# DeepBlender/DeepDenoiser

Hardware: AMD Instinct MI355X
Metric: train tiles/sec (128x128x32ch U-Net KPCN) (higher is better)
Workload: dtype bf16; 1 GPU; BASELINE config 2: U-Net [64,96,128]x4 + 5x5 KernelPrediction + 3-scale MultiScalePrediction, 32-channel render-pass stack, 128x128 tiles, full training step (fwd+SMAPE loss+bwd+Adam); global_batch=128, parallelism=dp1, hipgraph=True, inputs=resident in HBM

## Files before the change

### deepdenoiser_amd/_lib.py

```python

import ctypes as C
import os

_HERE = os.path.dirname(os.path.abspath(__file__))
LIB_PATH = os.environ.get("DD_LIB", os.path.join(_HERE, "libdd_hip.so"))

DD_F32, DD_BF16, DD_F16 = 0, 1, 2
IN_RELU, OUT_RELU, ACCUM, PIXSHUF, GATHER2X2 = 1, 2, 4, 8, 16
MAX_FEATURES, MAX_COMBINED = 32, 8
METRIC_SOURCES = MAX_FEATURES + MAX_COMBINED + 1
HISTOGRAM_DIFFERENCE, HISTOGRAM_VARIATION_DIFFERENCE, HISTOGRAM_MASKED_DIFFERENCE = 0, 1, 2
HISTOGRAM_VALUES_SCRATCH_BYTES = 20480
PREVIEW_SOURCE, PREVIEW_PREDICTION, PREVIEW_TARGET, PREVIEW_DIFFERENCE = 1, 2, 4, 8
PREVIEW_MAX_IMAGES, PREVIEW_THRESHOLDS = 16, 255
NONFINITE_MAX_PLANES = 32


def histogram_stats_offset(nb):
    return (nb + 1) // 2 * 8


def histogram_record_bytes(nb):
    return histogram_stats_offset(nb) + 48


SYMBOLS = (
    "dd_version", "dd_last_error", "dd_pack_weights", "dd_pack_weights_batched", "dd_conv_igemm", "dd_conv_wgrad", "dd_colsum", "dd_colsum_segments",
    "dd_maxpool_fwd", "dd_maxpool_bwd", "dd_avgpool", "dd_prepare_feature", "dd_gather_input",
    "dd_kpcn_fwd", "dd_kpcn_bwd", "dd_kpcn_hidden_fwd", "dd_kpcn_hidden_bwd", "dd_compose_pack", "dd_compose_blend_fwd", "dd_compose_blend_bwd",
    "dd_compose_unpack_bwd", "dd_invert_std_fwd", "dd_invert_std_bwd", "dd_loss_head", "dd_adam_step",
    "dd_stitch", "dd_recombine", "dd_probe_tr16", "dd_masked_add", "dd_zero_stuff", "dd_zero_unstuff", "dd_convert_channels",
    "dd_augment", "dd_loss_mask_sums", "dd_crc32c", "dd_extract_tiles", "dd_compose_net_fwd", "dd_compose_net_bwd",
    "dd_kpcn_head_fwd", "dd_kpcn_head_bwd", "dd_kpcn_head_bwd_multi", "dd_assemble_input", "dd_assemble_input_frames", "dd_conv3x3_bwd", "dd_conv3x3_bwd_multi", "dd_convt2x2_fwd", "dd_convt2x2_bwd", "dd_conv3x3_ks",
    "dd_conv_pw_count", "dd_wgrad_pw_count", "dd_space_to_depth2", "dd_convt3_wgrad", "dd_compose_stream_plan", "dd_compose_bwd_scratch_bytes",
    "dd_loss_msssim_scratch_bytes", "dd_loss_msssim_fwd", "dd_loss_msssim_bwd", "dd_loss_msssim_values",
    "dd_loss_metrics_scratch_bytes", "dd_loss_metrics", "dd_loss_head_path_count",
    "dd_loss_head_dscale", "dd_loss_msssim_bwd_dscale", "dd_grads_nonfinite", "dd_adam_step_scaled", "dd_scaler_update",
    "dd_histogram_values", "dd_loss_histograms_scratch_bytes", "dd_loss_histograms", "dd_loss_previews",
    "dd_nonfinite_scan", "dd_nonfinite_repair",
)


class ConvT3WgradArgs(C.Structure):
    _fields_ = [("s", C.c_void_p), ("lds", C.c_int), ("cout", C.c_int), ("cp", C.c_int),
                ("x", C.c_void_p), ("ldx", C.c_int), ("cin", C.c_int),
                ("dk", C.c_void_p),
                ("B", C.c_int), ("H", C.c_int), ("W", C.c_int), ("dtype", C.c_int)]


class ConvArgs(C.Structure):
    _fields_ = [("x", C.c_void_p), ("ldx", C.c_int), ("cin", C.c_int),
                ("wp", C.c_void_p), ("k_pad", C.c_int), ("n_pad", C.c_int),
                ("bias", C.c_void_p), ("nbias", C.c_int),
                ("res", C.c_void_p), ("ldres", C.c_int),
                ("mask", C.c_void_p), ("ldmask", C.c_int),
                ("y", C.c_void_p), ("ldy", C.c_int), ("n", C.c_int),
                ("B", C.c_int), ("H", C.c_int), ("W", C.c_int),
                ("taps", C.c_int), ("flags", C.c_int), ("dtype", C.c_int)]


class WgradArgs(C.Structure):
    _fields_ = [("p", C.c_void_p), ("ldp", C.c_int), ("m", C.c_int),
                ("q", C.c_void_p), ("ldq", C.c_int), ("n", C.c_int),
                ("out", C.c_void_p), ("bias_out", C.c_void_p), ("bias_mode", C.c_int),
                ("B", C.c_int), ("H", C.c_int), ("W", C.c_int),
                ("taps", C.c_int), ("flags", C.c_int), ("dtype", C.c_int), ("ksplit", C.c_int),
                ("stack_blocks", C.c_int), ("stack_width", C.c_int), ("stack_m0", C.c_int),
                ("stack_out", C.c_void_p * 8), ("stack_bias", C.c_void_p * 8)]


class ConvBwdArgs(C.Structure):
    _fields_ = [("dy", C.c_void_p), ("ld_dy", C.c_int), ("cout", C.c_int),
                ("x", C.c_void_p), ("ld_x", C.c_int), ("cin", C.c_int),
                ("wd", C.c_void_p), ("n_pad", C.c_int), ("k_pad", C.c_int),
                ("dx", C.c_void_p), ("ld_dx", C.c_int),
                ("dw", C.c_void_p), ("db", C.c_void_p),
                ("B", C.c_int), ("H", C.c_int), ("W", C.c_int),
                ("use_mask", C.c_int), ("accumulate", C.c_int), ("dtype", C.c_int)]


class ConvTArgs(C.Structure):
    _fields_ = [("x", C.c_void_p), ("ld_x", C.c_int), ("cin", C.c_int),
                ("y", C.c_void_p), ("ld_y", C.c_int), ("cout", C.c_int),
                ("w", C.c_void_p), ("n_pad", C.c_int), ("k_pad", C.c_int),
                ("bias", C.c_void_p), ("relu", C.c_int),
                ("dx", C.c_void_p), ("ld_dx", C.c_int), ("dw", C.c_void_p), ("db", C.c_void_p), ("use_mask", C.c_int), ("accumulate", C.c_int),
                ("B", C.c_int), ("H", C.c_int), ("W", C.c_int), ("dtype", C.c_int)]


class ConvKsArgs(C.Structure):
    _fields_ = [("x", C.c_void_p), ("ldx", C.c_int), ("cin", C.c_int),
                ("wp", C.c_void_p), ("n_pad", C.c_int), ("k_pad", C.c_int),
                ("bias", C.c_void_p), ("nbias", C.c_int),
                ("y", C.c_void_p), ("ldy", C.c_int),
                ("n0", C.c_int), ("n", C.c_int),
                ("B", C.c_int), ("H", C.c_int), ("W", C.c_int),
                ("mode", C.c_int), ("flags", C.c_int), ("dtype", C.c_int),
                ("mask", C.c_void_p), ("ldmask", C.c_int)]


class PackDesc(C.Structure):
    _fields_ = [("src", C.c_void_p), ("dst", C.c_void_p), ("taps", C.c_int), ("n", C.c_int), ("k", C.c_int), ("n_pad", C.c_int),
                ("k_pad", C.c_int), ("tap_flip", C.c_int), ("s_tap", C.c_long), ("s_n", C.c_long), ("s_k", C.c_long),
                ("dst_ld", C.c_long), ("dst_tap_stride", C.c_long)]


class FeatureParams(C.Structure):
    _fields_ = [("use_log1p", C.c_int), ("mean", C.c_float), ("inv_std", C.c_float),
                ("use_variance", C.c_int), ("variance_before", C.c_int), ("mode_neighbor", C.c_int),
                ("relative", C.c_int), ("compress", C.c_int), ("epsilon", C.c_float)]


class GatherEntry(C.Structure):
    _fields_ = [("src", C.c_void_p), ("pixel_stride", C.c_int), ("batch_stride_pixels", C.c_int),
                ("nch", C.c_int), ("dst_ch", C.c_int)]


class AssembleEntry(C.Structure):
    _fields_ = [("src", C.c_void_p), ("cs", C.c_int), ("kind", C.c_int), ("fp", FeatureParams), ("nch", C.c_int), ("dst_ch", C.c_int),
                ("std_out", C.c_void_p), ("ld_std", C.c_int)]


class LossDesc(C.Structure):
    _fields_ = [("n_features", C.c_int),
                ("pred", C.c_void_p * MAX_FEATURES), ("target", C.c_void_p * MAX_FEATURES),
                ("dpred", C.c_void_p * MAX_FEATURES),
                ("target_ld", C.c_int * MAX_FEATURES), ("pred_ld", C.c_int * MAX_FEATURES), ("nch", C.c_int * MAX_FEATURES),
                ("weight", C.c_float * MAX_FEATURES), ("var_weight", C.c_float * MAX_FEATURES),
                ("masked_weight", C.c_float * MAX_FEATURES), ("mask_feature", C.c_int * MAX_FEATURES),
                ("n_combined", C.c_int), ("comb", (C.c_int * 3) * MAX_COMBINED),
                ("comb_weight", C.c_float * MAX_COMBINED), ("comb_var_weight", C.c_float * MAX_COMBINED),
                ("comb_masked_weight", C.c_float * MAX_COMBINED), ("comb_mask_feature", C.c_int * MAX_COMBINED),
                ("n_image_combined", C.c_int), ("image_combined", C.c_int * MAX_COMBINED),
                ("n_image_features", C.c_int), ("image_features", C.c_int * MAX_FEATURES),
                ("image_weight", C.c_float), ("image_var_weight", C.c_float), ("kind", C.c_int), ("epsilon", C.c_float),
                ("mask_sums", C.c_void_p),
                ("pred_std", C.c_void_p * MAX_FEATURES), ("pred_inv", C.c_void_p * MAX_FEATURES),
                ("inv_log1p", C.c_int * MAX_FEATURES), ("inv_mean", C.c_float * MAX_FEATURES), ("inv_std", C.c_float * MAX_FEATURES)]


class MsSsimDesc(C.Structure):
    _fields_ = [("n_features", C.c_int),
                ("pred", C.c_void_p * MAX_FEATURES), ("target", C.c_void_p * MAX_FEATURES), ("dpred", C.c_void_p * MAX_FEATURES),
                ("target_ld", C.c_int * MAX_FEATURES), ("pred_ld", C.c_int * MAX_FEATURES), ("nch", C.c_int * MAX_FEATURES),
                ("ssim_weight", C.c_float * MAX_FEATURES),
                ("n_combined", C.c_int), ("comb", (C.c_int * 3) * MAX_COMBINED), ("comb_ssim_weight", C.c_float * MAX_COMBINED),
                ("n_image_combined", C.c_int), ("image_combined", C.c_int * MAX_COMBINED),
                ("n_image_features", C.c_int), ("image_features", C.c_int * MAX_FEATURES),
                ("image_ssim_weight", C.c_float)]


class ScalerState(C.Structure):
    _fields_ = [("scale", C.c_float), ("good_steps", C.c_int), ("found_nonfinite", C.c_int), ("adam_t", C.c_int), ("skipped_total", C.c_int)]


class AugmentDraw(C.Structure):
    _fields_ = [("flip", C.c_int), ("rotate", C.c_int), ("permute", C.c_int), ("normal_rotation", C.c_float * 9)]


AUG_PLAIN, AUG_RGB, AUG_NORMAL, AUG_SCREEN_NORMAL = 0, 1, 2, 3


class StitchEntry(C.Structure):
    _fields_ = [("tile", C.c_int), ("crop_y0", C.c_int), ("crop_y1", C.c_int), ("crop_x0", C.c_int),
                ("crop_x1", C.c_int), ("dst_img", C.c_int), ("dst_y", C.c_int), ("dst_x", C.c_int)]


class ComposeArgs(C.Structure):
    _fields_ = [("small", C.c_void_p), ("ld_small", C.c_int), ("fine", C.c_void_p), ("ld_fine", C.c_int), ("out", C.c_void_p), ("ld_out", C.c_int),
                ("w_in", C.c_void_p), ("b_in", C.c_void_p), ("w_res", C.c_void_p * 4), ("b_res", C.c_void_p * 4),
                ("w_out", C.c_void_p), ("b_out", C.c_void_p),
                ("save_netin", C.c_void_p), ("ld_netin", C.c_int), ("save_act", C.c_void_p * 5), ("ld_act", C.c_int * 5),
                ("save_wl", C.c_void_p), ("ld_wl", C.c_int),
                ("N", C.c_int), ("H", C.c_int), ("W", C.c_int), ("dtype", C.c_int)]


class ComposeBwdArgs(C.Structure):
    _fields_ = [("small", C.c_void_p), ("ld_small", C.c_int), ("fine", C.c_void_p), ("ld_fine", C.c_int), ("dout", C.c_void_p), ("ld_dout", C.c_int),
                ("act", C.c_void_p * 5), ("ld_act", C.c_int * 5), ("wl", C.c_void_p), ("ld_wl", C.c_int),
                ("w_in", C.c_void_p), ("w_res", C.c_void_p * 4), ("w_out", C.c_void_p),
                ("d_small", C.c_void_p), ("ld_dsmall", C.c_int), ("accumulate_small", C.c_int), ("d_fine", C.c_void_p), ("ld_dfine", C.c_int),
                ("dw_in", C.c_void_p), ("db_in", C.c_void_p), ("dw_res", C.c_void_p * 4), ("db_res", C.c_void_p * 4),
                ("dw_out", C.c_void_p), ("db_out", C.c_void_p),
                ("N", C.c_int), ("H", C.c_int), ("W", C.c_int), ("dtype", C.c_int),
                ("scratch", C.c_void_p), ("scratch_bytes", C.c_long)]


class HeadArgs(C.Structure):
    _fields_ = [("x", C.c_void_p), ("ldx", C.c_int), ("C", C.c_int), ("src", C.c_void_p), ("ldsrc", C.c_int),
                ("wa", C.c_void_p), ("ba", C.c_void_p), ("wb", C.c_void_p), ("bb", C.c_void_p),
                ("out", C.c_void_p), ("ld_out", C.c_int), ("dout", C.c_void_p), ("ld_dout", C.c_int),
                ("dx", C.c_void_p), ("ld_dx", C.c_int), ("accumulate_dx", C.c_int),
                ("dwa", C.c_void_p), ("dba", C.c_void_p), ("dwb", C.c_void_p), ("dbb", C.c_void_p),
                ("N", C.c_int), ("H", C.c_int), ("W", C.c_int), ("ksize", C.c_int), ("dtype", C.c_int)]


class RecombineDesc(C.Structure):
    _fields_ = [("n_triples", C.c_int), ("color", C.c_void_p * 4), ("direct", C.c_void_p * 4), ("indirect", C.c_void_p * 4),
                ("combined", C.c_void_p * 4), ("n_singles", C.c_int), ("single", C.c_void_p * 8), ("image", C.c_void_p)]


class NonfinitePlane(C.Structure):
    _fields_ = [("data", C.c_void_p), ("C", C.c_int), ("ld", C.c_int), ("mask", C.c_void_p)]


class NonfiniteDesc(C.Structure):
    _fields_ = [("n_planes", C.c_int), ("plane", NonfinitePlane * NONFINITE_MAX_PLANES)]


_lib = None


def _check_source_hash(lib):
    if "DD_LIB" in os.environ:
        return
    from . import build as _build
    try:
        want = _build.source_hash()
    except OSError:
        return
    got = lib.dd_version().decode()
    if ("src=" + want) not in got:
        raise RuntimeError("libdd_hip.so is stale: built from sources %s, the sources here hash to %s -- run `python -m deepdenoiser_amd.build`"
                           % (got.split("src=")[-1], want))


def source_hash():
    return load().dd_version().decode().split("src=")[-1]


def load():
    global _lib
    if _lib is not None:
        return _lib
    import torch
    if not os.path.exists(LIB_PATH):
        raise RuntimeError("libdd_hip.so is not built (%s missing): run `python -m deepdenoiser_amd.build`. "
                           "There is no CPU/PyTorch fallback for the hot path." % LIB_PATH)
    lib = C.CDLL(LIB_PATH)
    missing = [s for s in SYMBOLS if not hasattr(lib, s)]
    if missing:
        raise RuntimeError("libdd_hip.so lacks symbols %s: rebuild it" % missing)
    lib.dd_version.restype = C.c_char_p
    lib.dd_last_error.restype = C.c_char_p
    _check_source_hash(lib)
    for s in SYMBOLS[2:]:
        getattr(lib, s).restype = C.c_int
    vp, i, l, f = C.c_void_p, C.c_int, C.c_long, C.c_float
    lib.dd_pack_weights.argtypes = [vp, vp, i, i, i, i, i, i, l, l, l, i, vp]
    lib.dd_pack_weights_batched.argtypes = [vp, i, i, vp]
    lib.dd_conv_igemm.argtypes = [C.POINTER(ConvArgs), vp]
    lib.dd_conv_wgrad.argtypes = [C.POINTER(WgradArgs), vp]
    lib.dd_conv3x3_bwd.argtypes = [C.POINTER(ConvBwdArgs), vp]
    lib.dd_conv3x3_bwd_multi.argtypes = [C.POINTER(ConvBwdArgs), i, vp]
    lib.dd_convt2x2_fwd.argtypes = [C.POINTER(ConvTArgs), vp]
    lib.dd_convt2x2_bwd.argtypes = [C.POINTER(ConvTArgs), vp]
    lib.dd_conv3x3_ks.argtypes = [C.POINTER(ConvKsArgs), vp]
    lib.dd_space_to_depth2.argtypes = [vp, i, vp, i, i, i, i, i, i, i, vp]
    lib.dd_convt3_wgrad.argtypes = [C.POINTER(ConvT3WgradArgs), vp]
    lib.dd_conv_pw_count.argtypes = []
    lib.dd_conv_pw_count.restype = C.c_long
    lib.dd_wgrad_pw_count.argtypes = []
    lib.dd_wgrad_pw_count.restype = C.c_long
    lib.dd_colsum.argtypes = [vp, i, i, l, vp, i, vp]
    lib.dd_colsum_segments.argtypes = [vp, i, i, l, i, vp, i, vp, i, vp]
    lib.dd_maxpool_fwd.argtypes = [vp, i, vp, i, vp, i, i, i, i, i, i, i, i, vp]
    lib.dd_maxpool_bwd.argtypes = [vp, i, vp, vp, i, vp, i, i, i, i, i, i, i, i, i, vp]
    lib.dd_avgpool.argtypes = [vp, i, vp, i, i, i, i, i, i, vp]
    lib.dd_prepare_feature.argtypes = [vp, i, vp, i, C.POINTER(FeatureParams), i, i, i, vp]
    lib.dd_gather_input.argtypes = [vp, i, i, vp, i, i, i, i, i, i, vp]
    lib.dd_kpcn_fwd.argtypes = [vp, i, vp, i, vp, i, i, i, i, i, i, vp]
    lib.dd_kpcn_bwd.argtypes = [vp, i, vp, i, vp, i, vp, i, i, i, i, i, i, i, vp]
    lib.dd_kpcn_hidden_fwd.argtypes = [vp, i, vp, i, i, vp, i, vp, vp, i, i, i, i, i, i, vp]
    lib.dd_kpcn_hidden_bwd.argtypes = [vp, i, vp, i, i, vp, i, vp, vp, i, vp, i, i, i, i, i, i, i, vp]
    lib.dd_compose_pack.argtypes = [vp, i, vp, i, vp, i, i, i, i, i, i, vp]
    lib.dd_compose_blend_fwd.argtypes = [vp, i, vp, i, vp, i, vp, i, i, i, i, i, vp]
    lib.dd_compose_blend_bwd.argtypes = [vp, i, vp, i, vp, i, vp, i, vp, i, i, vp, i, vp, i, i, i, i, i, i, vp]
    lib.dd_compose_unpack_bwd.argtypes = [vp, i, vp, i, vp, i, i, i, i, i, vp]
    lib.dd_invert_std_fwd.argtypes = [vp, vp, l, i, f, f, vp]
    lib.dd_invert_std_bwd.argtypes = [vp, vp, vp, l, i, f, f, vp]
    lib.dd_loss_head.argtypes = [C.POINTER(LossDesc), i, i, i, vp, f, vp]
    lib.dd_loss_head_path_count.argtypes = [i]
    lib.dd_loss_head_path_count.restype = C.c_long
    lib.dd_loss_msssim_scratch_bytes.argtypes = [i, i, i, i]
    lib.dd_loss_msssim_scratch_bytes.restype = C.c_long
    lib.dd_loss_msssim_fwd.argtypes = [C.POINTER(MsSsimDesc), i, i, i, vp, vp, vp]
    lib.dd_loss_msssim_bwd.argtypes = [C.POINTER(MsSsimDesc), i, i, i, vp, f, vp]
    lib.dd_loss_msssim_values.argtypes = [C.POINTER(MsSsimDesc), i, i, i, vp, vp, vp]
    lib.dd_loss_metrics_scratch_bytes.argtypes = [i, i, i]
    lib.dd_loss_metrics_scratch_bytes.restype = C.c_long
    lib.dd_loss_metrics.argtypes = [C.POINTER(LossDesc), i, i, i, vp, vp, vp]
    lib.dd_histogram_values.argtypes = [vp, l, vp, i, vp, vp, vp]
    lib.dd_loss_histograms_scratch_bytes.argtypes = [i, i, i, i]
    lib.dd_loss_histograms_scratch_bytes.restype = C.c_long
    lib.dd_loss_histograms.argtypes = [C.POINTER(LossDesc), i, i, i, C.POINTER(C.c_int), i, vp, i, vp, vp, vp]
    lib.dd_loss_previews.argtypes = [C.POINTER(LossDesc), C.POINTER(vp), C.POINTER(C.c_int), i, i, i, C.POINTER(C.c_int), i, C.POINTER(C.c_int), i, i, vp, f, f,
                                     vp, vp]
    lib.dd_adam_step.argtypes = [vp, vp, vp, vp, l, f, f, f, f, f, vp]
    lib.dd_loss_head_dscale.argtypes = [C.POINTER(LossDesc), i, i, i, vp, vp, vp]
    lib.dd_loss_msssim_bwd_dscale.argtypes = [C.POINTER(MsSsimDesc), i, i, i, vp, vp, vp]
    lib.dd_grads_nonfinite.argtypes = [vp, l, vp, vp]
    lib.dd_adam_step_scaled.argtypes = [vp, vp, vp, vp, l, C.c_double, C.c_double, C.c_double, f, f, vp, vp]
    lib.dd_scaler_update.argtypes = [vp, f, f, i, f, f, vp]
    lib.dd_nonfinite_scan.argtypes = [C.POINTER(NonfiniteDesc), i, i, i, vp, vp]
    lib.dd_nonfinite_repair.argtypes = [C.POINTER(NonfiniteDesc), i, i, i, i, vp, vp]
    lib.dd_stitch.argtypes = [vp, i, i, vp, i, i, i, i, vp, i, vp]
    lib.dd_recombine.argtypes = [C.POINTER(RecombineDesc), l, vp]
    lib.dd_probe_tr16.argtypes = [vp, vp, vp, vp]
    lib.dd_masked_add.argtypes = [vp, i, vp, i, vp, i, i, l, i, i, vp]
    lib.dd_convert_channels.argtypes = [vp, i, i, vp, i, i, i, i, l, vp]
    lib.dd_zero_stuff.argtypes = [vp, i, vp, i, i, i, i, i, i, vp]
    lib.dd_zero_unstuff.argtypes = [vp, i, vp, i, vp, i, i, i, i, i, i, i, vp]
    lib.dd_augment.argtypes = [vp, vp, i, i, i, i, vp, i, i, i, i, i, vp]
    lib.dd_loss_mask_sums.argtypes = [vp, i, i, i, vp, vp]
    lib.dd_crc32c.argtypes = [vp, C.c_size_t, C.c_uint32, C.POINTER(C.c_uint32)]
    lib.dd_extract_tiles.argtypes = [vp, i, i, i, i, vp, i, i, vp, i, vp]
    lib.dd_compose_net_fwd.argtypes = [C.POINTER(ComposeArgs), vp]
    lib.dd_compose_net_bwd.argtypes = [C.POINTER(ComposeBwdArgs), vp]
    lib.dd_compose_stream_plan.argtypes = [i, i, i, i, C.POINTER(C.c_int)]
    lib.dd_compose_bwd_scratch_bytes.argtypes = [i, i, i]
    lib.dd_compose_bwd_scratch_bytes.restype = C.c_long
    lib.dd_assemble_input.argtypes = [vp, i, i, vp, i, i, i, i, i, i, vp]
    lib.dd_assemble_input_frames.argtypes = [vp, i, i, vp, i, i, i, i, i, i, vp, i, i, vp]
    lib.dd_kpcn_head_fwd.argtypes = [C.POINTER(HeadArgs), vp]
    lib.dd_kpcn_head_bwd.argtypes = [C.POINTER(HeadArgs), vp]
    lib.dd_kpcn_head_bwd_multi.argtypes = [C.POINTER(HeadArgs), i, vp]
    _lib = lib
    return lib


def check(rc):
    if rc != 0:
        raise RuntimeError("libdd_hip: %s (status %d)" % (load().dd_last_error().decode(), rc))
```

### deepdenoiser_amd/csrc/dd_compose_stream.h

```cpp
#pragma once
#include "dd_common.h"
#include <type_traits>

namespace {

typedef __attribute__((ext_vector_type(16))) float f32x16_t;
typedef __attribute__((ext_vector_type(2))) unsigned int cs_u32x2;

template <typename T> __device__ __forceinline__ f32x16_t mma32(uint4 a, uint4 b, f32x16_t c);
template <> __device__ __forceinline__ f32x16_t mma32<bf16_t>(uint4 a, uint4 b, f32x16_t c) {
  return __builtin_amdgcn_mfma_f32_32x32x16_bf16(__builtin_bit_cast(bf16x8_t, a), __builtin_bit_cast(bf16x8_t, b), c, 0, 0, 0);
}
template <> __device__ __forceinline__ f32x16_t mma32<f16_t>(uint4 a, uint4 b, f32x16_t c) {
  return __builtin_amdgcn_mfma_f32_32x32x16_f16(__builtin_bit_cast(f16x8_t, a), __builtin_bit_cast(f16x8_t, b), c, 0, 0, 0);
}

typedef __attribute__((ext_vector_type(4))) unsigned int cs_u32x4;
template <typename T> __device__ __forceinline__ f32x16_t mma32_zero(uint4 a, uint4 b);
template <> __device__ __forceinline__ f32x16_t mma32_zero<bf16_t>(uint4 a, uint4 b) {
  f32x16_t d;
  const cs_u32x4 av = {a.x, a.y, a.z, a.w}, bv = {b.x, b.y, b.z, b.w};
  asm volatile("v_mfma_f32_32x32x16_bf16 %0, %1, %2, 0" : "=&v"(d) : "v"(av), "v"(bv));
  return d;
}
template <> __device__ __forceinline__ f32x16_t mma32_zero<f16_t>(uint4 a, uint4 b) {
  f32x16_t d;
  const cs_u32x4 av = {a.x, a.y, a.z, a.w}, bv = {b.x, b.y, b.z, b.w};
  asm volatile("v_mfma_f32_32x32x16_f16 %0, %1, %2, 0" : "=&v"(d) : "v"(av), "v"(bv));
  return d;
}

template <typename T> __device__ __forceinline__ void unpack2(uint32_t w, float& lo, float& hi);
template <> __device__ __forceinline__ void unpack2<bf16_t>(uint32_t w, float& lo, float& hi) { lo = __uint_as_float(w << 16); hi = __uint_as_float(w & 0xffff0000u); }
template <> __device__ __forceinline__ void unpack2<f16_t>(uint32_t w, float& lo, float& hi) { unpack_f16x2(w, lo, hi); }
template <typename T> __device__ __forceinline__ uint32_t packo(float lo, float hi) {
  uint32_t w = pack2<T>(lo, hi);
  asm("" : "+v"(w));
  return w;
}
template <typename T> struct One;
template <> struct One<bf16_t> { static constexpr uint32_t v = 0x3f80u; };
template <> struct One<f16_t> { static constexpr uint32_t v = 0x3c00u; };

__device__ __forceinline__ float dpp_xor1(float v) { return __int_as_float(__builtin_amdgcn_update_dpp(0, __float_as_int(v), 0xB1, 0xF, 0xF, true)); }
__device__ __forceinline__ void both_halves(float v, float& lower, float& upper) {
  const cs_u32x2 r = __builtin_amdgcn_permlane32_swap(__float_as_uint(v), __float_as_uint(v), false, false);
  lower = __uint_as_float(r[0]); upper = __uint_as_float(r[1]);
}

constexpr int PIXB = 48;

struct Unit { int b, yb0, yb1, xs, xe, fx0; };

template <typename P>
__device__ __forceinline__ void decode_unit(const P& p, int u, Unit& U) {
  const int j = u % p.nb, t = u / p.nb;
  const int st = t % p.n_strips;
  U.b = t / p.n_strips;
  U.yb0 = j * p.BH; U.yb1 = min(p.H, U.yb0 + p.BH);
  U.xs = st * p.SO; U.xe = min(p.W, U.xs + p.SO);
  U.fx0 = p.n_strips > 1 ? U.xs - 4 : 0;
}

struct Cursor {
  int urel, i;
  Unit U;
  template <typename P>
  __device__ __forceinline__ void init(const P& p, int u0, int nunits, int V) {
    urel = V >= 0 ? V / p.VB : -1 - ((-V - 1) / p.VB);
    i = V - urel * p.VB;
    U = Unit{0, 0, 0, 0, 0, 0};
    if (urel >= 0 && urel < nunits) decode_unit(p, u0 + urel, U);
  }
  template <typename P>
  __device__ __forceinline__ void advance(const P& p, int u0, int nunits, int rows) {
    i += rows;
    while (i >= p.VB) {
      i -= p.VB;
      ++urel;
      if (urel >= 0 && urel < nunits) decode_unit(p, u0 + urel, U);
    }
  }
};

__device__ __forceinline__ int sfl(int v) { return __builtin_amdgcn_readfirstlane(v); }
__device__ __forceinline__ int opaque(int v) { asm volatile("" : "+v"(v)); return v; }
__device__ __forceinline__ int posmod(int v, int d) { const int m = v % d; return m < 0 ? m + d : m; }

template <typename T> __device__ __forceinline__ float split3(float v, int e) {
  const float hi = Elem<T>::to_f32(Elem<T>::from_f32(v));
  const float mid = Elem<T>::to_f32(Elem<T>::from_f32(v - hi));
  const float lo = Elem<T>::to_f32(Elem<T>::from_f32(v - hi - mid));
  return e == 0 ? hi : e == 1 ? mid : lo;
}

}
```

### deepdenoiser_amd/csrc/dd_compose_stream.hip

```cpp
#include "dd_compose_stream.h"

#ifdef CS_PROFILE
__device__ unsigned long long cs_phase[4][8];
#define CSP_DECL() unsigned long long csp_last = __builtin_readcyclecounter(); const bool csp_on = blockIdx.x == 0 && t == 0 && lane == 0
#define CSP(i) do { const unsigned long long now_ = __builtin_readcyclecounter(); if (csp_on) cs_phase[LAYER][i] += now_ - csp_last; csp_last = now_; } while (0)
extern "C" int dd_debug_cs_phases(unsigned long long* out32, int reset) {
  if (out32) (void)hipMemcpyFromSymbol(out32, HIP_SYMBOL(cs_phase), sizeof(unsigned long long) * 32);
  if (reset) { unsigned long long z[32] = {0}; (void)hipMemcpyToSymbol(HIP_SYMBOL(cs_phase), z, sizeof(z)); }
  return 0;
}
#else
#define CSP_DECL()
#define CSP(i)
#endif


namespace {

constexpr int KS_MAX = 16;
constexpr int AUX_BYTES = 16 + 3 * 1024;

struct CsP {
  const float* small; const float* fine; float* out;
  const float* w_in; const float* b_in; const float* w_res[4]; const float* b_res[4]; const float* w_out; const float* b_out;
  void* save_act[5]; void* save_wl; void* save_netin;
  int ld_small, ld_fine, ld_out, ld_act[5], ld_wl, ld_netin;
  int N, H, W;
  int FW, R, TPR;
  int n_strips, SO;
  int BH, nb, VB;
  int units;
};

template <typename T>
__device__ __forceinline__ void stage_weights(char* img, char* aux, const CsP& p, int tid) {
  for (int i = tid; i < 4 * KS_MAX * 64 * 8; i += 1024) {
    const int e = i & 7, ln = (i >> 3) & 63, c = (i >> 9) & (KS_MAX - 1), l = i >> 13;
    const int m = ln & 31, g = 2 * c + (ln >> 5);
    float v = 0.f;
    if (m < 24) {
      if (g < 27) v = p.w_res[l][((g / 3) * 24 + 8 * (g % 3) + e) * 24 + m];
      else if (g == 27) { if (e < 3) v = split3<T>(p.b_res[l][m], e); }
    }
    reinterpret_cast<T*>(img)[i] = Elem<T>::from_f32(v);
  }
  T* ax = reinterpret_cast<T*>(aux);
  for (int i = tid; i < 8 + 3 * 512; i += 1024) {
    float v = 0.f;
    if (i < 8) v = i < 3 ? 1.f : 0.f;
    else {
      const int j = i - 8, e = j & 7, ln = (j >> 3) & 63, which = j >> 9;
      const int m = ln & 31, h = ln >> 5;
      if (which == 0) { if (m == 0) v = p.w_out[e < 4 ? 4 * h + e : 8 + 4 * h + e - 4]; }
      else if (which == 1) { if (m == 0) v = e < 4 ? p.w_out[16 + 4 * h + e] : (e < 7 && h == 0) ? split3<T>(p.b_out[0], e - 4) : 0.f; }
      else if (m < 24) v = e < 3 ? p.w_in[((h ? 0 : 3) + e) * 24 + m] : (e < 6 && h == 0) ? split3<T>(p.b_in[m], e - 3) : 0.f;
    }
    ax[i] = Elem<T>::from_f32(v);
  }
}

template <typename T, int LAYER, bool SAVE, int NPRE>
__device__ __forceinline__ void cs_role(const CsP& p, char* smem, char* aux, int ring_bytes, int t, int lane, int u0, int nunits, int steps) {
  constexpr bool RESIDUAL = LAYER == 1 || LAYER == 3;
  constexpr bool FINAL = LAYER == 3;
  constexpr int KS = 14;
  constexpr uint32_t ONE = One<T>::v, ONE2 = ONE | (ONE << 16);
  const int R = p.R, TPR = p.TPR, FW = p.FW, VB = p.VB;
  const int n = lane & 31, h = lane >> 5;
  const int r = t / TPR, xc = t - r * TPR;
  const bool has_task = t < R * TPR;
  const int x = xc * 32 + n;
  const int pitch = (FW + 2) * PIXB, rp = R * pitch;
  const int D0 = 3 * R + 2, D1 = 2 * R + 2, D4 = 3 * R + 2;
  const int off1 = D0 * pitch, off2 = off1 + D1 * pitch, off3 = off2 + D1 * pitch, off4 = off3 + D1 * pitch;
  const int Din = LAYER == 0 ? D0 : D1;
  const int Dres = LAYER == 1 ? D0 : D4;
  const int in_bytes = Din * pitch, out_bytes = D1 * pitch, res_bytes = Dres * pitch, raw_bytes = D4 * pitch;
  char* rin = smem + (LAYER == 0 ? 0 : LAYER == 1 ? off1 : LAYER == 2 ? off2 : off3);
  char* rout = smem + (LAYER == 0 ? off1 : LAYER == 1 ? off2 : off3);
  char* rres = smem + (LAYER == 1 ? 0 : off4);

  uint4 wa[KS];
#pragma unroll
  for (int c = 0; c < KS; ++c) wa[c] = *reinterpret_cast<const uint4*>(smem + ((LAYER * KS_MAX + c) * 64 + lane) * 16);
  __syncthreads();
  for (int i = threadIdx.x; i < ring_bytes / 16; i += 1024) reinterpret_cast<uint4*>(smem)[i] = uint4{0u, 0u, 0u, 0u};

  const int H = p.H, W = p.W, h2 = H >> 1, w2 = W >> 1;
  const int lag = (LAYER + 1) * (R + 1);
  const int total_rows = nunits * VB;
  const int s_beg = has_task ? (lag - r + R - 1) / R : steps, s_end = has_task ? (total_rows + lag - r + R - 1) / R : steps;
  Cursor cur;
  cur.init(p, u0, nunits, r - lag);
  int o_in = posmod(r - lag, Din) * pitch, o_out = posmod(r - lag, D1) * pitch, o_res = posmod(r - lag, Dres) * pitch, o_raw = posmod(r - lag, D4) * pitch;
  auto wrap_add = [](int o, int add, int bytes) { o += add; return o >= bytes ? o - bytes : o; };
  const int xo = x * PIXB + h * 16;
  const int a4c = h ? x * PIXB : x * PIXB + 128;
  const int a13c = h ? (int)(aux - rin) : x * PIXB + 128;
  const int wr = (x + 1) * PIXB + h * 8;
  int ybase = 0, pixb = 0;
  bool col_in = false, col_own = false, cols_all_in = false;
  auto unit_values = [&](const Cursor& c, int& yb, int& pb, bool& ci, bool& co, bool& call) {
    const int gx = c.U.fx0 + x;
    yb = c.U.yb0 - 4;
    ci = (unsigned)gx < (unsigned)W;
    co = ci && gx >= c.U.xs && gx < c.U.xe;
    pb = c.U.b * H * W + (ci ? gx : 0);
    call = c.U.fx0 + xc * 32 >= 0 && c.U.fx0 + xc * 32 + 32 <= W;
  };
  unit_values(cur, ybase, pixb, col_in, col_own, cols_all_in);

  Cursor c0;
  int o0 = 0, ybase0 = 0, pixb0 = 0, pix0 = 0;
  bool col_in0 = false, col_own0 = false, cols_all_in0 = false, in0 = false, own0 = false, row_in0 = false;
  float xin[3] = {0.f, 0.f, 0.f};
  const int s0_end = has_task ? (total_rows - r + R - 1) / R : 0;
  auto load_x0 = [&](int s_next) {
    in0 = false; own0 = false; row_in0 = false;
    if (s_next < s0_end) {
      const int y = ybase0 + c0.i;
      row_in0 = (unsigned)y < (unsigned)H;
      in0 = row_in0 && col_in0;
      own0 = in0 && col_own0 && y >= c0.U.yb0 && y < c0.U.yb1;
      const int cy = row_in0 ? y : 0;
      pix0 = pixb0 + cy * W;
      const int cx = pix0 - (c0.U.b * H + cy) * W;
      const float* src = h ? p.small + (size_t)((c0.U.b * h2 + (cy >> 1)) * w2 + (cx >> 1)) * p.ld_small : p.fine + (size_t)pix0 * p.ld_fine;
#ifdef CS_EXP_NO_STAGE0_LOADS
      xin[0] = (float)pix0; xin[1] = 1.f; xin[2] = 0.5f;
      (void)src;
#else
      xin[0] = src[0]; xin[1] = src[1]; xin[2] = src[2];
#endif
    }
  };
  if (LAYER == 0) {
    c0.init(p, u0, nunits, r);
    o0 = posmod(r, D0) * pitch;
    unit_values(c0, ybase0, pixb0, col_in0, col_own0, cols_all_in0);
    load_x0(0);
  }

  f32x16_t acc;
  auto conv_part_n = [&](auto pre_t) {
    constexpr bool pre = decltype(pre_t)::value;
    constexpr int C0 = pre ? 0 : NPRE, C1 = pre ? NPRE : KS;
    const int o_m1 = o_in == 0 ? in_bytes - pitch : o_in - pitch;
    const int o_p1 = o_in + pitch == in_bytes ? 0 : o_in + pitch;
    const char* q0 = rin + xo + o_m1;
    const char* q1 = rin + xo + 16 + o_in;
    const char* q2 = rin + xo + o_p1;
    const char* q4 = rin + a4c + (h ? o_in : o_m1);
    const char* q13 = rin + a13c + (h ? 0 : o_p1);
    f32x16_t c_init = {0.f, 0.f, 0.f, 0.f, 0.f, 0.f, 0.f, 0.f, 0.f, 0.f, 0.f, 0.f, 0.f, 0.f, 0.f, 0.f};
    if (RESIDUAL && pre) {
      const char* qr = rres + o_res + wr;
      uint2 rv[3];
#pragma unroll
      for (int b = 0; b < 3; ++b) rv[b] = *reinterpret_cast<const uint2*>(qr + b * 16);
#pragma unroll
      for (int b = 0; b < 3; ++b) {
        float r0, r1, r2, r3;
        unpack2<T>(rv[b].x, r0, r1); unpack2<T>(rv[b].y, r2, r3);
        c_init[4 * b] = r0; c_init[4 * b + 1] = r1; c_init[4 * b + 2] = r2; c_init[4 * b + 3] = r3;
      }
    }
    constexpr int BATCH = 6;
#pragma unroll
    for (int c0_ = C0; c0_ < C1; c0_ += BATCH) {
      uint4 bf[BATCH];
#pragma unroll
      for (int c = c0_; c < c0_ + BATCH && c < C1; ++c) {
        const char* a = c < 4 ? q0 + 32 * c : c == 4 ? q4 : c < 9 ? q1 + 32 * (c - 5) : c < 13 ? q2 + 32 * (c - 9) : q13;
#ifdef CS_EXP_NO_LDSREAD
        bf[c - c0_] = uint4{(uint32_t)x, (uint32_t)c, 0u, 0u};
#else
        bf[c - c0_] = *reinterpret_cast<const uint4*>(a);
#endif
      }
      __builtin_amdgcn_sched_barrier(0);
#pragma unroll
      for (int c = c0_; c < c0_ + BATCH && c < C1; ++c) {
#ifdef CS_EXP_NO_MFMA
        acc[c] = ((pre && c == 0) ? c_init[c] : acc[c]) + __uint_as_float(bf[c - c0_].x ^ wa[c].x);
#else
        acc = mma32<T>(wa[c], bf[c - c0_], (pre && c == 0) ? c_init : acc);
#endif
      }
      __builtin_amdgcn_sched_barrier(0);
    }
    if (pre && NPRE == 0) acc = c_init;
  };

  bool act = 0 >= s_beg && 0 < s_end;
  if (act) conv_part_n(std::true_type());

  CSP_DECL();
  for (int s = 0; s < steps; ++s) {
    CSP(0);
#ifndef CS_EXP_NO_BARRIER
    __syncthreads();
#endif
    CSP(1);
    if (LAYER == 0) {
      if (s < s0_end) {
        const uint4 w0 = *reinterpret_cast<const uint4*>(aux + 16 + 2048 + lane * 16);
        const uint4 bx = {pack2<T>(xin[0], xin[1]), pack2<T>(xin[2], h ? 0.f : 1.f), h ? 0u : ONE2, 0u};
        const f32x16_t z = {0.f, 0.f, 0.f, 0.f, 0.f, 0.f, 0.f, 0.f, 0.f, 0.f, 0.f, 0.f, 0.f, 0.f, 0.f, 0.f};
        const f32x16_t a0 = mma32<T>(w0, bx, z);
        char* o = rin + o0 + wr;
        const bool in_now = in0, own_now = own0, all_in = row_in0 && cols_all_in0;
        const int pix_now = pix0;
        if (SAVE && own_now && p.save_netin) {
          T* d = reinterpret_cast<T*>(p.save_netin) + (size_t)pix_now * p.ld_netin + (h ? 0 : 3);
#pragma unroll
          for (int e = 0; e < 3; ++e) d[e] = Elem<T>::from_f32(xin[e]);
          if (!h) { d[3] = Elem<T>::from_f32(0.f); d[4] = Elem<T>::from_f32(0.f); }
        }
        uint2 pk[3];
#pragma unroll
        for (int b = 0; b < 3; ++b) {
          pk[b].x = relu_bf16x2(packo<T>(a0[4 * b], a0[4 * b + 1]));
          pk[b].y = relu_bf16x2(packo<T>(a0[4 * b + 2], a0[4 * b + 3]));
        }
        if (!all_in) {
#pragma unroll
          for (int b = 0; b < 3; ++b) { pk[b].x = in_now ? pk[b].x : 0u; pk[b].y = in_now ? pk[b].y : 0u; }
        }
#pragma unroll
        for (int b = 0; b < 3; ++b) {
          *reinterpret_cast<uint2*>(o + b * 16) = pk[b];
          if (SAVE && own_now && p.save_act[0])
            *reinterpret_cast<uint2*>(reinterpret_cast<char*>(p.save_act[0]) + ((size_t)pix_now * p.ld_act[0] + 8 * b + 4 * h) * 2) = pk[b];
        }
      }
      c0.i += R;
      if (c0.i >= VB) {
        c0.i -= R;
        c0.advance(p, u0, nunits, R);
        unit_values(c0, ybase0, pixb0, col_in0, col_own0, cols_all_in0);
      }
      o0 = wrap_add(o0, rp, D0 * pitch);
      load_x0(s + 1);
    }
    CSP(2);
    if (act) {
      const int y = ybase + cur.i;
      const bool row_in = (unsigned)y < (unsigned)H;
      const bool all_in = row_in && cols_all_in;
      const bool inside = row_in && col_in;
      const bool own = inside && col_own && y >= cur.U.yb0 && y < cur.U.yb1;
      const int cy = row_in ? y : 0;
      const int pix = pixb + cy * W;
      float f3[3] = {0.f, 0.f, 0.f}, s3[3] = {0.f, 0.f, 0.f};
      if (FINAL) {
#ifndef CS_EXP_NO_TAIL_LOADS
        const int cx = pix - (cur.U.b * H + cy) * W;
        const float* fr = p.fine + (size_t)(pix + (h - (cy & 1)) * W) * p.ld_fine;
        const float* sp = p.small + (size_t)((cur.U.b * h2 + (cy >> 1)) * w2 + (cx >> 1)) * p.ld_small;
#pragma unroll
        for (int c = 0; c < 3; ++c) { f3[c] = fr[c]; s3[c] = sp[c]; }
#endif
      }
      conv_part_n(std::false_type());
      CSP(4);
      uint4 wo1 = {0u, 0u, 0u, 0u}, wo2 = {0u, 0u, 0u, 0u};
      if (FINAL) {
        wo1 = *reinterpret_cast<const uint4*>(aux + 16 + lane * 16);
        wo2 = *reinterpret_cast<const uint4*>(aux + 16 + 1024 + lane * 16);
      }
      uint2 pk[3];
#pragma unroll
      for (int b = 0; b < 3; ++b) {
        pk[b].x = packo<T>(acc[4 * b], acc[4 * b + 1]);
        pk[b].y = packo<T>(acc[4 * b + 2], acc[4 * b + 3]);
      }
      if (!FINAL) {
        if (LAYER == 1) {
          char* o4 = smem + off4 + o_raw + wr;
          if (!all_in) {
#pragma unroll
            for (int b = 0; b < 3; ++b) { pk[b].x = inside ? pk[b].x : 0u; pk[b].y = inside ? pk[b].y : 0u; }
          }
#pragma unroll
          for (int b = 0; b < 3; ++b) {
            *reinterpret_cast<uint2*>(o4 + b * 16) = pk[b];
            if (SAVE && own && p.save_act[2])
              *reinterpret_cast<uint2*>(reinterpret_cast<char*>(p.save_act[2]) + ((size_t)pix * p.ld_act[2] + 8 * b + 4 * h) * 2) = pk[b];
          }
        }
#pragma unroll
        for (int b = 0; b < 3; ++b) { pk[b].x = relu_bf16x2(pk[b].x); pk[b].y = relu_bf16x2(pk[b].y); }
        if (LAYER != 1 && !all_in) {
#pragma unroll
          for (int b = 0; b < 3; ++b) { pk[b].x = inside ? pk[b].x : 0u; pk[b].y = inside ? pk[b].y : 0u; }
        }
        char* o = rout + o_out + wr;
#pragma unroll
        for (int b = 0; b < 3; ++b) {
          *reinterpret_cast<uint2*>(o + b * 16) = pk[b];
          if (SAVE && LAYER != 1 && own && p.save_act[LAYER + 1])
            *reinterpret_cast<uint2*>(reinterpret_cast<char*>(p.save_act[LAYER + 1]) + ((size_t)pix * p.ld_act[LAYER + 1] + 8 * b + 4 * h) * 2) = pk[b];
        }
      } else {
#ifdef CS_EXP_NO_TAIL
        if (own && h == 0 && pk[0].x == 0x12345u) p.out[(size_t)pix * p.ld_out] = 1.f;
#else
        if (SAVE && own && p.save_act[4]) {
#pragma unroll
          for (int b = 0; b < 3; ++b)
            *reinterpret_cast<uint2*>(reinterpret_cast<char*>(p.save_act[4]) + ((size_t)pix * p.ld_act[4] + 8 * b + 4 * h) * 2) = pk[b];
        }
        const f32x16_t z = {0.f, 0.f, 0.f, 0.f, 0.f, 0.f, 0.f, 0.f, 0.f, 0.f, 0.f, 0.f, 0.f, 0.f, 0.f, 0.f};
        f32x16_t a2 = mma32<T>(wo1, uint4{pk[0].x, pk[0].y, pk[1].x, pk[1].y}, z);
        a2 = mma32<T>(wo2, uint4{pk[2].x, pk[2].y, ONE2, ONE}, a2);
        const uint32_t wlp = pack2<T>(fmaxf(a2[0], 0.f), 0.f);
        float wlv, unused;
        unpack2<T>(wlp, wlv, unused);
        const float wgt = 1.f / (1.f + __expf(-wlv));
        float res[3];
#pragma unroll
        for (int c = 0; c < 3; ++c) {
          const float pair = f3[c] + dpp_xor1(f3[c]);
          float p_lo, p_hi, f_lo, f_hi;
          both_halves(pair, p_lo, p_hi);
          both_halves(f3[c], f_lo, f_hi);
          const float low = 0.25f * (p_lo + p_hi);
          const float fme = (cy & 1) ? f_hi : f_lo;
          res[c] = fme - wgt * low + wgt * s3[c];
        }
        if (own && h == 0) {
          float* o = p.out + (size_t)pix * p.ld_out;
#pragma unroll
          for (int c = 0; c < 3; ++c) o[c] = res[c];
          if (SAVE && p.save_wl) reinterpret_cast<uint16_t*>(p.save_wl)[(size_t)pix * p.ld_wl] = (uint16_t)(wlp & 0xffffu);
        }
#endif
      }
    }
    CSP(5);
    cur.i += R;
    if (cur.i >= VB) {
      cur.i -= R;
      cur.advance(p, u0, nunits, R);
      unit_values(cur, ybase, pixb, col_in, col_own, cols_all_in);
    }
    o_in = wrap_add(o_in, rp, in_bytes);
    if (!FINAL) o_out = wrap_add(o_out, rp, out_bytes);
    if (RESIDUAL) o_res = wrap_add(o_res, rp, res_bytes);
    if (LAYER == 1) o_raw = wrap_add(o_raw, rp, raw_bytes);
    act = s + 1 >= s_beg && s + 1 < s_end;
    if (act) conv_part_n(std::true_type());
    CSP(6);
  }
}

template <typename T, bool SAVE, bool R1>
__global__ __launch_bounds__(1024) void compose_stream_fwd_kernel(const CsP p) {
  extern __shared__ __attribute__((aligned(16))) char smem[];
  const int tid = threadIdx.x, lane = tid & 63, wave = sfl(tid >> 6);
  const int rows = 12 * p.R + 10;
  const int ring_bytes = rows * (p.FW + 2) * PIXB;
  char* aux = smem + ring_bytes;
  stage_weights<T>(smem, aux, p, tid);
  const int G = gridDim.x, g = blockIdx.x;
  const int u0 = (int)(((long)p.units * g) / G), u1 = (int)(((long)p.units * (g + 1)) / G);
  const int nunits = u1 - u0;
  const int steps = nunits > 0 ? (nunits * p.VB + 4 * (p.R + 1) + p.R - 1) / p.R : 0;
  const int layer = wave >> 2, t = wave & 3;
  __syncthreads();
  const int r = t / p.TPR;
#define CS_ROLE(L)                                                                                   \
  do {                                                                                               \
    if (R1 || r == 0) cs_role<T, L, SAVE, 9>(p, smem, aux, ring_bytes, t, lane, u0, nunits, steps);  \
    else if (r == 1) cs_role<T, L, SAVE, 4>(p, smem, aux, ring_bytes, t, lane, u0, nunits, steps);   \
    else cs_role<T, L, SAVE, 0>(p, smem, aux, ring_bytes, t, lane, u0, nunits, steps);               \
  } while (0)
  if (layer == 0) CS_ROLE(0);
  else if (layer == 1) CS_ROLE(1);
  else if (layer == 2) CS_ROLE(2);
  else CS_ROLE(3);
#undef CS_ROLE
}

}

extern "C" int dd_compose_stream_plan(int N, int H, int W, int cus, int* out8) {
  if (N <= 0 || H <= 0 || W <= 0 || cus <= 0 || !out8) return DD_ERR_INVALID;
  int n_strips = 1, SO = W, FW = ((W + 31) / 32) * 32;
  if (W > 128) {
    for (n_strips = 2;; ++n_strips) {
      SO = (W + n_strips - 1) / n_strips;
      SO += SO & 1;
      FW = ((SO + 8 + 31) / 32) * 32;
      if (FW <= 128) break;
    }
  }
  const int R = FW == 32 ? 4 : FW == 64 ? 2 : 1;
  long best = -1; int bestBH = 0;
  for (int d = 1; d <= 16; ++d) {
    int BH = (H + d - 1) / d;
    BH = ((BH + 3) / 4) * 4;
    if (BH < 4) BH = 4;
    const int nb = (H + BH - 1) / BH;
    const long units = (long)N * n_strips * nb;
    const long G = units < cus ? units : cus;
    const long per = (units + G - 1) / G;
    const long cost = per * (BH + 8) + 4 * (R + 1);
    if (best < 0 || cost < best) { best = cost; bestBH = BH; }
  }
  const int nb = (H + bestBH - 1) / bestBH;
  out8[0] = FW; out8[1] = R; out8[2] = FW / 32; out8[3] = n_strips; out8[4] = SO; out8[5] = bestBH; out8[6] = nb; out8[7] = bestBH + 8;
  return DD_OK;
}

int dd_compose_stream_fwd_launch(const dd_compose_args* a, hipStream_t s) {
  CsP p;
  p.small = a->small; p.fine = a->fine; p.out = a->out;
  p.w_in = a->w_in; p.b_in = a->b_in; p.w_out = a->w_out; p.b_out = a->b_out;
  for (int l = 0; l < 4; ++l) { p.w_res[l] = a->w_res[l]; p.b_res[l] = a->b_res[l]; }
  bool save = a->save_wl != nullptr;
  for (int i = 0; i < 5; ++i) { p.save_act[i] = a->save_act[i]; p.ld_act[i] = a->ld_act[i]; save = save || a->save_act[i]; }
  p.save_wl = a->save_wl; p.ld_wl = a->ld_wl;
  p.save_netin = a->save_netin; p.ld_netin = a->ld_netin; save = save || a->save_netin;
  p.ld_small = a->ld_small; p.ld_fine = a->ld_fine; p.ld_out = a->ld_out;
  p.N = a->N; p.H = a->H; p.W = a->W;
  DD_REQUIRE((long)a->N * a->H * a->W < (1l << 31) / 64, "dd_compose_net_fwd: N * H * W = %ld pixels exceed the 32-bit offsets of the kernel", (long)a->N * a->H * a->W);
  const int cus = dd_device_cus();
  int g8[8];
  if (dd_compose_stream_plan(a->N, a->H, a->W, cus, g8) != DD_OK) return DD_ERR_INVALID;
  p.FW = g8[0]; p.R = g8[1]; p.TPR = g8[2]; p.n_strips = g8[3]; p.SO = g8[4]; p.BH = g8[5]; p.nb = g8[6]; p.VB = g8[7];
  p.units = a->N * p.n_strips * p.nb;
  const int grid = p.units < cus ? p.units : cus;
  const int lds = (12 * p.R + 10) * (p.FW + 2) * PIXB + AUX_BYTES;
#define CS_LAUNCH(T, SV, R1)                                                                          \
  do {                                                                                                \
    dd_allow_max_lds(reinterpret_cast<const void*>(compose_stream_fwd_kernel<T, SV, R1>));            \
    hipLaunchKernelGGL((compose_stream_fwd_kernel<T, SV, R1>), dim3(grid), dim3(1024), lds, s, p);    \
  } while (0)
#define CS_LAUNCH_R(T, SV) do { if (p.R == 1) CS_LAUNCH(T, SV, true); else CS_LAUNCH(T, SV, false); } while (0)
  if (a->dtype == DD_BF16) { if (save) CS_LAUNCH_R(bf16_t, true); else CS_LAUNCH_R(bf16_t, false); }
  else { if (save) CS_LAUNCH_R(f16_t, true); else CS_LAUNCH_R(f16_t, false); }
#undef CS_LAUNCH_R
#undef CS_LAUNCH
  DD_LAUNCH_CHECK();
  return DD_OK;
}
```

### deepdenoiser_amd/csrc/dd_compose_stream_bwd.hip

```cpp
#include "dd_compose_stream.h"

namespace {

constexpr int KS = 14;
constexpr int KS_MAX = 16;
constexpr int TAILB = 40;
constexpr int AUX_BYTES = 2 * 1024 + 128;

struct CbP {
  const float* small; const float* fine; const float* gout;
  const void* act[4];
  const void* wl;
  const float* w_in; const float* w_res[4]; const float* w_out;
  float* d_small; float* d_fine;
  void* g[5];
  void* x0;
  void* dz6;
  int ld_small, ld_fine, ld_gout, ld_act[4], ld_wl, ld_dsmall, ld_dfine, acc_small;
  int N, H, W;
  int FW, R, TPR, n_strips, SO, BH, nb, VB, units;
};

template <typename T>
__device__ __forceinline__ void stage_weights_bwd(char* img, char* aux, const CbP& p, int tid) {
  for (int i = tid; i < 4 * KS_MAX * 64 * 8; i += 1024) {
    const int e = i & 7, ln = (i >> 3) & 63, c = (i >> 9) & (KS_MAX - 1), l = i >> 13;
    const int m = ln & 31, g = 2 * c + (ln >> 5);
    float v = 0.f;
    if (m < 24 && g < 27) v = p.w_res[3 - l][((8 - g / 3) * 24 + m) * 24 + 8 * (g % 3) + e];
    reinterpret_cast<T*>(img)[i] = Elem<T>::from_f32(v);
  }
  T* ax = reinterpret_cast<T*>(aux);
  for (int i = tid; i < 2 * 512; i += 1024) {
    const int e = i & 7, ln = (i >> 3) & 63, which = i >> 9;
    const int m = ln & 31, h = ln >> 5;
    float v = 0.f;
    if (m < 6) {
      const int ch = which == 0 ? (e < 4 ? 4 * h + e : 8 + 4 * h + e - 4) : (e < 4 ? 16 + 4 * h + e : -1);
      if (ch >= 0) v = p.w_in[m * 24 + ch];
    }
    ax[i] = Elem<T>::from_f32(v);
  }
  float* wo = reinterpret_cast<float*>(aux + 2048);
  for (int i = tid; i < 32; i += 1024) wo[i] = i < 24 ? Elem<T>::to_f32(Elem<T>::from_f32(p.w_out[i])) : 0.f;
}

__device__ __forceinline__ uint2 mask2(uint2 v, uint2 m) { return uint2{mask_bf16x2(v.x, m.x), mask_bf16x2(v.y, m.y)}; }

template <typename T, int LAYER, int NPRE>
__device__ __forceinline__ void cb_role(const CbP& p, char* smem, char* aux, char* tail, int ring_bytes, int t, int lane, int u0, int nunits, int steps) {
  constexpr bool RES_AFTER = LAYER == 1;
  constexpr bool RES_INIT = LAYER == 3;
  constexpr bool FINAL = LAYER == 3;
  const int R = p.R, TPR = p.TPR, FW = p.FW, VB = p.VB;
  const int n = lane & 31, h = lane >> 5;
  const int r = t / TPR, xc = t - r * TPR;
  const bool has_task = t < R * TPR;
  const int x = xc * 32 + n;
  const int pitch = (FW + 2) * PIXB, rp = R * pitch;
  const int D0 = 3 * R + 2, D1 = 2 * R + 2;
  const int off1 = D0 * pitch, off2 = off1 + D1 * pitch, off3 = off2 + D0 * pitch;
  const int Din = (LAYER == 0 || LAYER == 2) ? D0 : D1;
  const int Dout = (LAYER == 1) ? D0 : D1;
  const int in_bytes = Din * pitch, out_bytes = Dout * pitch, res_bytes = D0 * pitch;
  char* rin = smem + (LAYER == 0 ? 0 : LAYER == 1 ? off1 : LAYER == 2 ? off2 : off3);
  char* rout = smem + (LAYER == 0 ? off1 : LAYER == 1 ? off2 : off3);
  char* rres = smem + (LAYER == 1 ? 0 : off2);
  const int DT = 2 * R + 2, tail_pitch = FW * TAILB, tail_bytes = DT * tail_pitch;

  uint4 wa[KS];
#pragma unroll
  for (int c = 0; c < KS; ++c) wa[c] = *reinterpret_cast<const uint4*>(smem + ((LAYER * KS_MAX + c) * 64 + lane) * 16);
  __syncthreads();
  for (int i = threadIdx.x; i < ring_bytes / 16; i += 1024) reinterpret_cast<uint4*>(smem)[i] = uint4{0u, 0u, 0u, 0u};

  const int H = p.H, W = p.W, h2 = H >> 1, w2 = W >> 1;
  const int lag = (LAYER + 1) * (R + 1);
  const int total_rows = nunits * VB;
  const int s_beg = has_task ? (lag - r + R - 1) / R : steps, s_end = has_task ? (total_rows + lag - r + R - 1) / R : steps;
  Cursor cur;
  cur.init(p, u0, nunits, r - lag);
  int o_in = posmod(r - lag, Din) * pitch, o_out = posmod(r - lag, Dout) * pitch, o_res = posmod(r - lag, D0) * pitch;
  int o_tail = posmod(r - lag, DT) * tail_pitch;
  auto wrap_add = [](int o, int add, int bytes) { o += add; return o >= bytes ? o - bytes : o; };
  const int xo = x * PIXB + h * 16;
  const int a4c = h ? x * PIXB : x * PIXB + 128;
  const int a13c = x * PIXB + 128;
  const int wr = (x + 1) * PIXB + h * 8;
  int ybase = 0, pixb = 0;
  bool col_in = false, col_own = false, cols_all_in = false;
  auto unit_values = [&](const Cursor& c, int& yb, int& pb, bool& ci, bool& co, bool& call) {
    const int gx = c.U.fx0 + x;
    yb = c.U.yb0 - 4;
    ci = (unsigned)gx < (unsigned)W;
    co = ci && gx >= c.U.xs && gx < c.U.xe;
    pb = c.U.b * H * W + (ci ? gx : 0);
    call = c.U.fx0 + xc * 32 >= 0 && c.U.fx0 + xc * 32 + 32 <= W;
  };
  unit_values(cur, ybase, pixb, col_in, col_own, cols_all_in);

  Cursor c0;
  int o0 = 0, ybase0 = 0, pixb0 = 0, pix0 = 0;
  bool col_in0 = false, col_own0 = false, cols_all_in0 = false, in0 = false, own0 = false, odd0 = false;
  float g0[3] = {0.f, 0.f, 0.f}, sm0[3] = {0.f, 0.f, 0.f}, f0[3] = {0.f, 0.f, 0.f}, wl0 = 0.f;
  const int s0_end = has_task ? (total_rows - r + R - 1) / R : 0;
  auto load_s0 = [&](int s_next) {
    in0 = false; own0 = false;
    if (s_next < s0_end) {
      const int y = ybase0 + c0.i;
      const bool row_in = (unsigned)y < (unsigned)H;
      in0 = row_in && col_in0;
      own0 = in0 && col_own0 && y >= c0.U.yb0 && y < c0.U.yb1;
      const int cy = row_in ? y : 0;
      odd0 = (cy & 1) != 0;
      pix0 = pixb0 + cy * W;
      const int cx = pix0 - (c0.U.b * H + cy) * W;
      const float* gp = p.gout + (size_t)pix0 * p.ld_gout;
      const float* sp = p.small + (size_t)((c0.U.b * h2 + (cy >> 1)) * w2 + (cx >> 1)) * p.ld_small;
      const float* fr = p.fine + (size_t)(pix0 + (h - (cy & 1)) * W) * p.ld_fine;
#pragma unroll
      for (int c = 0; c < 3; ++c) { g0[c] = gp[c]; sm0[c] = sp[c]; f0[c] = fr[c]; }
      wl0 = Elem<T>::to_f32(reinterpret_cast<const T*>(p.wl)[(size_t)pix0 * p.ld_wl]);
    }
  };
  if (LAYER == 0) {
    c0.init(p, u0, nunits, r);
    o0 = posmod(r, D0) * pitch;
    unit_values(c0, ybase0, pixb0, col_in0, col_own0, cols_all_in0);
    load_s0(0);
  }

  f32x16_t acc;
  auto conv_part_n = [&](auto pre_t) {
    constexpr bool pre = decltype(pre_t)::value;
    constexpr int C0 = pre ? 0 : NPRE, C1 = pre ? NPRE : KS;
    const int o_m1 = o_in == 0 ? in_bytes - pitch : o_in - pitch;
    const int o_p1 = o_in + pitch == in_bytes ? 0 : o_in + pitch;
    const char* q0 = rin + xo + o_m1;
    const char* q1 = rin + xo + 16 + o_in;
    const char* q2 = rin + xo + o_p1;
    const char* q4 = rin + a4c + (h ? o_in : o_m1);
    const char* q13 = rin + a13c + o_p1;
    f32x16_t c_init = {0.f, 0.f, 0.f, 0.f, 0.f, 0.f, 0.f, 0.f, 0.f, 0.f, 0.f, 0.f, 0.f, 0.f, 0.f, 0.f};
    if (RES_INIT && pre) {
      const char* qr = rres + o_res + wr;
      uint2 rv[3];
#pragma unroll
      for (int b = 0; b < 3; ++b) rv[b] = *reinterpret_cast<const uint2*>(qr + b * 16);
#pragma unroll
      for (int b = 0; b < 3; ++b) {
        float r0, r1, r2, r3;
        unpack2<T>(rv[b].x, r0, r1); unpack2<T>(rv[b].y, r2, r3);
        c_init[4 * b] = r0; c_init[4 * b + 1] = r1; c_init[4 * b + 2] = r2; c_init[4 * b + 3] = r3;
      }
    }
    constexpr int BATCH = 6;
#pragma unroll
    for (int c0_ = C0; c0_ < C1; c0_ += BATCH) {
      uint4 bf[BATCH];
#pragma unroll
      for (int c = c0_; c < c0_ + BATCH && c < C1; ++c) {
        const char* a = c < 4 ? q0 + 32 * c : c == 4 ? q4 : c < 9 ? q1 + 32 * (c - 5) : c < 13 ? q2 + 32 * (c - 9) : q13;
        bf[c - c0_] = *reinterpret_cast<const uint4*>(a);
      }
      __builtin_amdgcn_sched_barrier(0);
#pragma unroll
      for (int c = c0_; c < c0_ + BATCH && c < C1; ++c) acc = mma32<T>(wa[c], bf[c - c0_], (pre && c == 0) ? c_init : acc);
      __builtin_amdgcn_sched_barrier(0);
    }
    if (pre && NPRE == 0) acc = c_init;
  };

  bool act = 0 >= s_beg && 0 < s_end;
  if (act) conv_part_n(std::true_type());
  int prev_y = -1, prev_pixb = 0, prev_b = 0;
  bool prev_own_row = false, prev_col_own = false;

  for (int s = 0; s < steps; ++s) {
    __syncthreads();
    if (LAYER == 0) {
      if (s < s0_end) {
        float low[3], f_own[3], dwv = 0.f;
        const bool odd_row = odd0;
#pragma unroll
        for (int c = 0; c < 3; ++c) {
          const float pair = f0[c] + dpp_xor1(f0[c]);
          float p_lo, p_hi, f_lo, f_hi;
          both_halves(pair, p_lo, p_hi);
          both_halves(f0[c], f_lo, f_hi);
          f_own[c] = odd_row ? f_hi : f_lo;
          low[c] = 0.25f * (p_lo + p_hi);
          dwv += g0[c] * (sm0[c] - low[c]);
        }
        const float w = 1.f / (1.f + __expf(-wl0));
        float dz6 = (in0 && wl0 > 0.f) ? dwv * w * (1.f - w) : 0.f;
        const uint32_t dzp = pack2<T>(dz6, 0.f);
        float unused;
        unpack2<T>(dzp, dz6, unused);
        if (own0 && h == 0) {
          reinterpret_cast<uint16_t*>(p.dz6)[pix0] = (uint16_t)(dzp & 0xffffu);
          float fo[3];
#pragma unroll
          for (int c = 0; c < 3; ++c) fo[c] = f_own[c];
          reinterpret_cast<uint4*>(p.x0)[pix0] = uint4{pack2<T>(sm0[0], sm0[1]), pack2<T>(sm0[2], fo[0]), pack2<T>(fo[1], fo[2]), One<T>::v};
        }
        const float* wo = reinterpret_cast<const float*>(aux + 2048);
        char* o = rin + o0 + wr;
        char* gd = reinterpret_cast<char*>(p.g[4]) + ((size_t)pix0 * 24 + 4 * h) * 2;
#pragma unroll
        for (int b = 0; b < 3; ++b) {
          const f32x4_t wv = *reinterpret_cast<const f32x4_t*>(wo + 8 * b + 4 * h);
          uint2 pk;
          pk.x = pack2<T>(wv[0] * dz6, wv[1] * dz6); pk.y = pack2<T>(wv[2] * dz6, wv[3] * dz6);
          *reinterpret_cast<uint2*>(o + b * 16) = pk;
          if (own0) *reinterpret_cast<uint2*>(gd + b * 16) = pk;
        }
      }
      c0.i += R;
      if (c0.i >= VB) {
        c0.i -= R;
        c0.advance(p, u0, nunits, R);
        unit_values(c0, ybase0, pixb0, col_in0, col_own0, cols_all_in0);
      }
      o0 = wrap_add(o0, rp, D0 * pitch);
      load_s0(s + 1);
    }
    if (FINAL && prev_y >= 0 && (prev_y & 1)) {
      int o_odd = o_tail - R * tail_pitch; if (o_odd < 0) o_odd += tail_bytes;
      int o_even = o_odd - tail_pitch; if (o_even < 0) o_even += tail_bytes;
      const float* rec = reinterpret_cast<const float*>(tail + (h ? o_odd : o_even) + x * TAILB);
      float u[3], ds[3], q[3];
#pragma unroll
      for (int c = 0; c < 3; ++c) { u[c] = rec[c]; ds[c] = rec[3 + c]; q[c] = rec[6 + c]; }
      const int yrow = prev_y - 1 + h;
      const int pix = prev_pixb + yrow * W;
      const bool own = prev_own_row && prev_col_own;
      float* dsm = p.d_small + (size_t)((prev_b * h2 + (prev_y >> 1)) * w2 + ((pix - (prev_b * H + yrow) * W) >> 1)) * p.ld_dsmall;
      float old[3] = {0.f, 0.f, 0.f};
      const bool writer = own && h == 0 && !(n & 1);
      if (p.acc_small && writer) { old[0] = dsm[0]; old[1] = dsm[1]; old[2] = dsm[2]; }
#pragma unroll
      for (int c = 0; c < 3; ++c) {
        float a_lo, a_hi, b_lo, b_hi;
        both_halves(u[c] + dpp_xor1(u[c]), a_lo, a_hi);
        both_halves(ds[c] + dpp_xor1(ds[c]), b_lo, b_hi);
        const float ts = a_lo + a_hi, dsum = b_lo + b_hi;
        if (own) p.d_fine[(size_t)pix * p.ld_dfine + c] = q[c] - 0.25f * ts;
        if (writer) dsm[c] = old[c] + ts + dsum;
      }
    }
    int parked_y = -1;
    if (act) {
      const int y = ybase + cur.i;
      const bool row_in = (unsigned)y < (unsigned)H;
      const bool all_in = row_in && cols_all_in;
      const bool inside = row_in && col_in;
      const bool own_row = y >= cur.U.yb0 && y < cur.U.yb1;
      const bool own = inside && col_own && own_row;
      const int cy = row_in ? y : 0;
      const int pix = pixb + cy * W;
      constexpr int MASK_ACT = 3 - LAYER;
      const char* mp = reinterpret_cast<const char*>(p.act[MASK_ACT]) + ((size_t)pix * p.ld_act[MASK_ACT] + 4 * h) * 2;
      uint2 mk[3];
#pragma unroll
#ifdef CB_EXP_NO_MASK_LOADS
      for (int b = 0; b < 3; ++b) mk[b] = uint2{0x3f803f80u, (unsigned)pix};
      (void)mp;
#else
      for (int b = 0; b < 3; ++b) mk[b] = *reinterpret_cast<const uint2*>(mp + b * 16);
#endif
      float gt[3] = {0.f, 0.f, 0.f}, wlt = 0.f;
      if (FINAL) {
        const float* gp = p.gout + (size_t)pix * p.ld_gout;
#pragma unroll
        for (int c = 0; c < 3; ++c) gt[c] = gp[c];
        wlt = Elem<T>::to_f32(reinterpret_cast<const T*>(p.wl)[(size_t)pix * p.ld_wl]);
      }
      uint2 rv[3] = {uint2{0u, 0u}, uint2{0u, 0u}, uint2{0u, 0u}};
      if (RES_AFTER) {
        const char* qr = rres + o_res + wr;
#pragma unroll
        for (int b = 0; b < 3; ++b) rv[b] = *reinterpret_cast<const uint2*>(qr + b * 16);
      }
      conv_part_n(std::false_type());
      uint2 pk[3];
      if (RES_AFTER) {
#pragma unroll
        for (int b = 0; b < 3; ++b) {
          float m0, m1, m2, m3, r0, r1, r2, r3;
          unpack2<T>(mk[b].x, m0, m1); unpack2<T>(mk[b].y, m2, m3);
          unpack2<T>(rv[b].x, r0, r1); unpack2<T>(rv[b].y, r2, r3);
          pk[b].x = packo<T>(r0 + (m0 > 0.f ? acc[4 * b] : 0.f), r1 + (m1 > 0.f ? acc[4 * b + 1] : 0.f));
          pk[b].y = packo<T>(r2 + (m2 > 0.f ? acc[4 * b + 2] : 0.f), r3 + (m3 > 0.f ? acc[4 * b + 3] : 0.f));
        }
      } else {
#pragma unroll
        for (int b = 0; b < 3; ++b) {
          pk[b].x = packo<T>(acc[4 * b], acc[4 * b + 1]);
          pk[b].y = packo<T>(acc[4 * b + 2], acc[4 * b + 3]);
          pk[b] = mask2(pk[b], mk[b]);
        }
      }
      if (!all_in) {
#pragma unroll
        for (int b = 0; b < 3; ++b) { pk[b].x = inside ? pk[b].x : 0u; pk[b].y = inside ? pk[b].y : 0u; }
      }
#ifdef CB_EXP_NO_G_STORES
      if (own && pk[0].x == 0x12345u) {
#else
      if (own) {
#endif
        char* gp = reinterpret_cast<char*>(p.g[3 - LAYER]) + ((size_t)pix * 24 + 4 * h) * 2;
#pragma unroll
        for (int b = 0; b < 3; ++b) *reinterpret_cast<uint2*>(gp + b * 16) = pk[b];
      }
      if (!FINAL) {
        char* o = rout + o_out + wr;
#pragma unroll
        for (int b = 0; b < 3; ++b) *reinterpret_cast<uint2*>(o + b * 16) = pk[b];
      } else {
        const uint4 wi1 = *reinterpret_cast<const uint4*>(aux + lane * 16);
        const uint4 wi2 = *reinterpret_cast<const uint4*>(aux + 1024 + lane * 16);
        const f32x16_t z = {0.f, 0.f, 0.f, 0.f, 0.f, 0.f, 0.f, 0.f, 0.f, 0.f, 0.f, 0.f, 0.f, 0.f, 0.f, 0.f};
        f32x16_t d = mma32<T>(wi1, uint4{pk[0].x, pk[0].y, pk[1].x, pk[1].y}, z);
        d = mma32<T>(wi2, uint4{pk[2].x, pk[2].y, 0u, 0u}, d);
        float dx[4];
#pragma unroll
        for (int e = 0; e < 4; ++e) dx[e] = Elem<T>::to_f32(Elem<T>::from_f32(d[e]));
        const float w = 1.f / (1.f + __expf(-wlt));
        float* rec = reinterpret_cast<float*>(tail + o_tail + x * TAILB);
        const bool live = inside;
        if (h == 0) {
#pragma unroll
          for (int c = 0; c < 3; ++c) { rec[c] = live ? w * gt[c] : 0.f; rec[3 + c] = live ? dx[c] : 0.f; }
          rec[6] = gt[0] + dx[3];
        } else {
          rec[7] = gt[1] + dx[0];
          rec[8] = gt[2] + dx[1];
        }
        parked_y = y;
        prev_own_row = own_row; prev_col_own = col_own && col_in; prev_pixb = pixb; prev_b = cur.U.b;
      }
    }
    prev_y = parked_y;
    cur.i += R;
    if (cur.i >= VB) {
      cur.i -= R;
      cur.advance(p, u0, nunits, R);
      unit_values(cur, ybase, pixb, col_in, col_own, cols_all_in);
    }
    o_in = wrap_add(o_in, rp, in_bytes);
    if (!FINAL) o_out = wrap_add(o_out, rp, out_bytes);
    if (RES_AFTER || RES_INIT) o_res = wrap_add(o_res, rp, res_bytes);
    if (FINAL) o_tail = wrap_add(o_tail, R * tail_pitch, tail_bytes);
    act = s + 1 >= s_beg && s + 1 < s_end;
    if (act) conv_part_n(std::true_type());
  }
  if (FINAL) {
    __syncthreads();
    if (prev_y >= 0 && (prev_y & 1)) {
      int o_odd = o_tail - R * tail_pitch; if (o_odd < 0) o_odd += tail_bytes;
      int o_even = o_odd - tail_pitch; if (o_even < 0) o_even += tail_bytes;
      const float* rec = reinterpret_cast<const float*>(tail + (h ? o_odd : o_even) + x * TAILB);
      const int yrow = prev_y - 1 + h;
      const int pix = prev_pixb + yrow * W;
      const bool own = prev_own_row && prev_col_own;
      float* dsm = p.d_small + (size_t)((prev_b * h2 + (prev_y >> 1)) * w2 + ((pix - (prev_b * H + yrow) * W) >> 1)) * p.ld_dsmall;
      const bool writer = own && h == 0 && !(n & 1);
#pragma unroll
      for (int c = 0; c < 3; ++c) {
        float a_lo, a_hi, b_lo, b_hi;
        both_halves(rec[c] + dpp_xor1(rec[c]), a_lo, a_hi);
        both_halves(rec[3 + c] + dpp_xor1(rec[3 + c]), b_lo, b_hi);
        const float ts = a_lo + a_hi, dsum = b_lo + b_hi;
        if (own) p.d_fine[(size_t)pix * p.ld_dfine + c] = rec[6 + c] - 0.25f * ts;
        if (writer) dsm[c] = (p.acc_small ? dsm[c] : 0.f) + ts + dsum;
      }
    }
  } else {
    __syncthreads();
  }
}

template <typename T, int RR>
__global__ __launch_bounds__(1024) void compose_stream_bwd_kernel(const CbP p) {
  extern __shared__ __attribute__((aligned(16))) char smem[];
  const int tid = threadIdx.x, lane = tid & 63, wave = sfl(tid >> 6);
  const int rows = 10 * p.R + 8;
  const int ring_bytes = rows * (p.FW + 2) * PIXB;
  char* aux = smem + ring_bytes;
  char* tail = aux + AUX_BYTES;
  stage_weights_bwd<T>(smem, aux, p, tid);
  const int G = gridDim.x, g = blockIdx.x;
  const int u0 = (int)(((long)p.units * g) / G), u1 = (int)(((long)p.units * (g + 1)) / G);
  const int nunits = u1 - u0;
  const int steps = nunits > 0 ? (nunits * p.VB + 4 * (p.R + 1) + p.R - 1) / p.R : 0;
  const int layer = wave >> 2, t = wave & 3;
  __syncthreads();
  const int r = t / p.TPR;
#define CB_ROLE(L)                                                                                        \
  do {                                                                                                    \
    if (RR == 1 || r == 0) cb_role<T, L, 9>(p, smem, aux, tail, ring_bytes, t, lane, u0, nunits, steps);  \
    else if (RR == 2 || r == 1) cb_role<T, L, 4>(p, smem, aux, tail, ring_bytes, t, lane, u0, nunits, steps); \
    else cb_role<T, L, 0>(p, smem, aux, tail, ring_bytes, t, lane, u0, nunits, steps);                    \
  } while (0)
  if (layer == 0) CB_ROLE(0);
  else if (layer == 1) CB_ROLE(1);
  else if (layer == 2) CB_ROLE(2);
  else CB_ROLE(3);
#undef CB_ROLE
}

}

int dd_compose_stream_plan(int N, int H, int W, int cus, int* out8);

extern "C" long dd_compose_bwd_scratch_bytes(int N, int H, int W) { return (long)N * H * W * (5 * 48 + 16 + 16); }

int dd_compose_stream_bwd_data_launch(const dd_compose_bwd_args* a, void* scratch, hipStream_t s) {
  CbP p;
  p.small = a->small; p.fine = a->fine; p.gout = a->dout; p.wl = a->wl;
  for (int i = 0; i < 4; ++i) { p.act[i] = a->act[i]; p.ld_act[i] = a->ld_act[i]; }
  p.w_in = a->w_in; p.w_out = a->w_out;
  for (int l = 0; l < 4; ++l) p.w_res[l] = a->w_res[l];
  p.d_small = a->d_small; p.d_fine = a->d_fine;
  const long npix = (long)a->N * a->H * a->W;
  for (int i = 0; i < 5; ++i) p.g[i] = reinterpret_cast<char*>(scratch) + (size_t)i * npix * 48;
  p.x0 = reinterpret_cast<char*>(scratch) + (size_t)5 * npix * 48;
  p.dz6 = reinterpret_cast<char*>(scratch) + (size_t)npix * (5 * 48 + 16);
  p.ld_small = a->ld_small; p.ld_fine = a->ld_fine; p.ld_gout = a->ld_dout; p.ld_wl = a->ld_wl; p.ld_dsmall = a->ld_dsmall; p.ld_dfine = a->ld_dfine;
  p.acc_small = a->accumulate_small;
  p.N = a->N; p.H = a->H; p.W = a->W;
  const int cus = dd_device_cus();
  int g8[8];
  if (dd_compose_stream_plan(a->N, a->H, a->W, cus, g8) != DD_OK) return DD_ERR_INVALID;
  p.FW = g8[0]; p.R = g8[1]; p.TPR = g8[2]; p.n_strips = g8[3]; p.SO = g8[4]; p.BH = g8[5]; p.nb = g8[6]; p.VB = g8[7];
  p.units = a->N * p.n_strips * p.nb;
  const int grid = p.units < cus ? p.units : cus;
  const int lds = (10 * p.R + 8) * (p.FW + 2) * PIXB + AUX_BYTES + (2 * p.R + 2) * p.FW * TAILB;
#define CB_LAUNCH(T, RR)                                                                              \
  do {                                                                                                \
    dd_allow_max_lds(reinterpret_cast<const void*>(compose_stream_bwd_kernel<T, RR>));                \
    hipLaunchKernelGGL((compose_stream_bwd_kernel<T, RR>), dim3(grid), dim3(1024), lds, s, p);        \
  } while (0)
#define CB_LAUNCH_R(T) do { if (p.R == 1) CB_LAUNCH(T, 1); else if (p.R == 2) CB_LAUNCH(T, 2); else CB_LAUNCH(T, 4); } while (0)
  DD_REQUIRE(p.R == 1 || p.R == 2 || p.R == 4, "dd_compose_net_bwd: %d rows per step", p.R);
  if (a->dtype == DD_BF16) CB_LAUNCH_R(bf16_t); else CB_LAUNCH_R(f16_t);
#undef CB_LAUNCH_R
#undef CB_LAUNCH
  DD_LAUNCH_CHECK();
  return DD_OK;
}

namespace {

constexpr int WG_SW = 64;
constexpr int WG_GROW = 4096, WG_AROW = 3072;
constexpr int WG_WAVES = 12;

struct CwP {
  const void* act[5];
  const void* g[5];
  const void* x0;
  const void* dz6;
  const void* zero16;
  float* dw_in; float* db_in; float* dw_res[4]; float* db_res[4]; float* dw_out; float* db_out;
  int N, H, W, strips, BH, nb, units;
};

typedef __attribute__((address_space(3))) s16x4_t* cw_tr_ptr;
__device__ __forceinline__ uint2 cw_tr(unsigned addr) {
  const s16x4_t v = __builtin_amdgcn_ds_read_tr16_b64_v4i16(reinterpret_cast<cw_tr_ptr>(addr));
  return __builtin_bit_cast(uint2, v);
}
__device__ __forceinline__ void cw_dma_1k(const void* gptr, unsigned lds_addr) {
  asm volatile("s_mov_b32 m0, %1\n\ts_nop 0\n\tglobal_load_lds_dwordx4 %0, off" : : "v"(gptr), "s"(lds_addr) : "memory");
}

template <int N> __device__ __forceinline__ void cw_wait_vm() { asm volatile("s_waitcnt vmcnt(%0)" : : "n"(N) : "memory"); }

constexpr int CW_G_OFF = 0, CW_A_OFF = CW_G_OFF + 20 * WG_GROW, CW_A3_OFF = CW_A_OFF + 12 * WG_AROW, CW_Z1_OFF = CW_A3_OFF + 3 * WG_AROW;
constexpr int CW_X0_OFF = CW_Z1_OFF + 3 * WG_AROW, CW_Z6_OFF = CW_X0_OFF + 3 * 1024, CW_LDS = CW_Z6_OFF + 3 * 1024;

template <typename T>
__global__ __launch_bounds__(WG_WAVES * 64) void compose_stream_wgrad_kernel(const CwP p) {
  extern __shared__ __attribute__((aligned(1024))) char smem[];
  constexpr uint32_t ONE = One<T>::v, ONE2 = ONE | (ONE << 16);
  const int tid = threadIdx.x, lane = tid & 63, wave = sfl(tid >> 6);
  const unsigned lds0 = (unsigned)(uintptr_t)(__attribute__((address_space(3))) char*)smem;
  const int H = p.H, W = p.W;
  const int G = gridDim.x, gb = blockIdx.x;
  const int u0 = (int)(((long)p.units * gb) / G), u1 = (int)(((long)p.units * (gb + 1)) / G);

  const int layer = wave / 3, dyi = wave % 3;
  f32x16_t acc[4];
#pragma unroll
  for (int i = 0; i < 4; ++i)
#pragma unroll
    for (int e = 0; e < 16; ++e) acc[i][e] = 0.f;
  const int m = lane & 31, kh = lane >> 5, t16 = lane & 15, cblk = (lane >> 4) & 1;
  const unsigned tr_lane = (unsigned)((t16 >> 2) * PIXB + cblk * 32 + (t16 & 3) * 8);
  const bool ones_row = m == 24;
  auto gslot = [](int row) { return (row + 10) % 5; };
  auto aslot = [](int row) { return (row + 9) % 3; };

  for (int u = u0; u < u1; ++u) {
    const int j = u % p.nb, tq = u / p.nb, st = tq % p.strips, b = tq / p.strips;
    const int yb0 = j * p.BH, yb1 = min(H, yb0 + p.BH), xs = st * WG_SW;
    struct Piece { const char* src; bool colok; unsigned dst; int isg, rowb; size_t rb; };
    auto make_piece = [&](int c) {
      Piece q;
      int chunk, gx, part = 0;
      const char* base;
      size_t pxbytes = 48;
      q.rb = (size_t)W * 48;
      if (c < 16) {
        const int tensor = c >> 2; chunk = c & 3;
        const int piece = chunk * 64 + lane, px = (piece * 171) >> 9;
        part = piece - px * 3; gx = xs - 1 + px;
        base = reinterpret_cast<const char*>(p.g[1 + tensor]);
        q.isg = 1; q.rowb = WG_GROW;
        q.dst = lds0 + CW_G_OFF + tensor * 5 * WG_GROW + chunk * 1024;
      } else if (c < 34) {
        const int tensor = (c - 16) / 3; chunk = (c - 16) % 3;
        const int piece = chunk * 64 + lane, px = (piece * 171) >> 9;
        part = piece - px * 3; gx = xs + px;
        base = tensor < 5 ? reinterpret_cast<const char*>(p.act[tensor]) : reinterpret_cast<const char*>(p.g[0]);
        q.isg = 0; q.rowb = WG_AROW;
        q.dst = lds0 + chunk * 1024 + (tensor < 4 ? CW_A_OFF + tensor * 3 * WG_AROW : tensor == 4 ? CW_A3_OFF : CW_Z1_OFF);
      } else if (c == 34) {
        gx = xs + lane; base = reinterpret_cast<const char*>(p.x0); pxbytes = 16; q.rb = (size_t)W * 16;
        q.isg = 0; q.rowb = 1024; q.dst = lds0 + CW_X0_OFF;
      } else {
        gx = lane < 8 ? xs + 8 * lane : W; base = reinterpret_cast<const char*>(p.dz6); pxbytes = 2; q.rb = (size_t)W * 2;
        q.isg = 0; q.rowb = 1024; q.dst = lds0 + CW_Z6_OFF;
      }
      q.colok = (unsigned)gx < (unsigned)W;
      q.src = base + ((size_t)(b * H) * W + (q.colok ? gx : 0)) * pxbytes + part * 16;
      return q;
    };
    const Piece q0 = make_piece(wave), q1 = make_piece(wave + 12), q2 = make_piece(wave + 24);
    auto issue = [&](const Piece& q, int y) {
      const int row = y + q.isg;
      const bool ok = (unsigned)row < (unsigned)H && q.colok;
      const char* src = ok ? q.src + (size_t)row * q.rb : reinterpret_cast<const char*>(p.zero16);
      const unsigned dst = q.dst + (q.isg ? gslot(row) : aslot(row)) * q.rowb;
      cw_dma_1k(src, (unsigned)sfl((int)dst));
    };
    auto dma = [&](int y) { issue(q0, y); issue(q1, y); issue(q2, y); };
    auto dma_first = [&](int y) {
#pragma unroll
      for (int e = 0; e < 3; ++e) {
        const int c = wave + 12 * e;
        if (c < 32) {
          const int tensor = (c >> 2) & 3, chunk = c & 3, row = y - 1 + (c >> 4);
          const int piece = chunk * 64 + lane, px = (piece * 171) >> 9, part = piece - px * 3;
          const int gx = xs - 1 + px;
          const bool ok = (unsigned)row < (unsigned)H && (unsigned)gx < (unsigned)W;
          const char* src = ok ? reinterpret_cast<const char*>(p.g[1 + tensor]) + ((size_t)((b * H + row) * W + gx) * 24) * 2 + part * 16
                               : reinterpret_cast<const char*>(p.zero16);
          cw_dma_1k(src, (unsigned)sfl((int)(lds0 + CW_G_OFF + (tensor * 5 + gslot(row)) * WG_GROW + chunk * 1024)));
        }
      }
    };
    dma_first(yb0);
    dma(yb0);
    dma(yb0 + 1);
    for (int y = yb0; y < yb1; ++y) {
      cw_wait_vm<3>();
      __syncthreads();
      dma(y + 2);
      const int grow = y - (dyi - 1);
      const unsigned abase = lds0 + CW_A_OFF + (layer * 3 + aslot(y)) * WG_AROW + tr_lane + kh * 8 * PIXB;
      const unsigned gbase = lds0 + CW_G_OFF + (layer * 5 + gslot(grow)) * WG_GROW + tr_lane + kh * 8 * PIXB;
      if ((unsigned)grow < (unsigned)H) {
#pragma unroll
        for (int k = 0; k < 4; ++k) {
          const uint2 a_lo = cw_tr(abase + k * 16 * PIXB), a_hi = cw_tr(abase + k * 16 * PIXB + 4 * PIXB);
          uint4 af = {a_lo.x, a_lo.y, a_hi.x, a_hi.y};
          if (layer == 2) af = relu16<T>(af);
          if (ones_row && dyi == 1) af = uint4{ONE2, ONE2, ONE2, ONE2};
          const uint2 w01 = cw_tr(gbase + k * 16 * PIXB), w23 = cw_tr(gbase + k * 16 * PIXB + 4 * PIXB), w45 = cw_tr(gbase + k * 16 * PIXB + 8 * PIXB);
          const uint4 f_m1 = {w01.x, w01.y, w23.x, w23.y};
          const uint4 f_p1 = {w01.y, w23.x, w23.y, w45.x};
          const uint4 f_0 = {__builtin_amdgcn_alignbit(w01.y, w01.x, 16), __builtin_amdgcn_alignbit(w23.x, w01.y, 16),
                             __builtin_amdgcn_alignbit(w23.y, w23.x, 16), __builtin_amdgcn_alignbit(w45.x, w23.y, 16)};
          acc[0] = mma32<T>(af, f_p1, acc[0]);
          acc[1] = mma32<T>(af, f_0, acc[1]);
          acc[2] = mma32<T>(af, f_m1, acc[2]);
        }
      }
      if (wave == 0) {
        const unsigned xbase = lds0 + CW_X0_OFF + aslot(y) * 1024 + (unsigned)((t16 >> 2) * 16 + (t16 & 3) * 8) + kh * 8 * 16;
        const unsigned zbase = lds0 + CW_Z1_OFF + aslot(y) * WG_AROW + tr_lane + kh * 8 * PIXB;
#pragma unroll
        for (int k = 0; k < 4; ++k) {
          uint4 af = {0u, 0u, 0u, 0u};
          if (cblk == 0) {
            const uint2 a_lo = cw_tr(xbase + k * 16 * 16), a_hi = cw_tr(xbase + k * 16 * 16 + 4 * 16);
            af = uint4{a_lo.x, a_lo.y, a_hi.x, a_hi.y};
          }
          const uint2 b_lo = cw_tr(zbase + k * 16 * PIXB), b_hi = cw_tr(zbase + k * 16 * PIXB + 4 * PIXB);
          acc[3] = mma32<T>(af, uint4{b_lo.x, b_lo.y, b_hi.x, b_hi.y}, acc[3]);
        }
      } else if (wave == 1) {
        const unsigned a3base = lds0 + CW_A3_OFF + aslot(y) * WG_AROW + tr_lane + kh * 8 * PIXB;
        const char* z6 = smem + CW_Z6_OFF + aslot(y) * 1024;
#pragma unroll
        for (int k = 0; k < 4; ++k) {
          const uint2 a_lo = cw_tr(a3base + k * 16 * PIXB), a_hi = cw_tr(a3base + k * 16 * PIXB + 4 * PIXB);
          uint4 af = {a_lo.x, a_lo.y, a_hi.x, a_hi.y};
          if (ones_row) {
            const int px = xs + k * 16 + kh * 8;
            af = uint4{px < W ? ONE2 : 0u, px + 2 < W ? ONE2 : 0u, px + 4 < W ? ONE2 : 0u, px + 6 < W ? ONE2 : 0u};
          }
          uint4 bfr = {0u, 0u, 0u, 0u};
          if (m == 0) bfr = *reinterpret_cast<const uint4*>(z6 + (k * 16 + kh * 8) * 2);
          acc[3] = mma32<T>(af, bfr, acc[3]);
        }
      }
    }
    cw_wait_vm<0>();
    __syncthreads();
  }

  dd_det_wait();
  if (u1 > u0) {
    float* dw = p.dw_res[layer];
#pragma unroll
    for (int dxi = 0; dxi < 3; ++dxi) {
      const int tap = dyi * 3 + dxi;
#pragma unroll
      for (int i = 0; i < 16; ++i) {
        const int row = (i >> 2) * 8 + kh * 4 + (i & 3), col = m;
        if (col < 24) {
          if (row < 24) atomicAdd(dw + (tap * 24 + row) * 24 + col, acc[dxi][i]);
          else if (row == 24 && tap == 4) atomicAdd(p.db_res[layer] + col, acc[dxi][i]);
        }
      }
    }
    if (wave == 0) {
#pragma unroll
      for (int i = 0; i < 16; ++i) {
        const int row = (i >> 2) * 8 + kh * 4 + (i & 3), col = m;
        if (col < 24) {
          if (row < 6) atomicAdd(p.dw_in + row * 24 + col, acc[3][i]);
          else if (row == 6) atomicAdd(p.db_in + col, acc[3][i]);
        }
      }
    } else if (wave == 1) {
#pragma unroll
      for (int i = 0; i < 16; ++i) {
        const int row = (i >> 2) * 8 + kh * 4 + (i & 3);
        if (m == 0) {
          if (row < 24) atomicAdd(p.dw_out + row, acc[3][i]);
          else if (row == 24) atomicAdd(p.db_out, acc[3][i]);
        }
      }
    }
  }
  dd_det_end();
}

}

static __device__ uint4 dd_cw_zero_page = {0u, 0u, 0u, 0u};

int dd_compose_stream_wgrad_launch(const dd_compose_bwd_args* a, void* scratch, hipStream_t s) {
  CwP p;
  for (int i = 0; i < 5; ++i) p.act[i] = a->act[i];
  const long npix = (long)a->N * a->H * a->W;
  for (int i = 0; i < 5; ++i) p.g[i] = reinterpret_cast<char*>(scratch) + (size_t)i * npix * 48;
  p.x0 = reinterpret_cast<char*>(scratch) + (size_t)5 * npix * 48;
  p.dz6 = reinterpret_cast<char*>(scratch) + (size_t)npix * (5 * 48 + 16);
  void* zp = nullptr;
  if (hipGetSymbolAddress(&zp, HIP_SYMBOL(dd_cw_zero_page)) != hipSuccess) { dd_set_error("dd_compose_net_bwd: no zero page"); return DD_ERR_LAUNCH; }
  p.zero16 = zp;
  p.dw_in = a->dw_in; p.db_in = a->db_in; p.dw_out = a->dw_out; p.db_out = a->db_out;
  for (int l = 0; l < 4; ++l) { p.dw_res[l] = a->dw_res[l]; p.db_res[l] = a->db_res[l]; }
  p.N = a->N; p.H = a->H; p.W = a->W;
  p.strips = (a->W + WG_SW - 1) / WG_SW;
  const int cus = dd_device_cus();
  long best = -1; int bestBH = a->H;
  for (int d = 1; d <= 32; ++d) {
    int BH = (a->H + d - 1) / d; BH += BH & 1;
    if (BH < 2) BH = 2;
    const int nb = (a->H + BH - 1) / BH;
    const long units = (long)a->N * p.strips * nb;
    const long Gn = units < cus ? units : cus;
    const long cost = ((units + Gn - 1) / Gn) * (BH + 2);
    if (best < 0 || cost < best) { best = cost; bestBH = BH; }
  }
  p.BH = bestBH; p.nb = (a->H + bestBH - 1) / bestBH;
  p.units = a->N * p.strips * p.nb;
  const int grid = p.units < cus ? p.units : cus;
  constexpr int LDS = CW_LDS;
  dd_det_sync();
  if (a->dtype == DD_BF16) {
    dd_allow_max_lds(reinterpret_cast<const void*>(compose_stream_wgrad_kernel<bf16_t>));
    hipLaunchKernelGGL(compose_stream_wgrad_kernel<bf16_t>, dim3(grid), dim3(WG_WAVES * 64), LDS, s, p);
  } else {
    dd_allow_max_lds(reinterpret_cast<const void*>(compose_stream_wgrad_kernel<f16_t>));
    hipLaunchKernelGGL(compose_stream_wgrad_kernel<f16_t>, dim3(grid), dim3(WG_WAVES * 64), LDS, s, p);
  }
  DD_LAUNCH_CHECK();
  return DD_OK;
}
```

### deepdenoiser_amd/program.py

```python

import ctypes as C
import math
import os

import numpy as np
import torch

from . import _lib as L
from . import loss_scale as LS
from .engine import DT, Graph, round_up
from .naming import Naming
from .render_passes import RenderPasses

_LOSS_KIND = {"DIFFERENCE": 1, "ABSOLUTE": 2, "SMOOTH_ABSOLUTE": 3, "SQUARED": 4, "SMAPE": 5}


class _Namer:

    def __init__(self, scope):
        self.scope, self.counts = scope, {}

    def __call__(self, kind):
        n = self.counts.get(kind, 0)
        self.counts[kind] = n + 1
        return "%s/%s" % (self.scope, kind if n == 0 else "%s_%d" % (kind, n))


def _block_ptr(t, image_offset):
    return t.ptr + image_offset * t.H * t.W * t.ld * 4


class HostInputStager:

    def __init__(self, program, depth=2):
        self.prog = program
        self.device = program.arch.device
        self.copy_stream = torch.cuda.Stream(device=self.device)
        self.depth = depth
        self.slots = [None] * depth
        self.ready = [None] * depth
        self.free = [None] * depth
        self.head = self.tail = self.count = 0

    def _like(self, slot, feats, labels):
        if self.slots[slot] is None:
            self.slots[slot] = ({k: torch.empty(v.shape, dtype=v.dtype, device=self.device) for k, v in feats.items()},
                                {k: torch.empty(v.shape, dtype=v.dtype, device=self.device) for k, v in (labels or {}).items()})
        return self.slots[slot]

    def stage(self, features, labels=None):
        assert self.count < self.depth, "every staging slot holds an unconsumed batch"
        slot = self.head
        df, dl = self._like(slot, features, labels)
        with torch.cuda.stream(self.copy_stream):
            if self.free[slot] is not None:
                self.copy_stream.wait_event(self.free[slot])
            for k, v in features.items():
                df[k].copy_(v, non_blocking=True)
            for k, v in (labels or {}).items():
                dl[k].copy_(v, non_blocking=True)
            ev = torch.cuda.Event()
            ev.record(self.copy_stream)
        self.ready[slot] = (ev, features, labels)
        self.head = (self.head + 1) % self.depth
        self.count += 1

    def consume(self):
        assert self.count > 0, "nothing staged"
        slot = self.tail
        ev = self.ready[slot][0]
        main = torch.cuda.current_stream(self.device)
        main.wait_event(ev)
        df, dl = self.slots[slot]
        self.prog.set_inputs(df, dl if dl else None)
        done = torch.cuda.Event()
        done.record(main)
        self.free[slot] = done
        self.tail = (self.tail + 1) % self.depth
        self.count -= 1


class Program:
    def __init__(self, arch, B, H, W, training_json=None):
        self.arch, self.B, self.H, self.W = arch, B, H, W
        self.training = training_json is not None
        self.training_json = training_json
        self.post_hidden = []
        self._invert_records = {}
        self._compose_scratch = []
        self._atable_ring = []
        S = arch.number_of_scales()
        if H % (1 << (len(arch.filters) - 1)) or W % (1 << (len(arch.filters) - 1)):
            raise ValueError("tile size %dx%d must be divisible by 2^(levels-1)" % (H, W))
        g = self.g = Graph(arch.device, arch.dtype, params=arch.params)
        g.training = self.training
        lib = self.lib = g.lib
        dev = arch.device
        tuples = arch.feature_prediction_tuples
        T, M = len(tuples), arch.tuple_size
        self.T, self.M, self.S = T, M, S
        self.head = [tuples[t].feature_predictions[j] for j in range(M) for t in range(T)]
        self.head_index = {f.name: i for i, f in enumerate(self.head)}
        NF, NA = len(self.head), len(arch.auxiliary_features)
        self.NF = NF
        all_feats = self.head + arch.auxiliary_features
        HW = H * W

        self.raw = {f.name: torch.zeros((B, H, W, f.number_of_channels), dtype=torch.float32, device=dev) for f in all_feats}
        nvs = [f.feature_variance.channels(f.number_of_channels) for f in all_feats]
        VL = 3 + max(nvs + [0])
        self.VL = VL
        fuse_input = os.environ.get("DD_FUSE_INPUT", "1") != "0"
        self.fused_input = fuse_input
        self.sources = torch.zeros(((NF if fuse_input else NF + NA) * B, H, W, VL), dtype=torch.float32, device=dev)
        if not fuse_input:
            for i, f in enumerate(all_feats):
                self._prepare_op(f, i, VL, self.sources)
        self.raw3 = None
        if arch.use_kernel_prediction and not arch.use_standardized_source_for_kernel_prediction:
            self.raw3 = torch.zeros((NF * B, H, W, 3), dtype=torch.float32, device=dev)
            for i, f in enumerate(self.head):
                self._prepare_op(f, i, 3, self.raw3, identity=True)

        emb = None
        if arch.feature_flag_mode == "EMBEDDING":
            V = len(arch.feature_flag_names)
            emb = g.params.get("embedding/feature_flags_embedding_matrix", (V, V // 2), V, V // 2)
        self.flags_raw = {}
        if arch.feature_flag_mode == "ONE_HOT_ENCODING":
            V = len(arch.feature_flag_names)
            self.flags_raw = {t.name: torch.zeros((B, H, W, V), dtype=torch.float32, device=dev) for t in tuples}
        cin = arch.input_channels()
        X = g.tensor(T * B, H, W, cin, requires_grad=(self.training and emb is not None))
        self.X = X
        n_entries = M + NA + (1 if arch.feature_flag_mode != "NONE" else 0)
        emb_ch0 = [0]

        def make_gather():
            tab = (L.GatherEntry * (T * n_entries))()
            for t, tup in enumerate(tuples):
                ch, e = 0, 0
                for j in range(M):
                    nch = 3 + nvs[j * T + t]
                    tab[t * n_entries + e] = L.GatherEntry(self.sources.data_ptr() + (j * T + t) * B * HW * VL * 4, VL, HW, nch, ch)
                    ch, e = ch + nch, e + 1
                for a in range(NA):
                    nch = 3 + nvs[NF + a]
                    tab[t * n_entries + e] = L.GatherEntry(self.sources.data_ptr() + (NF + a) * B * HW * VL * 4, VL, HW, nch, ch)
                    ch, e = ch + nch, e + 1
                if arch.feature_flag_mode == "ONE_HOT_ENCODING":
                    V = len(arch.feature_flag_names)
                    tab[t * n_entries + e] = L.GatherEntry(self.flags_raw[tup.name].data_ptr(), V, HW, V, ch)
                    ch += V
                elif emb is not None:
                    D = emb.shape[1]
                    row = arch.feature_flag_names.index(tup.name)
                    tab[t * n_entries + e] = L.GatherEntry(g.params.value_ptr(emb) + row * D * 4, 0, 0, D, ch)
                    emb_ch0[0] = ch
                    ch += D
                assert ch == cin, (ch, cin)
            table_dev = torch.frombuffer(bytearray(bytes(tab)), dtype=torch.uint8).to(dev)

            def gather(stream, table_dev=table_dev):
                L.check(lib.dd_gather_input(table_dev.data_ptr(), T, n_entries, X.ptr, X.ld, X.Cp, B, H, W, g.code, stream))
            return gather

        atable_dev = torch.zeros(T * n_entries * C.sizeof(L.AssembleEntry), dtype=torch.uint8, device=dev)

        self.frame_input = None
        self.frame_origins = None

        def build_assemble_table(frames=None):
            tab = (L.AssembleEntry * (T * n_entries))()
            for t, tup in enumerate(tuples):
                ch, e = 0, 0
                members = [(self.head[j * T + t], j * T + t) for j in range(M)] + [(f, None) for f in arch.auxiliary_features]
                for k, (f, head_i) in enumerate(members):
                    nv = nvs[head_i] if head_i is not None else nvs[NF + (k - M)]
                    en = tab[t * n_entries + e]
                    src = self.raw[f.name] if frames is None else frames[f.name]
                    en.src, en.cs, en.kind, en.fp = src.data_ptr(), f.number_of_channels, 0, self._feature_params(f)
                    en.nch, en.dst_ch = 3 + nv, ch
                    if head_i is not None:
                        en.std_out, en.ld_std = self.sources.data_ptr() + head_i * B * HW * VL * 4, VL
                    ch, e = ch + 3 + nv, e + 1
                if arch.feature_flag_mode == "ONE_HOT_ENCODING":
                    V = len(arch.feature_flag_names)
                    en = tab[t * n_entries + e]
                    en.src, en.kind, en.nch, en.dst_ch = self.flags_raw[tup.name].data_ptr(), 2, V, ch
                    ch += V
                elif emb is not None:
                    D = emb.shape[1]
                    row = arch.feature_flag_names.index(tup.name)
                    en = tab[t * n_entries + e]
                    en.src, en.kind, en.nch, en.dst_ch = g.params.value_ptr(emb) + row * D * 4, 1, D, ch
                    emb_ch0[0] = ch
                    ch += D
                assert ch == cin, (ch, cin)
            ring = self._atable_ring
            if not ring:
                for _ in range(4):
                    ring.append([torch.empty(atable_dev.numel(), dtype=torch.uint8, pin_memory=True), None])
            slot = ring.pop(0)
            ring.append(slot)
            if slot[1] is not None:
                slot[1].synchronize()
            slot[0].copy_(torch.frombuffer(bytearray(bytes(tab)), dtype=torch.uint8))
            atable_dev.copy_(slot[0], non_blocking=True)
            slot[1] = torch.cuda.Event()
            slot[1].record()

        self._build_assemble_table = build_assemble_table

        self._atable_sources = None

        def assemble(stream):
            if self.frame_input is not None:
                assert self._atable_sources == "frames", "enable_frame_input() without set_frame_sources()"
                L.check(lib.dd_assemble_input_frames(atable_dev.data_ptr(), T, n_entries, X.ptr, X.ld, X.Cp, B, H, W, g.code,
                                                     self.frame_origins.data_ptr(), self.frame_input[0], self.frame_input[1], stream))
                return
            if self._atable_sources != "tiles":
                build_assemble_table()
                self._atable_sources = "tiles"
            L.check(lib.dd_assemble_input(atable_dev.data_ptr(), T, n_entries, X.ptr, X.ld, X.Cp, B, H, W, g.code, stream))
        if fuse_input:
            g.fwd(assemble, "input_assembly")
        else:
            g.fwd(g._defer(make_gather, "input_assembly"))
        if X.requires_grad:
            def emb_backward():
                if not X.grad_written:
                    return
                gx = X.grad()
                D = emb.shape[1]
                esz = 4 if g.dtype == "f32" else 2

                rows_of = (C.c_int * T)(*[arch.feature_flag_names.index(tup.name) for tup in tuples])
                per16 = 16 // esz
                one_launch = (T <= 64 and D <= 8 * per16 and (emb_ch0[0] * esz) % 16 == 0 and gx.ld % per16 == 0
                              and emb_ch0[0] + -(-D // per16) * per16 <= gx.ld)

                def run(stream):
                    if one_launch:
                        L.check(lib.dd_colsum_segments(gx.ptr + emb_ch0[0] * esz, gx.ld, D, B * HW, T, g.params.grad_ptr(emb), D, rows_of,
                                                       g.code, stream))
                        return
                    for t, tup in enumerate(tuples):
                        row = arch.feature_flag_names.index(tup.name)
                        L.check(lib.dd_colsum(gx.ptr + (t * B * HW * gx.ld + emb_ch0[0]) * esz, gx.ld, D, B * HW,
                                              g.params.grad_ptr(emb) + row * D * 4, g.code, stream))
                g.bwd(run, "bias_grad", grad_params=[emb])
            g.on_backward(emb_backward)

        namer = _Namer("reused_core_architecture")
        if arch.core_name == "U-Net":
            outs = self._unet(X, namer)
        else:
            outs = self._tiramisu(X, namer)
        self.core_outputs = list(outs)
        post = []
        oc = arch.number_of_output_channels
        fuse_head = (arch.use_kernel_prediction and M == 1 and arch.kernel_size in (3, 5) and g.dtype != "f32"
                     and all(o.C % 8 == 0 and o.C <= 128 for o in outs) and os.environ.get("DD_FUSE_HEAD", "1") != "0")
        self.fused_head = fuse_head
        head_layers = []
        hidden = []
        for o in outs:
            la, lb = g.layer(namer("conv2d"), 1, o.C, oc), g.layer(namer("conv2d"), 1, oc, oc)
            head_layers.append((o, la, lb))
            if not fuse_head:
                hid = g.conv(o, la, relu=True)
                self.post_hidden.append(hid)
                hidden.append((hid, lb))
                post.append(g.conv(hid, lb, relu=False))
        if arch.use_multiscale_predictions:
            post, head_layers, hidden = list(reversed(post)), list(reversed(head_layers)), list(reversed(hidden))
        self.post = post
        self.fp32_logits = (not fuse_head and g.dtype != "f32" and arch.use_kernel_prediction and os.environ.get("DD_KPCN_FP32_LOGITS", "1") != "0")
        self._hidden = hidden

        N = NF * B
        dims = [(H >> s, W >> s) for s in range(len(head_layers))]
        K = [self._head_tensor(N, h, w) for (h, w) in dims]
        if arch.use_kernel_prediction:
            src0 = DT(self.sources if self.raw3 is None else self.raw3, N, H, W, 3, 3, 0, "f32")
            srcs = []
            for s, (h, w) in enumerate(dims):
                if s == 0:
                    src = src0
                else:
                    src = self._head_tensor(N, h, w, requires_grad=False)
                    g.fwd(self._avgpool_op(src0, src, 1 << s))
                srcs.append(src)
                if not fuse_head:
                    self._kpcn(src, post[s], K[s], hidden[s] if self.fp32_logits else None)
            if fuse_head:
                for s in reversed(range(len(dims))):
                    self._kpcn_head(head_layers[s], srcs[s], K[s])
        else:
            for s in range(len(post)):
                self._direct(post[s], K[s])
        P = list(K)
        if not arch.invert_standardization_after_multiscale_predictions:
            P = [self._invert(p) for p in P]
        if arch.use_multiscale_predictions:
            cnamer = None
            for s in range(len(P) - 1, 0, -1):
                cnamer = _Namer("reused_compose_scales")
                P[s - 1] = self._compose(P[s], P[s - 1], cnamer)
        if arch.invert_standardization_after_multiscale_predictions:
            P = [self._invert(p) for p in P]
        self.predictions = P
        self.dims = dims

        self.echo = {}
        for f in self.head:
            if not f.load_data:
                i = self.head_index[f.name]
                for s, (h, w) in enumerate(dims):
                    e = torch.zeros((B, h, w, 3), dtype=torch.float32, device=dev)
                    self.echo[(f.name, s)] = e
                    blk = self.sources[i * B:(i + 1) * B]
                    g.fwd(lambda stream, e=e, blk=blk, h=h, w=w: e.copy_(blk[:, :h, :w, :3]))

        self.loss_buf = torch.zeros(1, dtype=torch.float32, device=dev)
        self.label_ops, self.masked, self.mask_reduce = [], False, None
        ls = getattr(arch, "loss_scale", None)
        self.scaler = None
        if LS.is_dynamic(ls):
            if self.training:
                if getattr(arch, "loss_scaler", None) is None:
                    arch.loss_scaler = LS.LossScaler(LS.parse(ls, arch.dtype), dev, adam_t=getattr(arch, "adam_step", 0))
                self.scaler = arch.loss_scaler
            ls = None
        self.loss_scale = float(ls if ls is not None else (4096.0 if arch.dtype == "f16" else 1.0))
        if self.loss_scale <= 0.0:
            raise ValueError("loss_scale must be positive")
        self.step_count = 0
        self.grad_hook = None
        self._metric_state = None
        self._histogram_state = None
        self._preview_state = None
        self.write_histograms = False
        if self.training:
            self._build_loss(dims)
            g.build_backward()
            self._merge_head_backward()
        g.finalize(arch.seed)

    @property
    def loss_scale(self):
        return self.scaler.scale() if self.scaler is not None else self._loss_scale

    @loss_scale.setter
    def loss_scale(self, value):
        self._loss_scale = value

    @staticmethod
    def _feature_params(f, identity=False):
        fp = L.FeatureParams()
        st, fv = f.feature_standardization, f.feature_variance
        if identity:
            fp.use_log1p, fp.mean, fp.inv_std, fp.use_variance = 0, 0.0, 1.0, 0
        else:
            fp.use_log1p, fp.mean = int(st.use_log1p), st.mean
            fp.inv_std = 1.0 / math.sqrt(st.variance) if st.variance != 1.0 else 1.0
            fp.use_variance = int(fv.use_variance)
        fp.variance_before = int(fv.compute_before_standardization)
        fp.mode_neighbor = int(fv.variance_mode == "neighbor")
        fp.relative, fp.compress, fp.epsilon = int(fv.relative_variance), int(fv.compress_to_one_channel), 1e-4
        return fp

    def _prepare_op(self, f, index, ldd, dst, identity=False):
        g, lib, B, H, W = self.g, self.lib, self.B, self.H, self.W
        fp = self._feature_params(f, identity)
        raw = self.raw[f.name]
        ptr = dst.data_ptr() + index * B * H * W * ldd * 4
        cs = f.number_of_channels

        def run(stream, fp=fp):
            L.check(lib.dd_prepare_feature(raw.data_ptr(), cs, ptr, ldd, C.byref(fp), B, H, W, stream))
        g.fwd(run, "input_assembly")

    def _head_tensor(self, N, h, w, requires_grad=True):
        buf = torch.zeros((N, h, w, 3), dtype=torch.float32, device=self.arch.device)
        return DT(buf, N, h, w, 3, 3, 0, "f32", False, requires_grad)

    def _avgpool_op(self, x, y, f):
        lib = self.lib

        def run(stream):
            L.check(lib.dd_avgpool(x.ptr, x.ld, y.ptr, y.ld, 3, x.B, x.H, x.W, f, stream))
        return run

    def _unet(self, x, namer):
        g, arch = self.g, self.arch
        filters, n = arch.filters, arch.convs_per_block
        steps = len(filters) - 1
        for f in filters:
            if f % 8:
                raise ValueError("U-Net filter counts must be multiples of 8 (got %s)" % (filters,))
        cats, results = [], []

        def conv_run(x, f, count, last_out=None, first_split=None):
            layers = []
            for c in range(count):
                layers.append(g.layer(namer("conv2d"), 3, x.C if c == 0 else f, f))
            c = 0
            while c < count:
                out = last_out if c == count - 1 else None
                split = first_split if c == 0 else None
                x = g.conv(x, layers[c], relu=True, out=out, split_at=split)
                c += 1
            return x

        for i in range(steps):
            f = filters[i]
            cat = g.tensor(x.B, x.H, x.W, 2 * f, relu=True)
            x = conv_run(x, f, n, last_out=cat.view(0, f))
            cats.append(cat)
            x = g.maxpool(x, 3, 2)
        for i in range(steps):
            index = steps - i
            f = filters[index]
            x = conv_run(x, f, n, first_split=f if i > 0 else None)
            if arch.use_multiscale_predictions:
                results.append(x)
            cat, fp = cats[index - 1], filters[index - 1]
            g.conv_transpose2(x, g.layer(namer("conv2d_transpose"), 2, x.C, fp, "convT2"), out=cat.view(fp, fp), relu=True)
            x = cat
        x = conv_run(x, filters[0], n, first_split=filters[0])
        results.append(x)
        return results

    def _tiramisu(self, x, namer):
        g, arch = self.g, self.arch
        filters, n = arch.filters, arch.convs_per_block
        steps = len(filters) - 1
        for f in filters:
            if f % 8:
                raise ValueError("Tiramisu filter counts must be multiples of 8 (got %s)" % (filters,))
        c_in = [0] * (steps + 1)
        c_down = [0] * (steps + 1)
        c = filters[0]
        for i in range(steps + 1):
            c_in[i] = c
            c = c + n * filters[i]
            c_down[i] = c
        total = [0] * (steps + 1)
        total[steps] = c_down[steps]
        for i in range(steps):
            total[i] = c_down[i] + filters[i] + n * filters[i]
        bufs = [g.tensor(x.B, x.H >> i, x.W >> i, total[i], relu=False) for i in range(steps + 1)]
        for b in bufs:
            b.gstate["zero_init"] = True

        def dense(buf, c0, f):
            return g.dense_block(buf, c0, f, [g.layer(namer("conv2d"), 3, c0 + j * f, f) for j in range(n)])

        pre = bufs[0].view(0, filters[0], relu=False)
        pre.self_mask = True
        g.conv(x, g.layer(namer("conv2d"), 3, x.C, filters[0]), relu=True, out=pre)
        pre.relu = False
        results = []
        for i in range(steps):
            cc = dense(bufs[i], c_in[i], filters[i])
            assert cc == c_down[i]
            t = g.conv(bufs[i].view(0, cc), g.layer(namer("conv2d"), 1, cc, cc), relu=False, in_relu=True)
            g.maxpool(t, 2, 2, out=bufs[i + 1].view(0, cc, relu=False))
        cc = dense(bufs[steps], c_in[steps], filters[steps])
        cur = bufs[steps].view(0, cc)
        for i in range(steps):
            index = steps - i
            if arch.use_multiscale_predictions:
                results.append(cur)
            lvl = index - 1
            fp = filters[lvl]
            up = bufs[lvl].view(c_down[lvl], fp, relu=False)
            up.self_mask = True
            g.conv_transpose3(cur, g.layer(namer("conv2d_transpose"), 3, cur.C, fp, "convT3"), out=up, relu=True)
            up.relu = False
            cc = dense(bufs[lvl], c_down[lvl] + fp, fp)
            cur = bufs[lvl].view(0, cc)
        results.append(cur)
        return results

    def _kpcn(self, src, logits, out, hidden=None):
        g, lib, arch = self.g, self.lib, self.arch
        k2, ks = arch.kernel_size ** 2, arch.kernel_size
        TB, M = self.T * self.B, self.M
        esz = 4 if g.dtype == "f32" else 2
        h, w = out.H, out.W
        hid, lb = hidden if hidden is not None else (None, None)

        def hidden_args(j):
            return (hid.ptr, hid.ld, hid.C, g.params.value_ptr(lb.kernel) + 4 * j * k2, lb.cout, g.params.value_ptr(lb.bias) + 4 * j * k2)

        def run(stream):
            for j in range(M):
                if hid is not None:
                    L.check(lib.dd_kpcn_hidden_fwd(_block_ptr(src, j * TB), src.ld, *hidden_args(j), _block_ptr(out, j * TB), out.ld, TB, h, w, ks, g.code, stream))
                    continue
                L.check(lib.dd_kpcn_fwd(_block_ptr(src, j * TB), src.ld, logits.ptr + j * k2 * esz, logits.ld,
                                        _block_ptr(out, j * TB), out.ld, TB, h, w, ks, g.code, stream))
        g.fwd(run, "kpcn_apply")

        def backward():
            if not out.grad_written:
                return
            go, gl = out.grad(), logits.grad()

            def runb(stream):
                for j in range(M):
                    pad = (logits.Cp - j * k2) if j == M - 1 else k2
                    if hid is not None:
                        L.check(lib.dd_kpcn_hidden_bwd(_block_ptr(src, j * TB), src.ld, *hidden_args(j), _block_ptr(go, j * TB), go.ld,
                                                       gl.ptr + j * k2 * esz, gl.ld, pad, TB, h, w, ks, g.code, stream))
                        continue
                    L.check(lib.dd_kpcn_bwd(_block_ptr(src, j * TB), src.ld, logits.ptr + j * k2 * esz, logits.ld,
                                            _block_ptr(go, j * TB), go.ld, gl.ptr + j * k2 * esz, gl.ld, pad, TB, h, w, ks, g.code, stream))
            g.bwd(runb, "kpcn_apply")
            logits.mark_grad_written()
        g.on_backward(backward)

    def _kpcn_head(self, head, src, out):
        g, lib = self.g, self.lib
        x, la, lb = head
        assert x.B == out.B and (x.H, x.W) == (out.H, out.W)

        def make():
            ha = L.HeadArgs()
            self._head_args(ha, head, src, out)

            def run(stream, ha=ha):
                L.check(lib.dd_kpcn_head_fwd(C.byref(ha), stream))
            return run
        g.fwd(g._defer(make, "kpcn_head", keep=(x.buf, src.buf, out.buf)))

        def backward():
            if not (out.grad_written and x.requires_grad):
                return
            go, gx = out.grad(), x.grad()
            desc = (head, src, out, go, gx, 1 if x.grad_written else 0)

            def makeb():
                hb = L.HeadArgs()
                self._head_args(hb, *desc)

                def runb(stream, hb=hb):
                    L.check(lib.dd_kpcn_head_bwd(C.byref(hb), stream))
                return runb
            g.bwd(g._defer(makeb, "kpcn_head", keep=(go.buf, gx.buf), head_bwd=desc), grad_params=[la.kernel, la.bias, lb.kernel, lb.bias])
            x.mark_grad_written()
        g.on_backward(backward)

    def _head_args(self, h, head, src, out, go=None, gx=None, accumulate=0):
        ps = self.g.params
        x, la, lb = head
        h.x, h.ldx, h.C, h.src, h.ldsrc = x.ptr, x.ld, x.C, src.ptr, src.ld
        h.wa, h.ba, h.wb, h.bb = ps.value_ptr(la.kernel), ps.value_ptr(la.bias), ps.value_ptr(lb.kernel), ps.value_ptr(lb.bias)
        h.out, h.ld_out = out.ptr, out.ld
        h.N, h.H, h.W, h.ksize, h.dtype = x.B, x.H, x.W, self.arch.kernel_size, self.g.code
        if go is not None:
            h.dout, h.ld_dout, h.dx, h.ld_dx, h.accumulate_dx = go.ptr, go.ld, gx.ptr, gx.ld, accumulate
            h.dwa, h.dba, h.dwb, h.dbb = ps.grad_ptr(la.kernel), ps.grad_ptr(la.bias), ps.grad_ptr(lb.kernel), ps.grad_ptr(lb.bias)

    def _merge_head_backward(self):
        g, lib = self.g, self.lib
        if os.environ.get("DD_HEAD_BWD_MULTI", "1") == "0":
            return
        ops, out, i = g.bwd_ops, [], 0
        while i < len(ops):
            j = i
            while j < len(ops) and getattr(ops[j], "head_bwd", None) is not None and j - i < 3:
                j += 1
            if j - i < 2:
                out.append(ops[i])
                i += 1
                continue
            members = ops[i:j]

            def make(descs=[op.head_bwd for op in members]):
                arr = (L.HeadArgs * len(descs))()
                for h, desc in zip(arr, descs):
                    self._head_args(h, *desc)

                def run(stream, arr=arr, n=len(descs)):
                    L.check(lib.dd_kpcn_head_bwd_multi(arr, n, stream))
                return run
            out.append(g._defer(make, "kpcn_head", grad_params=tuple(p_ for op in members for p_ in op.grad_params),
                                keep=[getattr(op, "keep", None) for op in members]))
            i = j
        g.bwd_ops = out

    def _direct(self, logits, out):
        g, lib = self.g, self.lib
        TB, M = self.T * self.B, self.M
        esz = 4 if g.dtype == "f32" else 2
        npix = TB * out.H * out.W

        def run(stream):
            for j in range(M):
                L.check(lib.dd_convert_channels(logits.ptr + j * 3 * esz, g.code, logits.ld, _block_ptr(out, j * TB), L.DD_F32, 3, 3, 3, npix, stream))
        g.fwd(run)

        def backward():
            if not out.grad_written:
                return
            go, gl = out.grad(), logits.grad()

            def runb(stream):
                for j in range(M):
                    pad = (logits.Cp - j * 3) if j == M - 1 else 3
                    L.check(lib.dd_convert_channels(_block_ptr(go, j * TB), L.DD_F32, 3, gl.ptr + j * 3 * esz, g.code, gl.ld, 3, pad, npix, stream))
            g.bwd(runb)
            logits.mark_grad_written()
        g.on_backward(backward)

    def _invert(self, x):
        g, lib, B = self.g, self.lib, self.B
        groups = []
        for i, f in enumerate(self.head):
            st = f.feature_standardization
            key = (st.use_log1p, st.mean, st.variance) if f.invert_standardization else (False, 0.0, 1.0)
            if groups and groups[-1][0] == key:
                groups[-1][2] += 1
            else:
                groups.append([key, i, 1])
        if all(k[0] == (False, 0.0, 1.0) for k in groups):
            return x
        y = self._head_tensor(x.B, x.H, x.W)
        per = B * x.H * x.W * 3

        def run(stream):
            for (log1p, mean, var), i0, cnt in groups:
                L.check(lib.dd_invert_std_fwd(_block_ptr(x, i0 * B), _block_ptr(y, i0 * B), per * cnt, int(log1p), mean, math.sqrt(var), stream))
        g.fwd(run)

        def backward():
            if not y.grad_written:
                return
            gy, gx = y.grad(), x.grad()
            assert not x.grad_written, "invert-standardization is expected to be the first gradient writer"

            def runb(stream):
                for (log1p, mean, var), i0, cnt in groups:
                    L.check(lib.dd_invert_std_bwd(_block_ptr(x, i0 * B), _block_ptr(gy, i0 * B), _block_ptr(gx, i0 * B), per * cnt,
                                                  int(log1p), mean, math.sqrt(var), stream))
            g.bwd(runb)
            x.mark_grad_written()
        g.on_backward(backward)
        self._invert_records[id(y)] = {"x": x, "groups": groups, "fwd": run, "tape": backward}
        return y

    def _compose(self, small, fine, namer):
        g, lib = self.g, self.lib
        N, h, w = fine.B, fine.H, fine.W
        netin = g.tensor(N, h, w, 6, requires_grad=self.training)
        n_fwd0, n_tape0 = len(g.fwd_ops), len(g._tape)

        def pack(stream):
            L.check(lib.dd_compose_pack(small.ptr, small.ld, fine.ptr, fine.ld, netin.ptr, netin.ld, netin.Cp, N, h, w, g.code, stream))
        g.fwd(pack)

        def pack_backward():
            if not netin.grad_written:
                return
            gn, gs, gf = netin.grad(), small.grad(), fine.grad()

            def runb(stream):
                L.check(lib.dd_compose_unpack_bwd(gn.ptr, gn.ld, gs.ptr, gs.ld, gf.ptr, gf.ld, N, h, w, g.code, stream))
            g.bwd(runb)
        g.on_backward(pack_backward)

        lay_in = g.layer(namer("conv2d"), 1, 6, 24)
        x = g.conv(netin, lay_in, relu=True)
        acts, lay_res = [x], []
        for _ in range(2):
            lay_res.append(g.layer(namer("conv2d"), 3, 24, 24))
            r = g.conv(x, lay_res[-1], relu=False, in_relu=True)
            lay_res.append(g.layer(namer("conv2d"), 3, 24, 24))
            x = g.conv(r, lay_res[-1], relu=False, in_relu=True, res=x)
            acts += [r, x]
        lay_out = g.layer(namer("conv2d"), 1, 24, 1)
        wl = g.conv(x, lay_out, relu=True)
        out = self._head_tensor(N, h, w)

        def blend(stream):
            L.check(lib.dd_compose_blend_fwd(small.ptr, small.ld, fine.ptr, fine.ld, wl.ptr, wl.ld, out.ptr, out.ld, N, h, w, g.code, stream))
        g.fwd(blend)

        def blend_backward():
            if not out.grad_written:
                return
            go, gs, gf, gw = out.grad(), small.grad(), fine.grad(), wl.grad()
            acc_small = 1 if small.grad_written else 0
            assert not fine.grad_written

            def runb(stream):
                L.check(lib.dd_compose_blend_bwd(go.ptr, go.ld, small.ptr, small.ld, fine.ptr, fine.ld, wl.ptr, wl.ld,
                                                 gs.ptr, gs.ld, acc_small, gf.ptr, gf.ld, gw.ptr, gw.ld, gw.Cp, N, h, w, g.code, stream))
            g.bwd(runb)
            small.mark_grad_written()
            fine.mark_grad_written()
            wl.mark_grad_written()
        g.on_backward(blend_backward)

        if g.dtype != "f32" and os.environ.get("DD_FUSE_COMPOSE", "1") != "0":
            del g.fwd_ops[n_fwd0:]
            ps, save = g.params, self.training
            fused_bwd = self.training and os.environ.get("DD_FUSE_COMPOSE_BWD", "1") != "0"

            def make_fused():
                ca = L.ComposeArgs()
                ca.small, ca.ld_small, ca.fine, ca.ld_fine, ca.out, ca.ld_out = small.ptr, small.ld, fine.ptr, fine.ld, out.ptr, out.ld
                ca.w_in, ca.b_in = ps.value_ptr(lay_in.kernel), ps.value_ptr(lay_in.bias)
                for i, lay in enumerate(lay_res):
                    ca.w_res[i], ca.b_res[i] = ps.value_ptr(lay.kernel), ps.value_ptr(lay.bias)
                ca.w_out, ca.b_out = ps.value_ptr(lay_out.kernel), ps.value_ptr(lay_out.bias)
                if save:
                    if not fused_bwd:
                        ca.save_netin, ca.ld_netin = netin.ptr, netin.ld
                    for i, t in enumerate(acts):
                        ca.save_act[i], ca.ld_act[i] = t.ptr, t.ld
                    ca.save_wl, ca.ld_wl = wl.ptr, wl.ld
                ca.N, ca.H, ca.W, ca.dtype = N, h, w, g.code

                def fused(stream, ca=ca):
                    L.check(lib.dd_compose_net_fwd(C.byref(ca), stream))
                return fused
            g.fwd(g._defer(make_fused, "compose_net", keep=(small.buf, fine.buf, out.buf, netin.buf, wl.buf, [t.buf for t in acts])))

            if fused_bwd:
                del g._tape[n_tape0:]
                layers = [lay_in] + lay_res + [lay_out]

                def fused_backward():
                    if not out.grad_written:
                        return
                    go, gs, gf = out.grad(), small.grad(), fine.grad()
                    acc_small = 1 if small.grad_written else 0
                    assert not fine.grad_written
                    cb = L.ComposeBwdArgs()
                    cb.small, cb.ld_small, cb.fine, cb.ld_fine, cb.dout, cb.ld_dout = small.ptr, small.ld, fine.ptr, fine.ld, go.ptr, go.ld
                    for i, t in enumerate(acts):
                        cb.act[i], cb.ld_act[i] = t.ptr, t.ld
                    cb.wl, cb.ld_wl = wl.ptr, wl.ld
                    cb.d_small, cb.ld_dsmall, cb.accumulate_small, cb.d_fine, cb.ld_dfine = gs.ptr, gs.ld, acc_small, gf.ptr, gf.ld
                    cb.N, cb.H, cb.W, cb.dtype = N, h, w, g.code
                    if os.environ.get("DD_COMPOSE_STREAM_BWD", "1") != "0":
                        need = int(lib.dd_compose_bwd_scratch_bytes(N, h, w))
                        pool = self._compose_scratch
                        if not pool or pool[-1].numel() < need:
                            pool.append(torch.empty(need, dtype=torch.uint8, device=self.arch.device))
                        cb.scratch, cb.scratch_bytes = pool[-1].data_ptr(), pool[-1].numel()

                    def make_fused_bwd():
                        cb.w_in, cb.w_out = ps.value_ptr(lay_in.kernel), ps.value_ptr(lay_out.kernel)
                        cb.dw_in, cb.db_in = ps.grad_ptr(lay_in.kernel), ps.grad_ptr(lay_in.bias)
                        cb.dw_out, cb.db_out = ps.grad_ptr(lay_out.kernel), ps.grad_ptr(lay_out.bias)
                        for i, lay in enumerate(lay_res):
                            cb.w_res[i], cb.dw_res[i], cb.db_res[i] = ps.value_ptr(lay.kernel), ps.grad_ptr(lay.kernel), ps.grad_ptr(lay.bias)

                        def runb(stream, cb=cb):
                            L.check(lib.dd_compose_net_bwd(C.byref(cb), stream))
                        return runb
                    g.bwd(g._defer(make_fused_bwd, "compose_net", keep=(go.buf, gs.buf, gf.buf)),
                          grad_params=[p_ for lay in layers for p_ in (lay.kernel, lay.bias)])
                    small.mark_grad_written()
                    fine.mark_grad_written()
                g.on_backward(fused_backward)
        return out

    def _build_loss(self, dims):
        arch, tj, g, lib, B = self.arch, self.training_json, self.g, self.lib, self.B
        dev = arch.device
        N = self.NF * B
        ms_loss = bool(tj["use_multiscale_loss"])
        n_scales = len(dims) if (ms_loss or tj["use_multiscale_metrics"]) else 1
        self.targets = [torch.zeros((N, h, w, 3), dtype=torch.float32, device=dev) for (h, w) in dims[:n_scales]]
        t0 = DT(self.targets[0], N, dims[0][0], dims[0][1], 3, 3, 0, "f32")
        for s in range(1, n_scales):
            op = self._avgpool_op(t0, DT(self.targets[s], N, dims[s][0], dims[s][1], 3, 3, 0, "f32"), 1 << s)
            op.tag = "pointwise"
            self.label_ops.append(op)

        def w3(j):
            return float(j["mean"]), float(j["variation"]), float(j["ms_ssim"])
        fs, cf, ci = tj["features_training_settings"], tj["combined_features_training_settings"], tj["combined_image_training_settings"]
        def wm(j):
            if j and j["ms_ssim"] > 0:
                raise NotImplementedError("the masked ms_ssim loss term cannot run: the reference raises 'Not implemented' there too "
                                          "(BaseFeatureTraining.masked_ms_ssim, Training.py:206-207)")
            if j and j["variation"] > 0:
                raise NotImplementedError("the masked variation loss term is out of scope (weight 0 in TrainingExample.json)")
            return float(j["mean"]) if j else 0.0
        m_feat, m_comb = wm(fs.get("loss_weights_masked")), wm(cf.get("loss_weights_masked"))

        def mask_pass(name):
            if RenderPasses.is_color_render_pass(name) or name in ("Environment", "Emission", "Volume Direct", "Volume Indirect"):
                return name
            if RenderPasses.is_direct_or_indirect_render_pass(name):
                return RenderPasses.direct_or_indirect_to_color_render_pass(name)
            return None
        (w_feat, v_feat, q_feat), (w_comb, v_comb, q_comb), (w_img, v_img, q_img) = w3(fs["loss_weights"]), w3(cf["loss_weights"]), w3(ci["loss_weights"])
        use_image = w_img > 0 or v_img > 0 or q_img > 0 or ci["statistics"]["track_mean"]
        use_comb = (use_image or w_comb > 0 or v_comb > 0 or q_comb > 0 or cf["statistics"]["track_mean"]
                    or cf.get("statistics_masked", {}).get("track_mean", False))
        loss_scales = len(dims) if ms_loss else 1
        norm = 1.0 / sum(1.0 / 4.0 ** s for s in range(loss_scales))
        dummy = self._dummy_dpred = [torch.zeros((B, h, w, 3), dtype=torch.float32, device=dev) for (h, w) in dims]
        self.loss_descs = []
        self.mask_sums = torch.zeros(loss_scales * (L.MAX_FEATURES + L.MAX_COMBINED), dtype=torch.float32, device=dev)
        n_triples = sum(all(n in self.head_index for n in names) for _, names in self._combined_triples()) if use_comb else 0
        ms_ssim = (q_feat > 0 and any(f.load_data for f in self.head)) or (q_comb > 0 and n_triples > 0) or q_img > 0
        if ms_ssim:
            self._check_ms_ssim(dims[0], q_feat)
        fuse_invert = (arch.invert_standardization_after_multiscale_predictions and v_feat == 0 and v_comb == 0 and v_img == 0 and not ms_ssim
                       and os.environ.get("DD_FUSE_LOSS_INVERT", "1") != "0")
        for s in range(loss_scales):
            h, w = dims[s]
            P = self.predictions[s]
            rec = self._invert_records.get(id(P)) if fuse_invert else None
            if rec is not None:
                assert not rec["x"].grad_written, "invert-standardization is expected to be the first gradient writer"
                g.fwd_ops.remove(rec["fwd"])
                g._tape.remove(rec["tape"])
                gP = rec["x"].grad()
            else:
                gP = P.grad()
            d = L.LossDesc()
            d.n_features = self.NF
            d.kind, d.epsilon = _LOSS_KIND[tj["loss_difference"]], 1e-2
            sf = norm / 4.0 ** s
            for i, f in enumerate(self.head):
                d.target[i] = self.targets[s].data_ptr() + i * B * h * w * 3 * 4
                d.target_ld[i] = 3
                d.nch[i] = f.number_of_channels
                if f.load_data:
                    d.pred[i], d.pred_ld[i] = _block_ptr(P, i * B), 3
                    d.dpred[i] = _block_ptr(gP, i * B)
                    if rec is not None:
                        (log1p, mean, var) = [k for k, i0, cnt in rec["groups"] if i0 <= i < i0 + cnt][0]
                        d.pred_std[i], d.pred_inv[i] = _block_ptr(rec["x"], i * B), _block_ptr(P, i * B)
                        d.inv_log1p[i], d.inv_mean[i], d.inv_std[i] = int(log1p), mean, math.sqrt(var)
                    d.weight[i], d.var_weight[i] = w_feat * sf, v_feat * sf
                    d.masked_weight[i], d.mask_feature[i] = 0.0, -1
                    if m_feat > 0:
                        if f.name == "Alpha":
                            raise Exception("Masking is not supported for the alpha pass, because it does not seem to make sense.")
                        cp = mask_pass(f.name)
                        if cp is not None:
                            d.masked_weight[i], d.mask_feature[i] = m_feat * sf, self.head_index[cp]
                else:
                    d.pred[i], d.pred_ld[i] = self.echo[(f.name, s)].data_ptr(), 3
                    d.dpred[i] = dummy[s].data_ptr()
                    d.weight[i], d.var_weight[i] = 0.0, 0.0
                    d.masked_weight[i], d.mask_feature[i] = 0.0, -1
            ncomb = 0
            comb_names = {}
            if use_comb:
                for tup_name, names in self._combined_triples():
                    if not all(n in self.head_index for n in names):
                        continue
                    for c in range(3):
                        d.comb[ncomb][c] = self.head_index[names[c]]
                    d.comb_weight[ncomb], d.comb_var_weight[ncomb] = w_comb * sf, v_comb * sf
                    d.comb_masked_weight[ncomb], d.comb_mask_feature[ncomb] = 0.0, -1
                    if m_comb > 0:
                        d.comb_masked_weight[ncomb] = m_comb * sf
                        d.comb_mask_feature[ncomb] = self.head_index[RenderPasses.combined_to_color_render_pass(tup_name)]
                    comb_names[tup_name] = ncomb
                    ncomb += 1
            d.n_combined = ncomb
            d.n_image_combined = d.n_image_features = 0
            d.image_weight = d.image_var_weight = 0.0
            if use_image:
                for n in ("Diffuse", "Glossy", "Subsurface", "Transmission"):
                    d.image_combined[d.n_image_combined] = comb_names[n]
                    d.n_image_combined += 1
                for n in ("Volume Direct", "Volume Indirect", "Emission", "Environment"):
                    d.image_features[d.n_image_features] = self.head_index[n]
                    d.n_image_features += 1
                d.image_weight, d.image_var_weight = w_img * sf, v_img * sf
            masked = any(d.masked_weight[i] != 0.0 for i in range(self.NF)) or any(d.comb_masked_weight[k] != 0.0 for k in range(ncomb))
            nm = L.MAX_FEATURES + L.MAX_COMBINED
            msums = self.mask_sums[s * nm:(s + 1) * nm] if masked else None
            d.mask_sums = msums.data_ptr() if masked else None
            self.loss_descs.append((d, msums))
            if masked:
                self.masked = True

                def count(stream, d=d, h=h, w=w, msums=msums):
                    L.check(lib.dd_loss_mask_sums(C.byref(d), B, h, w, msums.data_ptr(), stream))
                count.tag = "loss_head"
                self.label_ops.append(count)

            if self.scaler is not None:
                def run(stream, d=d, h=h, w=w):
                    L.check(lib.dd_loss_head_dscale(C.byref(d), B, h, w, self.loss_buf.data_ptr(), self.scaler.ptr, stream))
            else:
                def run(stream, d=d, h=h, w=w):
                    L.check(lib.dd_loss_head(C.byref(d), B, h, w, self.loss_buf.data_ptr(), self.loss_scale, stream))
            g.fwd(run, "loss_head")
            (rec["x"] if rec is not None else P).mark_grad_written()
            if s == 0 and ms_ssim:
                if w_feat == 0 and not any(gP.buf is t for t in g.zero_init_buffers):
                    g.zero_init_buffers.append(gP.buf)
                self._build_ms_ssim(d, gP, dims[0], q_feat, q_comb, q_img)

    def _check_ms_ssim(self, dim, q_feat):
        h, w = dim
        if h % 4 or w % 4 or min(h, w) < 44:
            raise ValueError("the ms_ssim loss term needs tiles whose height and width are multiples of 4 and at least 44 (got %d x %d): "
                             "tf.image.ssim_multiscale refuses a level smaller than its 11 x 11 filter (3 levels: side / 4 >= 11), and "
                             "levels of odd size would need its symmetric pad before the 2x2 pool, which is not built" % (h, w))
        if q_feat > 0:
            for f in self.head:
                if f.load_data and f.number_of_channels != 3:
                    raise ValueError("a features-level ms_ssim weight cannot be used with the loaded 1-channel target pass '%s': the reference "
                                     "transposes such a tensor into an image 1 pixel high (Training.py:187-190) and cannot build either" % f.name)

    def _build_ms_ssim(self, d, gP, dim, q_feat, q_comb, q_img):
        g, lib, B = self.g, self.lib, self.B
        h, w = dim
        m = L.MsSsimDesc()
        m.n_features = d.n_features
        n_sources = 0
        for i, f in enumerate(self.head):
            m.pred[i], m.target[i], m.pred_ld[i], m.target_ld[i], m.nch[i] = d.pred[i], d.target[i], d.pred_ld[i], d.target_ld[i], d.nch[i]
            m.dpred[i] = _block_ptr(gP, i * B) if f.load_data else None
            m.ssim_weight[i] = q_feat if f.load_data else 0.0
            n_sources += m.ssim_weight[i] > 0
        m.n_combined = d.n_combined
        for k in range(d.n_combined):
            for c in range(3):
                m.comb[k][c] = d.comb[k][c]
            m.comb_ssim_weight[k] = q_comb
            n_sources += q_comb > 0
        m.n_image_combined, m.n_image_features = d.n_image_combined, d.n_image_features
        for k in range(d.n_image_combined):
            m.image_combined[k] = d.image_combined[k]
        for k in range(d.n_image_features):
            m.image_features[k] = d.image_features[k]
        m.image_ssim_weight = q_img
        n_sources += q_img > 0
        if n_sources == 0:
            return
        nbytes = lib.dd_loss_msssim_scratch_bytes(B, h, w, n_sources)
        if nbytes < 0:
            L.check(int(nbytes))
        scratch = torch.zeros(nbytes // 4, dtype=torch.float32, device=self.arch.device)
        self.ms_ssim_desc = (m, scratch)

        def run(stream, m=m, h=h, w=w, scratch=scratch):
            L.check(lib.dd_loss_msssim_fwd(C.byref(m), B, h, w, scratch.data_ptr(), self.loss_buf.data_ptr(), stream))
        g.fwd(run, "loss_head")

        def backward():
            if self.scaler is not None:
                def runb(stream, m=m, h=h, w=w, scratch=scratch):
                    L.check(lib.dd_loss_msssim_bwd_dscale(C.byref(m), B, h, w, scratch.data_ptr(), self.scaler.ptr, stream))
            else:
                def runb(stream, m=m, h=h, w=w, scratch=scratch):
                    L.check(lib.dd_loss_msssim_bwd(C.byref(m), B, h, w, scratch.data_ptr(), self.loss_scale, stream))
            g.bwd(runb, "loss_head")
        g.on_backward(backward)

    def _combined_triples(self):
        arch = self.arch
        out = []
        if arch.feature_prediction_tuple_type == "COMBINED":
            for tup in arch.feature_prediction_tuples:
                out.append((tup.name, [f.name for f in tup.feature_predictions]))
        else:
            for cname, names in arch.combined_feature_names:
                out.append((cname, names))
        return out

    def set_inputs(self, features, labels=None, non_blocking=False):
        if self.frame_input is not None:
            self.disable_frame_input()
        for f in self.head + self.arch.auxiliary_features:
            self.raw[f.name].copy_(features[Naming.source_feature_name(f.name, index=0)], non_blocking=non_blocking)
        for name, buf in self.flags_raw.items():
            key = Naming.feature_flags_name(name)
            if key in features:
                buf.copy_(features[key], non_blocking=non_blocking)
            else:
                buf.zero_()
                buf[..., self.arch.feature_flag_names.index(name)] = 1.0
        if labels is not None:
            B = self.B
            for i, f in enumerate(self.head):
                self.targets[0][i * B:(i + 1) * B, :, :, :f.number_of_channels].copy_(labels[Naming.target_feature_name(f.name)],
                                                                                      non_blocking=non_blocking)

    def enable_frame_input(self, frame_h, frame_w):
        if not self.fused_input:
            raise RuntimeError("frame input needs the fused input assembly (DD_FUSE_INPUT=0 is set)")
        if self.frame_origins is None:
            self.frame_origins = torch.zeros((self.B, 2), dtype=torch.int32, device=self.arch.device)
        self.frame_input = (int(frame_h), int(frame_w))

    def set_frame_sources(self, frames):
        fh, fw = self.frame_input
        for f in self.head + self.arch.auxiliary_features:
            t = frames[f.name]
            if tuple(t.shape) != (fh, fw, f.number_of_channels) or t.dtype != torch.float32 or not t.is_contiguous():
                raise ValueError("%s: expected a contiguous float32 [%d,%d,%d] frame, got %s" % (f.name, fh, fw, f.number_of_channels, tuple(t.shape)))
        ptrs = tuple(frames[f.name].data_ptr() for f in self.head + self.arch.auxiliary_features)
        if self._atable_sources == "frames" and ptrs == self.__dict__.get("_frame_ptrs"):
            return
        self._build_assemble_table(frames)
        self._atable_sources, self._frame_ptrs = "frames", ptrs

    def disable_frame_input(self):
        self.frame_input = None
        if self._atable_sources != "tiles":
            self._build_assemble_table()
            self._atable_sources = "tiles"

    def host_stager(self, depth=2):
        return HostInputStager(self, depth)

    def pack_weights(self):
        self.g.run(self.g.pack_ops)

    def run_label_ops(self):
        self.g.run(self.label_ops)
        if self.masked and self.mask_reduce is not None:
            self.mask_reduce(self.mask_sums)

    def forward(self, pack=True, labels=True):
        if pack:
            self.pack_weights()
        if labels and self.label_ops:
            self.run_label_ops()
        self.g.run(self.g.fwd_ops)

    def backward(self):
        self.g.run(self.g.bwd_ops)

    def zero_grads(self):
        self.arch.params.grads.zero_()
        self.loss_buf.zero_()
        for t in self.g.zero_init_buffers:
            t.zero_()

    def adam(self, learning_rate=None, grad_scale=1.0, beta1=0.9, beta2=0.999, eps=1e-8):
        ps = self.arch.params
        lr = self.training_json["learning_rate"] if learning_rate is None else learning_rate
        if self.scaler is not None:
            ps.raw_writes = getattr(ps, "raw_writes", 0) + 1
            self.scaler.step(ps, lr, grad_scale, beta1, beta2, eps, self.g.stream_ptr())
            return
        if self.arch.dtype == "f16" and not bool(torch.isfinite(ps.grads).all()):
            self.skipped_steps = getattr(self, "skipped_steps", 0) + 1
            import warnings
            warnings.warn("fp16 gradients overflowed at loss_scale=%g: optimizer step skipped (%d so far)" % (self.loss_scale, self.skipped_steps))
            return
        self.arch.adam_step = getattr(self.arch, "adam_step", 0) + 1
        t = self.arch.adam_step
        lr_t = lr * math.sqrt(1.0 - beta2 ** t) / (1.0 - beta1 ** t)
        ps.raw_writes = getattr(ps, "raw_writes", 0) + 1
        L.check(self.lib.dd_adam_step(ps.values.data_ptr(), ps.grads.data_ptr(), ps.m.data_ptr(), ps.v.data_ptr(), ps.values.numel(),
                                      lr_t, beta1, beta2, eps, grad_scale / self.loss_scale, self.g.stream_ptr()))

    def sync_adam_step(self):
        if self.scaler is None:
            return None
        st = self.scaler.state()
        self.arch.adam_step = st["adam_t"]
        return st

    def train_step(self, features=None, labels=None):
        if features is not None:
            self.set_inputs(features, labels)
        self.zero_grads()
        self.forward(pack=True)
        self.backward()
        grad_scale = 1.0
        if self.grad_hook is not None:
            grad_scale = self.grad_hook(self.arch.params.grads)
        self.adam(grad_scale=grad_scale)
        return self.loss_buf

    def profile_ops(self, repeats=3, detail=False):
        g = self.g
        ops = list(g.pack_ops) + list(self.label_ops) + list(g.fwd_ops) + list(g.bwd_ops)
        samples = [[] for _ in ops]
        for rep_i in range(repeats + 1):
            self.zero_grads()
            evs = []
            s = g.stream_ptr()
            for op in ops:
                e0, e1 = torch.cuda.Event(enable_timing=True), torch.cuda.Event(enable_timing=True)
                e0.record()
                op(s)
                e1.record()
                evs.append((e0, e1))
            torch.cuda.synchronize()
            if rep_i == 0:
                continue
            for i, (e0, e1) in enumerate(evs):
                samples[i].append(e0.elapsed_time(e1))
        per_op, acc = [], {}
        for op, v in zip(ops, samples):
            v = sorted(v)
            ms = v[len(v) // 2] if len(v) % 2 else 0.5 * (v[len(v) // 2 - 1] + v[len(v) // 2])
            per_op.append(1e3 * ms)
            tag = getattr(op, "tag", "pointwise")
            n, tot = acc.get(tag, (0, 0.0))
            acc[tag] = (n + 1, tot + ms)
        flops = {}
        for op in ops:
            info = getattr(op, "info", None)
            if info and "flops" in info:
                tag = getattr(op, "tag", "pointwise")
                flops[tag] = flops.get(tag, 0.0) + info["flops"]
        out = {tag: (n, ms, flops.get(tag, 0.0)) for tag, (n, ms) in acc.items()}
        if detail:
            return out, [(getattr(op, "tag", "pointwise"), getattr(op, "info", None), us) for op, us in zip(ops, per_op)]
        return out

    def metric_plan(self):
        return self._metrics_built()["plan"]

    def _metric_sources(self, d, s, triples, use_image):
        B = self.B
        h, w = self.dims[s]
        d.n_features = self.NF
        for i, f in enumerate(self.head):
            d.target[i], d.target_ld[i], d.nch[i] = self.targets[s].data_ptr() + i * B * h * w * 3 * 4, 3, f.number_of_channels
            d.pred[i] = _block_ptr(self.predictions[s], i * B) if f.load_data else self.echo[(f.name, s)].data_ptr()
            d.pred_ld[i] = self.predictions[s].ld if f.load_data else 3
        d.n_combined = len(triples)
        for k, (_, names) in enumerate(triples):
            for c in range(3):
                d.comb[k][c] = self.head_index[names[c]]
        d.n_image_combined = d.n_image_features = 0
        if use_image:
            cidx = {c: k for k, (c, _) in enumerate(triples)}
            for n in ("Diffuse", "Glossy", "Subsurface", "Transmission"):
                d.image_combined[d.n_image_combined] = cidx[n]
                d.n_image_combined += 1
            for n in ("Volume Direct", "Volume Indirect", "Emission", "Environment"):
                d.image_features[d.n_image_features] = self.head_index[n]
                d.n_image_features += 1

    def _metrics_built(self):
        if self._metric_state is not None:
            return self._metric_state
        if not self.training:
            raise RuntimeError("metrics() needs a training program (built with a Training.json): there are no targets otherwise")
        from . import metrics as M
        arch, tj, lib, B, dev = self.arch, self.training_json, self.lib, self.B, self.arch.device
        plan = M.metric_plan(arch, tj, histograms=self.write_histograms)
        scales = sorted({e.scale_index for e in plan if e.quantity != "ms_ssim"})
        assert all(k < len(self.targets) for k in scales), "scaled targets exist whenever use_multiscale_metrics is set"
        use_image, use_comb = M.combined_levels(tj)
        triples = M.combined_triples(arch) if use_comb else []
        slot_of = {("feature", f.name): i for i, f in enumerate(self.head)}
        slot_of.update({("combined", c): L.MAX_FEATURES + k for k, (c, _) in enumerate(triples)})
        slot_of[("image", M.IMAGE_NAME)] = L.MAX_FEATURES + L.MAX_COMBINED
        masked_feat = any(e.quantity == "masked_mean" and e.source[0] == "feature" for e in plan)
        masked_comb = any(e.quantity == "masked_mean" and e.source[0] == "combined" for e in plan)

        def sources(d, s, h, w):
            self._metric_sources(d, s, triples, use_image)

        rows = L.METRIC_SOURCES * B * 4
        ms_sources = [e.source for e in plan if e.quantity == "ms_ssim"]
        table = torch.zeros(len(scales) * rows + len(ms_sources) * B, dtype=torch.float32, device=dev)
        launches, keep = [], []
        for j, s in enumerate(scales):
            h, w = self.dims[s]
            d = L.LossDesc()
            sources(d, s, h, w)
            d.kind, d.epsilon = _LOSS_KIND[tj["loss_difference"]], 1e-2
            for i, f in enumerate(self.head):
                cp = M.mask_pass(f.name) if (masked_feat and f.load_data) else None
                d.mask_feature[i] = self.head_index[cp] if cp is not None else -1
            for k, (cname, _) in enumerate(triples):
                d.comb_mask_feature[k] = self.head_index[RenderPasses.combined_to_color_render_pass(cname)] if masked_comb else -1
            nbytes = lib.dd_loss_metrics_scratch_bytes(B, h, w)
            if nbytes < 0:
                L.check(int(nbytes))
            scratch = torch.zeros(nbytes // 4, dtype=torch.float32, device=dev)
            out = table[j * rows:(j + 1) * rows]
            keep.append((d, scratch))

            def run(stream, d=d, h=h, w=w, scratch=scratch, out=out):
                L.check(lib.dd_loss_metrics(C.byref(d), B, h, w, scratch.data_ptr(), out.data_ptr(), stream))
            launches.append(run)
        if ms_sources:
            h, w = self.dims[0]
            self._check_ms_ssim((h, w), 1.0 if any(src[0] == "feature" for src in ms_sources) else 0.0)
            ld = L.LossDesc()
            sources(ld, 0, h, w)
            m = L.MsSsimDesc()
            m.n_features, m.n_combined = ld.n_features, ld.n_combined
            m.n_image_combined, m.n_image_features = ld.n_image_combined, ld.n_image_features
            for i, f in enumerate(self.head):
                m.pred[i], m.target[i], m.pred_ld[i], m.target_ld[i], m.nch[i] = ld.pred[i], ld.target[i], ld.pred_ld[i], 3, ld.nch[i]
                m.dpred[i] = None
                m.ssim_weight[i] = 1.0 if ("feature", f.name) in ms_sources else 0.0
            for k, (cname, _) in enumerate(triples):
                for c in range(3):
                    m.comb[k][c] = ld.comb[k][c]
                m.comb_ssim_weight[k] = 1.0 if ("combined", cname) in ms_sources else 0.0
            for k in range(ld.n_image_combined):
                m.image_combined[k] = ld.image_combined[k]
            for k in range(ld.n_image_features):
                m.image_features[k] = ld.image_features[k]
            m.image_ssim_weight = 1.0 if ("image", M.IMAGE_NAME) in ms_sources else 0.0
            order = ([("feature", f.name) for f in self.head if ("feature", f.name) in ms_sources]
                     + [("combined", c) for c, _ in triples if ("combined", c) in ms_sources]
                     + [src for src in ms_sources if src[0] == "image"])
            nbytes = lib.dd_loss_msssim_scratch_bytes(B, h, w, len(order))
            if nbytes < 0:
                L.check(int(nbytes))
            scratch = torch.zeros(nbytes // 4, dtype=torch.float32, device=dev)
            out = table[len(scales) * rows:]
            keep.append((m, scratch))

            def run_ms(stream, m=m, h=h, w=w, scratch=scratch, out=out):
                L.check(lib.dd_loss_msssim_values(C.byref(m), B, h, w, scratch.data_ptr(), out.data_ptr(), stream))
            launches.append(run_ms)
            ms_sources = order
        self._metric_state = {"plan": plan, "scales": scales, "slot_of": slot_of, "table": table, "launches": launches, "keep": keep,
                              "rows": rows, "ms_sources": ms_sources}
        return self._metric_state

    def metric_table(self):
        st = self._metrics_built()
        self.g.run(st["launches"])
        return st["table"]

    def metric_values(self, table, real=None, count=None):
        from . import metrics as M
        st = self._metrics_built()
        if not st["plan"]:
            return []
        host = table.detach().cpu().numpy() if torch.is_tensor(table) else table
        n = len(st["scales"])
        images = host.size // (n * L.METRIC_SOURCES * 4 + len(st["ms_sources"]))
        rows = L.METRIC_SOURCES * images * 4
        assert host.size == n * rows + len(st["ms_sources"]) * images, "not a metric table of this program"
        tables = {s: host[j * rows:(j + 1) * rows].reshape(L.METRIC_SOURCES, images, 4) for j, s in enumerate(st["scales"])}
        ms = host[n * rows:].reshape(len(st["ms_sources"]), -1) if st["ms_sources"] else None
        ms_values = {src: ms[j] for j, src in enumerate(st["ms_sources"])}
        return M.metric_values(st["plan"], st["slot_of"], tables, self.dims, real, ms_values, count)

    def metrics(self, real=None):
        return self.metric_values(self.metric_table(), real)

    def histogram_plan(self):
        return self._histograms_built()["plan"]

    def _histograms_built(self):
        if self._histogram_state is not None:
            return self._histogram_state
        if not self.training:
            raise RuntimeError("histograms() needs a training program (built with a Training.json): there are no targets otherwise")
        from . import metrics as M
        arch, tj, lib, B, dev = self.arch, self.training_json, self.lib, self.B, self.arch.device
        plan = M.histogram_plan(arch, tj)
        scales = sorted({e.scale_index for e in plan})
        assert all(k < len(self.targets) for k in scales), "scaled targets exist whenever use_multiscale_metrics is set"
        use_image, use_comb = M.combined_levels(tj)
        triples = M.combined_triples(arch) if use_comb else []
        slot_of = {("feature", f.name): i for i, f in enumerate(self.head)}
        slot_of.update({("combined", c): L.MAX_FEATURES + k for k, (c, _) in enumerate(triples)})
        slot_of[("image", M.IMAGE_NAME)] = L.MAX_FEATURES + L.MAX_COMBINED
        limits_host = M.histogram_limits()
        nb = len(limits_host)
        rec_bytes = L.histogram_record_bytes(nb)
        limits = torch.from_numpy(limits_host).to(dev)
        records = torch.zeros(max(len(plan), 1) * rec_bytes, dtype=torch.uint8, device=dev)
        order, launches, keep = [], [], [limits]
        for s in scales:
            h, w = self.dims[s]
            entries = [i for i, e in enumerate(plan) if e.scale_index == s]
            d = L.LossDesc()
            self._metric_sources(d, s, triples, use_image)
            d.kind, d.epsilon = _LOSS_KIND[tj["loss_difference"]], 1e-2
            for i, f in enumerate(self.head):
                cp = M.mask_pass(f.name) if f.load_data else None
                d.mask_feature[i] = self.head_index.get(cp, -1) if cp is not None else -1
            for k, (cname, _) in enumerate(triples):
                d.comb_mask_feature[k] = self.head_index.get(RenderPasses.combined_to_color_render_pass(cname), -1)
            sel = (C.c_int * (2 * len(entries)))()
            for r, i in enumerate(entries):
                sel[2 * r], sel[2 * r + 1] = slot_of[plan[i].source], M.HISTOGRAM_KINDS.index(plan[i].kind)
            nbytes = lib.dd_loss_histograms_scratch_bytes(B, h, w, len(entries))
            if nbytes < 0:
                L.check(int(nbytes))
            scratch = torch.zeros(nbytes // 8, dtype=torch.float64, device=dev)
            out = records[len(order) * rec_bytes:(len(order) + len(entries)) * rec_bytes]
            order += entries
            keep.append((d, sel, scratch))

            def run(stream, d=d, h=h, w=w, sel=sel, n=len(entries), scratch=scratch, out=out):
                L.check(lib.dd_loss_histograms(C.byref(d), B, h, w, sel, n, limits.data_ptr(), nb, out.data_ptr(), scratch.data_ptr(), stream))
            launches.append(run)
        self._histogram_state = {"plan": plan, "order": order, "records": records, "launches": launches, "keep": keep, "nb": nb,
                                 "limits": limits_host}
        return self._histogram_state

    def histogram_table(self):
        st = self._histograms_built()
        self.g.run(st["launches"])
        return st["records"]

    def histogram_host_table(self, records=None):
        from . import metrics as M
        st = self._histograms_built()
        records = self.histogram_table() if records is None else records
        host = records.detach().cpu().numpy() if torch.is_tensor(records) else records
        n = len(st["plan"])
        table = M.decode_histogram_records(host[:n * L.histogram_record_bytes(st["nb"])], n, st["nb"])
        back = [0] * n
        for r, i in enumerate(st["order"]):
            back[i] = r
        return {k: v[back] for k, v in table.items()}

    def histograms(self, out=print):
        from . import metrics as M
        st = self._histograms_built()
        if not st["plan"]:
            return []
        return M.histogram_values(st["plan"], self.histogram_host_table(), st["limits"], out=out)

    def _previews_built(self):
        if self._preview_state is not None:
            return self._preview_state
        if not self.training:
            raise RuntimeError("previews() needs a training program (built with a Training.json): there are no targets otherwise")
        from . import metrics as M
        arch, tj, dev = self.arch, self.training_json, self.arch.device
        triples = M.combined_triples(arch)
        d = L.LossDesc()
        self._metric_sources(d, 0, triples, M.image_members(arch) is not None)
        d.kind, d.epsilon = _LOSS_KIND[tj["loss_difference"]], 1e-2
        source, source_ld = (C.c_void_p * L.MAX_FEATURES)(), (C.c_int * L.MAX_FEATURES)()
        for i, f in enumerate(self.head):
            source[i], source_ld[i] = self.raw[f.name].data_ptr(), f.number_of_channels
        slot_of = {("feature", f.name): i for i, f in enumerate(self.head)}
        slot_of.update({("combined", c): L.MAX_FEATURES + k for k, (c, _) in enumerate(triples)})
        slot_of[("image", M.IMAGE_NAME)] = L.MAX_FEATURES + L.MAX_COMBINED
        thresholds = torch.from_numpy(M.preview_thresholds()).to(dev)
        self._preview_state = {"desc": d, "source": source, "source_ld": source_ld, "slot_of": slot_of, "thresholds": thresholds, "out": {},
                               "plans": {w: M.preview_plan(arch, tj, w) for w in ("combined", "all")}}
        return self._preview_state

    def preview_plan(self, which="combined"):
        st = self._previews_built()
        if which not in st["plans"]:
            raise ValueError("previews: which = %r ('combined' or 'all')" % (which,))
        return st["plans"][which]

    def preview_table(self, images=(0, 1, 2), which="combined", panels=("source", "prediction", "target"), exposure=1.0, error_gain=1.0):
        from . import metrics as M
        st = self._previews_built()
        plan, mask = self.preview_plan(which), M.preview_panel_mask(panels)
        images = [int(b) for b in images]
        if not plan:
            raise ValueError("previews: the architecture has no source to show")
        P = bin(mask).count("1")
        shape = (len(plan), len(images) * self.H, P * self.W, 3)
        if shape not in st["out"]:
            st["out"][shape] = torch.zeros(shape, dtype=torch.uint8, device=self.arch.device)
        out = st["out"][shape]
        img = (C.c_int * max(len(images), 1))(*images)
        slots = (C.c_int * len(plan))(*[st["slot_of"][e.source] for e in plan])

        def run(stream):
            L.check(self.lib.dd_loss_previews(C.byref(st["desc"]), st["source"], st["source_ld"], self.B, self.H, self.W, img, len(images), slots, len(plan),
                                              mask, st["thresholds"].data_ptr(), float(exposure), float(error_gain), out.data_ptr(), stream))
        self.g.run([run])
        return out

    def preview_images(self, table, images, which="combined"):
        from . import metrics as M
        host = table.detach().cpu().numpy() if torch.is_tensor(table) else np.asarray(table)
        plan, n = self.preview_plan(which), len(images)
        assert host.shape[0] == len(plan) and host.shape[1] == n * self.H, "not a preview table of this plan"
        return [(tag, host[j, k * self.H:(k + 1) * self.H]) for j, e in enumerate(plan) for k, tag in enumerate(M.preview_tags(e.name, n))]

    def previews(self, images=(0, 1, 2), which="combined", panels=("source", "prediction", "target"), exposure=1.0, error_gain=1.0):
        images = list(images)
        return self.preview_images(self.preview_table(images, which, panels, exposure, error_gain), images, which)

    def prediction_dictionaries(self):
        B = self.B
        out = []
        for s, P in enumerate(self.predictions):
            d = {}
            for f in self.arch.feature_predictions:
                if not f.is_target:
                    continue
                i = self.head_index[f.name]
                if f.load_data:
                    p = P.buf[i * B:(i + 1) * B]
                else:
                    p = self.echo[(f.name, s)]
                d[Naming.feature_prediction_name(f.name)] = p[..., :f.number_of_channels]
            out.append(d)
        return out
```

### include/dd_hip.h

```cpp
#ifndef DD_HIP_H
#define DD_HIP_H

#include <stddef.h>
#include <stdint.h>

#ifdef __cplusplus
extern "C" {
#endif

typedef void* dd_stream;

enum dd_dtype { DD_F32 = 0, DD_BF16 = 1, DD_F16 = 2 };

enum dd_status {
  DD_OK = 0,
  DD_ERR_INVALID = -1,
  DD_ERR_LAUNCH = -2
};

enum dd_conv_flags {
  DD_IN_RELU = 1,
  DD_OUT_RELU = 2,
  DD_ACCUM = 4,
  DD_PIXSHUF = 8,
  DD_GATHER2X2 = 16
};

const char* dd_version(void);
const char* dd_last_error(void);

int dd_pack_weights(const float* src, void* dst, int dtype, int taps, int n, int k, int n_pad, int k_pad,
                    long s_tap, long s_n, long s_k, int tap_flip, dd_stream stream);

typedef struct { const float* src; void* dst; int taps, n, k, n_pad, k_pad, tap_flip; long s_tap, s_n, s_k; long dst_ld, dst_tap_stride; } dd_pack_desc;
int dd_pack_weights_batched(const dd_pack_desc* table, int n_layers, int dtype, dd_stream stream);

typedef struct {
  const void* x; int ldx; int cin;
  const void* wp; int k_pad; int n_pad;
  const float* bias; int nbias;
  const void* res; int ldres;
  const void* mask; int ldmask;
  void* y; int ldy; int n;
  int B, H, W;
  int taps; int flags; int dtype;
} dd_conv_args;
int dd_conv_igemm(const dd_conv_args* a, dd_stream stream);
long dd_conv_pw_count(void);
long dd_wgrad_pw_count(void);

typedef struct {
  const void* p; int ldp; int m;
  const void* q; int ldq; int n;
  float* out;
  float* bias_out; int bias_mode;
  int B, H, W;
  int taps; int flags; int dtype;
  int ksplit;
  int stack_blocks; int stack_width; int stack_m0;
  float* stack_out[8]; float* stack_bias[8];
} dd_wgrad_args;
int dd_conv_wgrad(const dd_wgrad_args* a, dd_stream stream);

typedef struct {
  const void* dy; int ld_dy; int cout;
  const void* x; int ld_x; int cin;
  const void* wd; int n_pad; int k_pad;
  void* dx; int ld_dx;
  float* dw; float* db;
  int B, H, W;
  int use_mask; int accumulate; int dtype;
} dd_conv_bwd_args;
int dd_conv3x3_bwd(const dd_conv_bwd_args* a, dd_stream stream);
int dd_conv3x3_bwd_multi(const dd_conv_bwd_args* a, int n, dd_stream stream);

typedef struct {
  const void* x; int ld_x; int cin;
  void* y; int ld_y; int cout;
  const void* w; int n_pad; int k_pad;
  const float* bias; int relu;
  void* dx; int ld_dx; float* dw; float* db; int use_mask; int accumulate;
  int B, H, W;
  int dtype;
} dd_convt_args;
int dd_convt2x2_fwd(const dd_convt_args* a, dd_stream stream);
int dd_convt2x2_bwd(const dd_convt_args* a, dd_stream stream);

typedef struct {
  const void* x; int ldx; int cin;
  const void* wp; int n_pad; int k_pad;
  const float* bias; int nbias;
  void* y; int ldy;
  int n0; int n;
  int B, H, W;
  int mode; int flags; int dtype;
  const void* mask; int ldmask;
} dd_conv_ks_args;
int dd_conv3x3_ks(const dd_conv_ks_args* a, dd_stream stream);

int dd_colsum(const void* x, int ld, int c, long rows, float* out, int dtype, dd_stream stream);
int dd_colsum_segments(const void* x, int ld, int c, long rows_per_segment, int n_segments, float* out, int out_ld, const int* out_row,
                       int dtype, dd_stream stream);

int dd_maxpool_fwd(const void* x, int ldx, void* y, int ldy, uint8_t* idx, int C, int B, int H, int W,
                   int pool, int stride, int relu_mask, int dtype, dd_stream stream);
int dd_maxpool_bwd(const void* dy, int lddy, const uint8_t* idx, void* dx, int lddx, const void* mask, int ldmask,
                   int C, int B, int H, int W, int pool, int stride, int accumulate, int dtype, dd_stream stream);

int dd_avgpool(const float* x, int ldx, float* y, int ldy, int C, int B, int H, int W, int f, dd_stream stream);

typedef struct {
  int use_log1p; float mean; float inv_std;
  int use_variance; int variance_before; int mode_neighbor; int relative; int compress; float epsilon;
} dd_feature_params;
int dd_prepare_feature(const float* src, int cs, float* dst, int ldd, const dd_feature_params* fp, int B, int H, int W, dd_stream stream);

typedef struct { const float* src; int pixel_stride; int batch_stride_pixels; int nch; int dst_ch; } dd_gather_entry;
int dd_gather_input(const dd_gather_entry* table, int n_tuples, int n_entries, void* dst, int ld, int c_pad,
                    int B, int H, int W, int dtype, dd_stream stream);

typedef struct { const float* src; int cs; int kind; dd_feature_params fp; int nch; int dst_ch; float* std_out; int ld_std; } dd_assemble_entry;
int dd_assemble_input(const dd_assemble_entry* table, int n_tuples, int n_entries, void* dst, int ld, int c_pad,
                      int B, int H, int W, int dtype, dd_stream stream);
int dd_assemble_input_frames(const dd_assemble_entry* table, int n_tuples, int n_entries, void* dst, int ld, int c_pad,
                             int B, int H, int W, int dtype, const int* origins_yx, int frame_h, int frame_w, dd_stream stream);

int dd_kpcn_fwd(const float* src, int ldsrc, const void* logits, int ldl, float* out, int ldo,
                int B, int H, int W, int ksize, int dtype, dd_stream stream);
int dd_kpcn_bwd(const float* src, int ldsrc, const void* logits, int ldl, const float* dout, int lddo,
                void* dlogits, int lddl, int dl_pad, int B, int H, int W, int ksize, int dtype, dd_stream stream);
int dd_kpcn_hidden_fwd(const float* src, int ldsrc, const void* hid, int ldh, int kh, const float* wb, int ldw, const float* bb,
                       float* out, int ldo, int B, int H, int W, int ksize, int dtype, dd_stream stream);
int dd_kpcn_hidden_bwd(const float* src, int ldsrc, const void* hid, int ldh, int kh, const float* wb, int ldw, const float* bb,
                       const float* dout, int lddo, void* dlogits, int lddl, int dl_pad, int B, int H, int W, int ksize, int dtype, dd_stream stream);

typedef struct {
  const void* x; int ldx; int C;
  const float* src; int ldsrc;
  const float* wa; const float* ba; const float* wb; const float* bb;
  float* out; int ld_out;
  const float* dout; int ld_dout;
  void* dx; int ld_dx; int accumulate_dx;
  float* dwa; float* dba; float* dwb; float* dbb;
  int N, H, W, ksize, dtype;
} dd_head_args;
int dd_kpcn_head_fwd(const dd_head_args* a, dd_stream stream);
int dd_kpcn_head_bwd(const dd_head_args* a, dd_stream stream);
int dd_kpcn_head_bwd_multi(const dd_head_args* a, int n, dd_stream stream);

int dd_compose_pack(const float* small, int lds, const float* fine, int ldf, void* dst, int ld, int c_pad,
                    int B, int H, int W, int dtype, dd_stream stream);
int dd_compose_blend_fwd(const float* small, int lds, const float* fine, int ldf, const void* wl, int ldw,
                         float* out, int ldo, int B, int H, int W, int dtype, dd_stream stream);
int dd_compose_blend_bwd(const float* dout, int lddo, const float* small, int lds, const float* fine, int ldf,
                         const void* wl, int ldw, float* dsmall, int ldds, int accumulate_small, float* dfine, int lddf,
                         void* dwl, int lddw, int dw_pad, int B, int H, int W, int dtype, dd_stream stream);
int dd_compose_unpack_bwd(const void* dnet, int ld, float* dsmall, int ldds, float* dfine, int lddf,
                          int B, int H, int W, int dtype, dd_stream stream);

typedef struct {
  const float* small; int ld_small;
  const float* fine; int ld_fine;
  float* out; int ld_out;
  const float* w_in; const float* b_in;
  const float* w_res[4]; const float* b_res[4];
  const float* w_out; const float* b_out;
  void* save_netin; int ld_netin;
  void* save_act[5]; int ld_act[5];
  void* save_wl; int ld_wl;
  int N, H, W, dtype;
} dd_compose_args;
int dd_compose_net_fwd(const dd_compose_args* a, dd_stream stream);
int dd_compose_stream_plan(int N, int H, int W, int cus, int* out8);

typedef struct {
  const float* small; int ld_small;
  const float* fine; int ld_fine;
  const float* dout; int ld_dout;
  const void* act[5]; int ld_act[5];
  const void* wl; int ld_wl;
  const float* w_in; const float* w_res[4]; const float* w_out;
  float* d_small; int ld_dsmall; int accumulate_small;
  float* d_fine; int ld_dfine;
  float* dw_in; float* db_in; float* dw_res[4]; float* db_res[4]; float* dw_out; float* db_out;
  int N, H, W, dtype;
  void* scratch; long scratch_bytes;
} dd_compose_bwd_args;
int dd_compose_net_bwd(const dd_compose_bwd_args* a, dd_stream stream);
long dd_compose_bwd_scratch_bytes(int N, int H, int W);

int dd_invert_std_fwd(const float* x, float* y, long n, int use_log1p, float mean, float std, dd_stream stream);
int dd_invert_std_bwd(const float* x, const float* dy, float* dx, long n, int use_log1p, float mean, float std, dd_stream stream);

#define DD_MAX_FEATURES 32
#define DD_MAX_COMBINED 8
typedef struct {
  int n_features;
  const float* pred[DD_MAX_FEATURES];
  const float* target[DD_MAX_FEATURES];
  float* dpred[DD_MAX_FEATURES];
  int target_ld[DD_MAX_FEATURES];
  int pred_ld[DD_MAX_FEATURES];
  int nch[DD_MAX_FEATURES];
  float weight[DD_MAX_FEATURES];
  float var_weight[DD_MAX_FEATURES];
  float masked_weight[DD_MAX_FEATURES];
  int mask_feature[DD_MAX_FEATURES];
  int n_combined;
  int comb[DD_MAX_COMBINED][3];
  float comb_weight[DD_MAX_COMBINED];
  float comb_var_weight[DD_MAX_COMBINED];
  float comb_masked_weight[DD_MAX_COMBINED];
  int comb_mask_feature[DD_MAX_COMBINED];
  int n_image_combined; int image_combined[DD_MAX_COMBINED];
  int n_image_features; int image_features[DD_MAX_FEATURES];
  float image_weight;
  float image_var_weight;
  int kind;
  float epsilon;
  const float* mask_sums;
  const float* pred_std[DD_MAX_FEATURES];
  float* pred_inv[DD_MAX_FEATURES];
  int inv_log1p[DD_MAX_FEATURES];
  float inv_mean[DD_MAX_FEATURES];
  float inv_std[DD_MAX_FEATURES];
} dd_loss_desc;
int dd_loss_mask_sums(const dd_loss_desc* desc, int B, int H, int W, float* mask_sums, dd_stream stream);
int dd_loss_head(const dd_loss_desc* desc, int B, int H, int W, float* loss_out, float grad_scale, dd_stream stream);
int dd_loss_head_dscale(const dd_loss_desc* desc, int B, int H, int W, float* loss_out, const float* grad_scale_dev, dd_stream stream);
long dd_loss_head_path_count(int path);

typedef struct {
  int n_features;
  const float* pred[DD_MAX_FEATURES];
  const float* target[DD_MAX_FEATURES];
  float* dpred[DD_MAX_FEATURES];
  int target_ld[DD_MAX_FEATURES];
  int pred_ld[DD_MAX_FEATURES];
  int nch[DD_MAX_FEATURES];
  float ssim_weight[DD_MAX_FEATURES];
  int n_combined;
  int comb[DD_MAX_COMBINED][3];
  float comb_ssim_weight[DD_MAX_COMBINED];
  int n_image_combined; int image_combined[DD_MAX_COMBINED];
  int n_image_features; int image_features[DD_MAX_FEATURES];
  float image_ssim_weight;
} dd_loss_msssim_desc;
long dd_loss_msssim_scratch_bytes(int B, int H, int W, int n_sources);
int dd_loss_msssim_fwd(const dd_loss_msssim_desc* desc, int B, int H, int W, float* scratch, float* loss_out, dd_stream stream);
int dd_loss_msssim_bwd(const dd_loss_msssim_desc* desc, int B, int H, int W, float* scratch, float grad_scale, dd_stream stream);
int dd_loss_msssim_bwd_dscale(const dd_loss_msssim_desc* desc, int B, int H, int W, float* scratch, const float* grad_scale_dev, dd_stream stream);
int dd_loss_msssim_values(const dd_loss_msssim_desc* desc, int B, int H, int W, float* scratch, float* ms_out, dd_stream stream);

#define DD_METRIC_SOURCES (DD_MAX_FEATURES + DD_MAX_COMBINED + 1)
long dd_loss_metrics_scratch_bytes(int B, int H, int W);
int dd_loss_metrics(const dd_loss_desc* desc, int B, int H, int W, float* scratch, float* table, dd_stream stream);

#define DD_HISTOGRAM_MAX_BUCKETS 4096
#define DD_HISTOGRAM_STATS_OFFSET(nb) ((((long)(nb) + 1) / 2) * 8)
#define DD_HISTOGRAM_RECORD_BYTES(nb) (DD_HISTOGRAM_STATS_OFFSET(nb) + 48)
#define DD_HISTOGRAM_VALUES_SCRATCH_BYTES 20480
#define DD_HISTOGRAM_MAX_CHUNKS 32
int dd_histogram_values(const float* values, long n, const double* limits, int nb, void* record, void* scratch, dd_stream stream);
#define DD_HISTOGRAM_DIFFERENCE 0
#define DD_HISTOGRAM_VARIATION_DIFFERENCE 1
#define DD_HISTOGRAM_MASKED_DIFFERENCE 2
long dd_loss_histograms_scratch_bytes(int B, int H, int W, int n_records);
int dd_loss_histograms(const dd_loss_desc* desc, int B, int H, int W, const int* selection, int n_records, const double* limits, int nb,
                       void* records, void* scratch, dd_stream stream);

#define DD_PREVIEW_MAX_IMAGES 16
#define DD_PREVIEW_THRESHOLDS 255
#define DD_PREVIEW_SOURCE 1
#define DD_PREVIEW_PREDICTION 2
#define DD_PREVIEW_TARGET 4
#define DD_PREVIEW_DIFFERENCE 8
int dd_loss_previews(const dd_loss_desc* desc, const float* const* source, const int* source_ld, int B, int H, int W, const int* images, int n_images,
                     const int* slots, int n_slots, int panels, const float* thresholds, float exposure, float error_gain, unsigned char* out,
                     dd_stream stream);

int dd_adam_step(float* params, const float* grads, float* m, float* v, long n, float lr_t, float beta1, float beta2,
                 float eps, float grad_scale, dd_stream stream);

typedef struct {
  float scale;
  int good_steps;
  int found_nonfinite;
  int adam_t;
  int skipped_total;
} dd_scaler_state;
int dd_grads_nonfinite(const float* grads, long n, dd_scaler_state* st, dd_stream stream);
int dd_adam_step_scaled(float* params, const float* grads, float* m, float* v, long n, double lr, double beta1, double beta2,
                        float eps, float grad_scale, const dd_scaler_state* st, dd_stream stream);
int dd_scaler_update(dd_scaler_state* st, float growth, float backoff, int growth_interval, float min_scale, float max_scale, dd_stream stream);

typedef struct { int tile; int crop_y0, crop_y1, crop_x0, crop_x1; int dst_img, dst_y, dst_x; } dd_stitch_entry;
int dd_stitch(const float* tiles, int tile_size, int ldt, float* frames, int frame_h, int frame_w, int ldf, int C,
              const dd_stitch_entry* table, int n_entries, dd_stream stream);

int dd_extract_tiles(const float* frame, int frame_h, int frame_w, int ldf, int C, float* tiles, int tile_size, int ldt,
                     const int* origins_yx, int n_tiles, dd_stream stream);

typedef struct {
  int n_triples; const float* color[4]; const float* direct[4]; const float* indirect[4]; float* combined[4];
  int n_singles; const float* single[8];
  float* image;
} dd_recombine_desc;
int dd_recombine(const dd_recombine_desc* desc, long npix, dd_stream stream);

#define DD_NONFINITE_MAX_PLANES 32
typedef struct { float* data; int C; int ld; unsigned char* mask; } dd_nonfinite_plane;
typedef struct { int n_planes; dd_nonfinite_plane plane[DD_NONFINITE_MAX_PLANES]; } dd_nonfinite_desc;
int dd_nonfinite_scan(const dd_nonfinite_desc* desc, int N, int H, int W, uint64_t* counts, dd_stream stream);
int dd_nonfinite_repair(const dd_nonfinite_desc* desc, int N, int H, int W, int radius, const uint64_t* counts, dd_stream stream);

int dd_masked_add(void* dst, int lddst, const void* src, int ldsrc, const void* mask, int ldmask, int C, long npix,
                  int accumulate, int dtype, dd_stream stream);
int dd_convert_channels(const void* src, int src_dtype, int ldsrc, void* dst, int dst_dtype, int lddst, int nch, int dst_pad,
                        long npix, dd_stream stream);
typedef struct { int flip; int rotate; int permute; float normal_rotation[9]; } dd_augment_draw;
enum { DD_AUG_PLAIN = 0, DD_AUG_RGB = 1, DD_AUG_NORMAL = 2, DD_AUG_SCREEN_NORMAL = 3 };
int dd_augment(const float* src, float* dst, int C, int B, int H, int W, const dd_augment_draw* draws, int kind,
               int use_flip, int use_rotate, int use_permute, int use_normal_rotation, dd_stream stream);

int dd_zero_stuff(const void* x, int ldx, void* y, int ldy, int C, int B, int H, int W, int dtype, dd_stream stream);
int dd_zero_unstuff(const void* dy, int lddy, void* dx, int lddx, const void* mask, int ldmask, int C, int B, int H, int W,
                    int accumulate, int dtype, dd_stream stream);

int dd_space_to_depth2(const void* y, int ldy, void* s, int lds, int C, int cp, int B, int H, int W, int dtype, dd_stream stream);
typedef struct {
  const void* s; int lds; int cout; int cp;
  const void* x; int ldx; int cin;
  float* dk;
  int B, H, W;
  int dtype;
} dd_convt3_wgrad_args;
int dd_convt3_wgrad(const dd_convt3_wgrad_args* a, dd_stream stream);

int dd_crc32c(const void* data, size_t n, uint32_t crc, uint32_t* out);

int dd_probe_tr16(const uint16_t* lds_image_4096, const int32_t* lane_byte_addr_64, uint16_t* out_64x4, dd_stream stream);

#ifdef __cplusplus
}
#endif
#endif
```

Baseline: 16010 tiles/s.

## Save compact ReLU bitmasks in compose forward and use them in backward

The fused compose-net forward now writes a 12-bit-per-half-pixel ReLU sign mask for each hidden activation. The streaming backward kernel reads this 2-byte word instead of reloading 48-byte bf16 activation rows to mask gradients, which cuts backward HBM traffic. It also stops materialising the g[4] gradient plane and instead has the weight-gradient kernel rebuild it from dz6 and w_out on the fly. In exchange it adds extra mask writes in forward, a new mask buffer, and more complex index logic.

```diff
diff --git a/deepdenoiser_amd/_lib.py b/deepdenoiser_amd/_lib.py
--- a/deepdenoiser_amd/_lib.py
+++ b/deepdenoiser_amd/_lib.py
@@ -32,7 +32,7 @@
     "dd_stitch", "dd_recombine", "dd_probe_tr16", "dd_masked_add", "dd_zero_stuff", "dd_zero_unstuff", "dd_convert_channels",
     "dd_augment", "dd_loss_mask_sums", "dd_crc32c", "dd_extract_tiles", "dd_compose_net_fwd", "dd_compose_net_bwd",
     "dd_kpcn_head_fwd", "dd_kpcn_head_bwd", "dd_kpcn_head_bwd_multi", "dd_assemble_input", "dd_assemble_input_frames", "dd_conv3x3_bwd", "dd_conv3x3_bwd_multi", "dd_convt2x2_fwd", "dd_convt2x2_bwd", "dd_conv3x3_ks",
-    "dd_conv_pw_count", "dd_wgrad_pw_count", "dd_space_to_depth2", "dd_convt3_wgrad", "dd_compose_stream_plan", "dd_compose_bwd_scratch_bytes",
+    "dd_conv_pw_count", "dd_wgrad_pw_count", "dd_space_to_depth2", "dd_convt3_wgrad", "dd_compose_stream_plan", "dd_compose_bwd_scratch_bytes", "dd_compose_mask_bytes",
     "dd_loss_msssim_scratch_bytes", "dd_loss_msssim_fwd", "dd_loss_msssim_bwd", "dd_loss_msssim_values",
     "dd_loss_metrics_scratch_bytes", "dd_loss_metrics", "dd_loss_head_path_count",
     "dd_loss_head_dscale", "dd_loss_msssim_bwd_dscale", "dd_grads_nonfinite", "dd_adam_step_scaled", "dd_scaler_update",
@@ -172,7 +172,7 @@
                 ("w_out", C.c_void_p), ("b_out", C.c_void_p),
                 ("save_netin", C.c_void_p), ("ld_netin", C.c_int), ("save_act", C.c_void_p * 5), ("ld_act", C.c_int * 5),
                 ("save_wl", C.c_void_p), ("ld_wl", C.c_int),
-                ("N", C.c_int), ("H", C.c_int), ("W", C.c_int), ("dtype", C.c_int)]
+                ("N", C.c_int), ("H", C.c_int), ("W", C.c_int), ("dtype", C.c_int), ("save_mask", C.c_void_p)]
 
 
 class ComposeBwdArgs(C.Structure):
@@ -183,7 +183,7 @@
                 ("dw_in", C.c_void_p), ("db_in", C.c_void_p), ("dw_res", C.c_void_p * 4), ("db_res", C.c_void_p * 4),
                 ("dw_out", C.c_void_p), ("db_out", C.c_void_p),
                 ("N", C.c_int), ("H", C.c_int), ("W", C.c_int), ("dtype", C.c_int),
-                ("scratch", C.c_void_p), ("scratch_bytes", C.c_long)]
+                ("scratch", C.c_void_p), ("scratch_bytes", C.c_long), ("mask", C.c_void_p)]
 
 
 class HeadArgs(C.Structure):
@@ -320,6 +320,8 @@
     lib.dd_compose_stream_plan.argtypes = [i, i, i, i, C.POINTER(C.c_int)]
     lib.dd_compose_bwd_scratch_bytes.argtypes = [i, i, i]
     lib.dd_compose_bwd_scratch_bytes.restype = C.c_long
+    lib.dd_compose_mask_bytes.argtypes = [i, i, i]
+    lib.dd_compose_mask_bytes.restype = C.c_long
     lib.dd_assemble_input.argtypes = [vp, i, i, vp, i, i, i, i, i, i, vp]
     lib.dd_assemble_input_frames.argtypes = [vp, i, i, vp, i, i, i, i, i, i, vp, i, i, vp]
     lib.dd_kpcn_head_fwd.argtypes = [C.POINTER(HeadArgs), vp]
diff --git a/deepdenoiser_amd/csrc/dd_compose_stream.h b/deepdenoiser_amd/csrc/dd_compose_stream.h
--- a/deepdenoiser_amd/csrc/dd_compose_stream.h
+++ b/deepdenoiser_amd/csrc/dd_compose_stream.h
@@ -50,6 +50,25 @@
 
 constexpr int PIXB = 48;
 
+typedef __attribute__((ext_vector_type(2))) unsigned short cs_u16x2;
+template <typename T> struct InfBits;
+template <> struct InfBits<bf16_t> { static constexpr unsigned short v = 0x7f80u; };
+template <> struct InfBits<f16_t> { static constexpr unsigned short v = 0x7c00u; };
+template <typename T, bool RAW>
+__device__ __forceinline__ uint32_t mask_bits(uint32_t w) {
+  const cs_u16x2 m = __builtin_bit_cast(cs_u16x2, w), one = {1, 1};
+  if (RAW) {
+    const cs_u16x2 inf = {InfBits<T>::v, InfBits<T>::v};
+    return __builtin_bit_cast(uint32_t, __builtin_elementwise_min(__builtin_elementwise_sub_sat(inf, (cs_u16x2)(m - one)), one));
+  }
+  return __builtin_bit_cast(uint32_t, __builtin_elementwise_min(m, one));
+}
+__device__ __forceinline__ uint16_t mask_word(uint32_t acc) { return (uint16_t)((acc | (acc >> 15)) & 0xfffu); }
+__device__ __forceinline__ uint32_t mask_pair(uint32_t v, uint32_t s2, int i) {
+  const dd_s16x2 keep = __builtin_bit_cast(dd_s16x2, s2 << (15 - 2 * i)) >> 15;
+  return v & __builtin_bit_cast(uint32_t, keep);
+}
+
 struct Unit { int b, yb0, yb1, xs, xe, fx0; };
 
 template <typename P>
diff --git a/deepdenoiser_amd/csrc/dd_compose_stream.hip b/deepdenoiser_amd/csrc/dd_compose_stream.hip
--- a/deepdenoiser_amd/csrc/dd_compose_stream.hip
+++ b/deepdenoiser_amd/csrc/dd_compose_stream.hip
@@ -24,6 +24,7 @@
   const float* small; const float* fine; float* out;
   const float* w_in; const float* b_in; const float* w_res[4]; const float* b_res[4]; const float* w_out; const float* b_out;
   void* save_act[5]; void* save_wl; void* save_netin;
+  uint16_t* save_mask[4];
   int ld_small, ld_fine, ld_out, ld_act[5], ld_wl, ld_netin;
   int N, H, W;
   int FW, R, TPR;
@@ -227,12 +228,15 @@
 #pragma unroll
           for (int b = 0; b < 3; ++b) { pk[b].x = in_now ? pk[b].x : 0u; pk[b].y = in_now ? pk[b].y : 0u; }
         }
+        uint32_t mb = 0u;
 #pragma unroll
         for (int b = 0; b < 3; ++b) {
           *reinterpret_cast<uint2*>(o + b * 16) = pk[b];
           if (SAVE && own_now && p.save_act[0])
             *reinterpret_cast<uint2*>(reinterpret_cast<char*>(p.save_act[0]) + ((size_t)pix_now * p.ld_act[0] + 8 * b + 4 * h) * 2) = pk[b];
-        }
+          if (SAVE) mb |= (mask_bits<T, false>(pk[b].x) << (4 * b)) | (mask_bits<T, false>(pk[b].y) << (4 * b + 2));
+        }
+        if (SAVE && own_now && p.save_mask[0]) *reinterpret_cast<uint16_t*>(reinterpret_cast<char*>(p.save_mask[0]) + (uint32_t)(4 * pix_now + 2 * h)) = mask_word(mb);
       }
       c0.i += R;
       if (c0.i >= VB) {
@@ -282,12 +286,15 @@
 #pragma unroll
             for (int b = 0; b < 3; ++b) { pk[b].x = inside ? pk[b].x : 0u; pk[b].y = inside ? pk[b].y : 0u; }
           }
+          uint32_t mb = 0u;
 #pragma unroll
           for (int b = 0; b < 3; ++b) {
             *reinterpret_cast<uint2*>(o4 + b * 16) = pk[b];
             if (SAVE && own && p.save_act[2])
               *reinterpret_cast<uint2*>(reinterpret_cast<char*>(p.save_act[2]) + ((size_t)pix * p.ld_act[2] + 8 * b + 4 * h) * 2) = pk[b];
+            if (SAVE) mb |= (mask_bits<T, true>(pk[b].x) << (4 * b)) | (mask_bits<T, true>(pk[b].y) << (4 * b + 2));
           }
+          if (SAVE && own && p.save_mask[2]) *reinterpret_cast<uint16_t*>(reinterpret_cast<char*>(p.save_mask[2]) + (uint32_t)(4 * pix + 2 * h)) = mask_word(mb);
         }
 #pragma unroll
         for (int b = 0; b < 3; ++b) { pk[b].x = relu_bf16x2(pk[b].x); pk[b].y = relu_bf16x2(pk[b].y); }
@@ -296,12 +303,15 @@
           for (int b = 0; b < 3; ++b) { pk[b].x = inside ? pk[b].x : 0u; pk[b].y = inside ? pk[b].y : 0u; }
         }
         char* o = rout + o_out + wr;
+        uint32_t mb = 0u;
 #pragma unroll
         for (int b = 0; b < 3; ++b) {
           *reinterpret_cast<uint2*>(o + b * 16) = pk[b];
           if (SAVE && LAYER != 1 && own && p.save_act[LAYER + 1])
             *reinterpret_cast<uint2*>(reinterpret_cast<char*>(p.save_act[LAYER + 1]) + ((size_t)pix * p.ld_act[LAYER + 1] + 8 * b + 4 * h) * 2) = pk[b];
-        }
+          if (SAVE && LAYER != 1) mb |= (mask_bits<T, false>(pk[b].x) << (4 * b)) | (mask_bits<T, false>(pk[b].y) << (4 * b + 2));
+        }
+        if (SAVE && LAYER != 1 && own && p.save_mask[LAYER + 1]) *reinterpret_cast<uint16_t*>(reinterpret_cast<char*>(p.save_mask[LAYER + 1]) + (uint32_t)(4 * pix + 2 * h)) = mask_word(mb);
       } else {
 #ifdef CS_EXP_NO_TAIL
         if (own && h == 0 && pk[0].x == 0x12345u) p.out[(size_t)pix * p.ld_out] = 1.f;
@@ -414,6 +424,8 @@
   return DD_OK;
 }
 
+extern "C" long dd_compose_mask_bytes(int N, int H, int W) { return (long)N * H * W * 16; }
+
 int dd_compose_stream_fwd_launch(const dd_compose_args* a, hipStream_t s) {
   CsP p;
   p.small = a->small; p.fine = a->fine; p.out = a->out;
@@ -423,6 +435,8 @@
   for (int i = 0; i < 5; ++i) { p.save_act[i] = a->save_act[i]; p.ld_act[i] = a->ld_act[i]; save = save || a->save_act[i]; }
   p.save_wl = a->save_wl; p.ld_wl = a->ld_wl;
   p.save_netin = a->save_netin; p.ld_netin = a->ld_netin; save = save || a->save_netin;
+  for (int i = 0; i < 4; ++i) p.save_mask[i] = a->save_mask ? reinterpret_cast<uint16_t*>(a->save_mask) + (size_t)i * 2 * a->N * a->H * a->W : nullptr;
+  save = save || a->save_mask;
   p.ld_small = a->ld_small; p.ld_fine = a->ld_fine; p.ld_out = a->ld_out;
   p.N = a->N; p.H = a->H; p.W = a->W;
   DD_REQUIRE((long)a->N * a->H * a->W < (1l << 31) / 64, "dd_compose_net_fwd: N * H * W = %ld pixels exceed the 32-bit offsets of the kernel", (long)a->N * a->H * a->W);
diff --git a/deepdenoiser_amd/csrc/dd_compose_stream_bwd.hip b/deepdenoiser_amd/csrc/dd_compose_stream_bwd.hip
--- a/deepdenoiser_amd/csrc/dd_compose_stream_bwd.hip
+++ b/deepdenoiser_amd/csrc/dd_compose_stream_bwd.hip
@@ -13,7 +13,8 @@
   const void* wl;
   const float* w_in; const float* w_res[4]; const float* w_out;
   float* d_small; float* d_fine;
-  void* g[5];
+  const uint16_t* mask[4];
+  void* g[4];
   void* x0;
   void* dz6;
   int ld_small, ld_fine, ld_gout, ld_act[4], ld_wl, ld_dsmall, ld_dfine, acc_small;
@@ -47,7 +48,7 @@
 
 __device__ __forceinline__ uint2 mask2(uint2 v, uint2 m) { return uint2{mask_bf16x2(v.x, m.x), mask_bf16x2(v.y, m.y)}; }
 
-template <typename T, int LAYER, int NPRE>
+template <typename T, int LAYER, int NPRE, bool MP>
 __device__ __forceinline__ void cb_role(const CbP& p, char* smem, char* aux, char* tail, int ring_bytes, int t, int lane, int u0, int nunits, int steps) {
   constexpr bool RES_AFTER = LAYER == 1;
   constexpr bool RES_INIT = LAYER == 3;
@@ -206,14 +207,12 @@
         }
         const float* wo = reinterpret_cast<const float*>(aux + 2048);
         char* o = rin + o0 + wr;
-        char* gd = reinterpret_cast<char*>(p.g[4]) + ((size_t)pix0 * 24 + 4 * h) * 2;
 #pragma unroll
         for (int b = 0; b < 3; ++b) {
           const f32x4_t wv = *reinterpret_cast<const f32x4_t*>(wo + 8 * b + 4 * h);
           uint2 pk;
           pk.x = pack2<T>(wv[0] * dz6, wv[1] * dz6); pk.y = pack2<T>(wv[2] * dz6, wv[3] * dz6);
           *reinterpret_cast<uint2*>(o + b * 16) = pk;
-          if (own0) *reinterpret_cast<uint2*>(gd + b * 16) = pk;
         }
       }
       c0.i += R;
@@ -260,15 +259,20 @@
       const int cy = row_in ? y : 0;
       const int pix = pixb + cy * W;
       constexpr int MASK_ACT = 3 - LAYER;
-      const char* mp = reinterpret_cast<const char*>(p.act[MASK_ACT]) + ((size_t)pix * p.ld_act[MASK_ACT] + 4 * h) * 2;
-      uint2 mk[3];
+      uint2 mk[3] = {uint2{0u, 0u}, uint2{0u, 0u}, uint2{0u, 0u}};
+      uint32_t mw = 0u;
+      if (MP) {
+        mw = *reinterpret_cast<const uint16_t*>(reinterpret_cast<const char*>(p.mask[MASK_ACT]) + (uint32_t)(4 * pix + 2 * h));
+      } else {
+        const char* mp = reinterpret_cast<const char*>(p.act[MASK_ACT]) + ((size_t)pix * p.ld_act[MASK_ACT] + 4 * h) * 2;
 #pragma unroll
 #ifdef CB_EXP_NO_MASK_LOADS
-      for (int b = 0; b < 3; ++b) mk[b] = uint2{0x3f803f80u, (unsigned)pix};
-      (void)mp;
+        for (int b = 0; b < 3; ++b) mk[b] = uint2{0x3f803f80u, (unsigned)pix};
+        (void)mp;
 #else
-      for (int b = 0; b < 3; ++b) mk[b] = *reinterpret_cast<const uint2*>(mp + b * 16);
+        for (int b = 0; b < 3; ++b) mk[b] = *reinterpret_cast<const uint2*>(mp + b * 16);
 #endif
+      }
       float gt[3] = {0.f, 0.f, 0.f}, wlt = 0.f;
       if (FINAL) {
         const float* gp = p.gout + (size_t)pix * p.ld_gout;
@@ -284,7 +288,18 @@
       }
       conv_part_n(std::false_type());
       uint2 pk[3];
-      if (RES_AFTER) {
+      if (RES_AFTER && MP) {
+#pragma unroll
+        for (int b = 0; b < 3; ++b) {
+          float r0, r1, r2, r3, c[4];
+          unpack2<T>(rv[b].x, r0, r1); unpack2<T>(rv[b].y, r2, r3);
+#pragma unroll
+          for (int e = 0; e < 4; ++e)
+            c[e] = __uint_as_float(__float_as_uint(acc[4 * b + e]) & (uint32_t)((int32_t)(mw << (31 - (4 * b + e))) >> 31));
+          pk[b].x = packo<T>(r0 + c[0], r1 + c[1]);
+          pk[b].y = packo<T>(r2 + c[2], r3 + c[3]);
+        }
+      } else if (RES_AFTER) {
 #pragma unroll
         for (int b = 0; b < 3; ++b) {
           float m0, m1, m2, m3, r0, r1, r2, r3;
@@ -298,7 +313,12 @@
         for (int b = 0; b < 3; ++b) {
           pk[b].x = packo<T>(acc[4 * b], acc[4 * b + 1]);
           pk[b].y = packo<T>(acc[4 * b + 2], acc[4 * b + 3]);
-          pk[b] = mask2(pk[b], mk[b]);
+          if (!MP) pk[b] = mask2(pk[b], mk[b]);
+        }
+        if (MP) {
+          const uint32_t s2 = mw | (mw << 15);
+#pragma unroll
+          for (int b = 0; b < 3; ++b) { pk[b].x = mask_pair(pk[b].x, s2, 2 * b); pk[b].y = mask_pair(pk[b].y, s2, 2 * b + 1); }
         }
       }
       if (!all_in) {
@@ -382,7 +402,7 @@
   }
 }
 
-template <typename T, int RR>
+template <typename T, int RR, bool MP>
 __global__ __launch_bounds__(1024) void compose_stream_bwd_kernel(const CbP p) {
   extern __shared__ __attribute__((aligned(16))) char smem[];
   const int tid = threadIdx.x, lane = tid & 63, wave = sfl(tid >> 6);
@@ -400,9 +420,9 @@
   const int r = t / p.TPR;
 #define CB_ROLE(L)                                                                                        \
   do {                                                                                                    \
-    if (RR == 1 || r == 0) cb_role<T, L, 9>(p, smem, aux, tail, ring_bytes, t, lane, u0, nunits, steps);  \
-    else if (RR == 2 || r == 1) cb_role<T, L, 4>(p, smem, aux, tail, ring_bytes, t, lane, u0, nunits, steps); \
-    else cb_role<T, L, 0>(p, smem, aux, tail, ring_bytes, t, lane, u0, nunits, steps);                    \
+    if (RR == 1 || r == 0) cb_role<T, L, 9, MP>(p, smem, aux, tail, ring_bytes, t, lane, u0, nunits, steps);  \
+    else if (RR == 2 || r == 1) cb_role<T, L, 4, MP>(p, smem, aux, tail, ring_bytes, t, lane, u0, nunits, steps); \
+    else cb_role<T, L, 0, MP>(p, smem, aux, tail, ring_bytes, t, lane, u0, nunits, steps);                    \
   } while (0)
   if (layer == 0) CB_ROLE(0);
   else if (layer == 1) CB_ROLE(1);
@@ -425,7 +445,8 @@
   for (int l = 0; l < 4; ++l) p.w_res[l] = a->w_res[l];
   p.d_small = a->d_small; p.d_fine = a->d_fine;
   const long npix = (long)a->N * a->H * a->W;
-  for (int i = 0; i < 5; ++i) p.g[i] = reinterpret_cast<char*>(scratch) + (size_t)i * npix * 48;
+  for (int i = 0; i < 4; ++i) p.g[i] = reinterpret_cast<char*>(scratch) + (size_t)i * npix * 48;
+  for (int i = 0; i < 4; ++i) p.mask[i] = a->mask ? reinterpret_cast<const uint16_t*>(a->mask) + (size_t)i * 2 * npix : nullptr;
   p.x0 = reinterpret_cast<char*>(scratch) + (size_t)5 * npix * 48;
   p.dz6 = reinterpret_cast<char*>(scratch) + (size_t)npix * (5 * 48 + 16);
   p.ld_small = a->ld_small; p.ld_fine = a->ld_fine; p.ld_gout = a->ld_dout; p.ld_wl = a->ld_wl; p.ld_dsmall = a->ld_dsmall; p.ld_dfine = a->ld_dfine;
@@ -438,15 +459,18 @@
   p.units = a->N * p.n_strips * p.nb;
   const int grid = p.units < cus ? p.units : cus;
   const int lds = (10 * p.R + 8) * (p.FW + 2) * PIXB + AUX_BYTES + (2 * p.R + 2) * p.FW * TAILB;
-#define CB_LAUNCH(T, RR)                                                                              \
+#define CB_LAUNCH(T, RR, MP)                                                                          \
   do {                                                                                                \
-    dd_allow_max_lds(reinterpret_cast<const void*>(compose_stream_bwd_kernel<T, RR>));                \
-    hipLaunchKernelGGL((compose_stream_bwd_kernel<T, RR>), dim3(grid), dim3(1024), lds, s, p);        \
+    dd_allow_max_lds(reinterpret_cast<const void*>(compose_stream_bwd_kernel<T, RR, MP>));            \
+    hipLaunchKernelGGL((compose_stream_bwd_kernel<T, RR, MP>), dim3(grid), dim3(1024), lds, s, p);    \
   } while (0)
-#define CB_LAUNCH_R(T) do { if (p.R == 1) CB_LAUNCH(T, 1); else if (p.R == 2) CB_LAUNCH(T, 2); else CB_LAUNCH(T, 4); } while (0)
+#define CB_LAUNCH_M(T, RR) do { if (a->mask) CB_LAUNCH(T, RR, true); else CB_LAUNCH(T, RR, false); } while (0)
+#define CB_LAUNCH_R(T) do { if (p.R == 1) CB_LAUNCH_M(T, 1); else if (p.R == 2) CB_LAUNCH_M(T, 2); else CB_LAUNCH_M(T, 4); } while (0)
   DD_REQUIRE(p.R == 1 || p.R == 2 || p.R == 4, "dd_compose_net_bwd: %d rows per step", p.R);
+  DD_REQUIRE(!a->mask || ((uintptr_t)a->mask % 2) == 0, "dd_compose_net_bwd: mask planes need 2-byte alignment");
   if (a->dtype == DD_BF16) CB_LAUNCH_R(bf16_t); else CB_LAUNCH_R(f16_t);
 #undef CB_LAUNCH_R
+#undef CB_LAUNCH_M
 #undef CB_LAUNCH
   DD_LAUNCH_CHECK();
   return DD_OK;
@@ -460,7 +484,8 @@
 
 struct CwP {
   const void* act[5];
-  const void* g[5];
+  const void* g[4];
+  const float* w_out;
   const void* x0;
   const void* dz6;
   const void* zero16;
@@ -480,7 +505,8 @@
 template <int N> __device__ __forceinline__ void cw_wait_vm() { asm volatile("s_waitcnt vmcnt(%0)" : : "n"(N) : "memory"); }
 
 constexpr int CW_G_OFF = 0, CW_A_OFF = CW_G_OFF + 20 * WG_GROW, CW_A3_OFF = CW_A_OFF + 12 * WG_AROW, CW_Z1_OFF = CW_A3_OFF + 3 * WG_AROW;
-constexpr int CW_X0_OFF = CW_Z1_OFF + 3 * WG_AROW, CW_Z6_OFF = CW_X0_OFF + 3 * 1024, CW_LDS = CW_Z6_OFF + 3 * 1024;
+constexpr int CW_X0_OFF = CW_Z1_OFF + 3 * WG_AROW, CW_Z6_OFF = CW_X0_OFF + 3 * 1024, CW_Z6H_OFF = CW_Z6_OFF + 3 * 1024;
+constexpr int CW_WO_OFF = CW_Z6H_OFF + 5 * 1024, CW_LDS = CW_WO_OFF + 128;
 
 template <typename T>
 __global__ __launch_bounds__(WG_WAVES * 64) void compose_stream_wgrad_kernel(const CwP p) {
@@ -503,56 +529,74 @@
   const bool ones_row = m == 24;
   auto gslot = [](int row) { return (row + 10) % 5; };
   auto aslot = [](int row) { return (row + 9) % 3; };
+  if (tid < 24) reinterpret_cast<float*>(smem + CW_WO_OFF)[tid] = Elem<T>::to_f32(Elem<T>::from_f32(p.w_out[tid]));
+  __syncthreads();
+  auto put_dA = [&](int slot, int pos, float z, bool exists) {
+    const f32x4_t* wo = reinterpret_cast<const f32x4_t*>(smem + CW_WO_OFF);
+    char* d = smem + CW_G_OFF + (3 * 5 + slot) * WG_GROW + pos * PIXB;
+#pragma unroll
+    for (int q = 0; q < 3; ++q) {
+      const f32x4_t w0 = wo[2 * q], w1 = wo[2 * q + 1];
+      uint4 v = {pack2<T>(w0[0] * z, w0[1] * z), pack2<T>(w0[2] * z, w0[3] * z), pack2<T>(w1[0] * z, w1[1] * z), pack2<T>(w1[2] * z, w1[3] * z)};
+      if (!exists) v = uint4{0u, 0u, 0u, 0u};
+      *reinterpret_cast<uint4*>(d + 16 * q) = v;
+    }
+  };
+  const bool has_q1 = wave == 0 || wave >= 4;
 
   for (int u = u0; u < u1; ++u) {
     const int j = u % p.nb, tq = u / p.nb, st = tq % p.strips, b = tq / p.strips;
     const int yb0 = j * p.BH, yb1 = min(H, yb0 + p.BH), xs = st * WG_SW;
-    struct Piece { const char* src; bool colok; unsigned dst; int isg, rowb; size_t rb; };
+    struct Piece { const char* src; bool colok; unsigned dst; int adv, rowb; size_t rb; };
     auto make_piece = [&](int c) {
       Piece q;
       int chunk, gx, part = 0;
       const char* base;
       size_t pxbytes = 48;
       q.rb = (size_t)W * 48;
-      if (c < 16) {
+      if (c == 12) {
+        gx = lane < 8 ? xs + 8 * lane : lane == 8 ? xs - 8 : lane == 9 ? xs + 64 : W;
+        base = reinterpret_cast<const char*>(p.dz6); pxbytes = 2; q.rb = (size_t)W * 2;
+        q.adv = 2; q.rowb = 1024; q.dst = lds0 + CW_Z6H_OFF;
+      } else if (c < 12) {
         const int tensor = c >> 2; chunk = c & 3;
         const int piece = chunk * 64 + lane, px = (piece * 171) >> 9;
         part = piece - px * 3; gx = xs - 1 + px;
         base = reinterpret_cast<const char*>(p.g[1 + tensor]);
-        q.isg = 1; q.rowb = WG_GROW;
+        q.adv = 1; q.rowb = WG_GROW;
         q.dst = lds0 + CW_G_OFF + tensor * 5 * WG_GROW + chunk * 1024;
       } else if (c < 34) {
         const int tensor = (c - 16) / 3; chunk = (c - 16) % 3;
         const int piece = chunk * 64 + lane, px = (piece * 171) >> 9;
         part = piece - px * 3; gx = xs + px;
         base = tensor < 5 ? reinterpret_cast<const char*>(p.act[tensor]) : reinterpret_cast<const char*>(p.g[0]);
-        q.isg = 0; q.rowb = WG_AROW;
+        q.adv = 0; q.rowb = WG_AROW;
         q.dst = lds0 + chunk * 1024 + (tensor < 4 ? CW_A_OFF + tensor * 3 * WG_AROW : tensor == 4 ? CW_A3_OFF : CW_Z1_OFF);
       } else if (c == 34) {
         gx = xs + lane; base = reinterpret_cast<const char*>(p.x0); pxbytes = 16; q.rb = (size_t)W * 16;
-        q.isg = 0; q.rowb = 1024; q.dst = lds0 + CW_X0_OFF;
+        q.adv = 0; q.rowb = 1024; q.dst = lds0 + CW_X0_OFF;
       } else {
         gx = lane < 8 ? xs + 8 * lane : W; base = reinterpret_cast<const char*>(p.dz6); pxbytes = 2; q.rb = (size_t)W * 2;
-        q.isg = 0; q.rowb = 1024; q.dst = lds0 + CW_Z6_OFF;
+        q.adv = 0; q.rowb = 1024; q.dst = lds0 + CW_Z6_OFF;
       }
       q.colok = (unsigned)gx < (unsigned)W;
       q.src = base + ((size_t)(b * H) * W + (q.colok ? gx : 0)) * pxbytes + part * 16;
       return q;
     };
-    const Piece q0 = make_piece(wave), q1 = make_piece(wave + 12), q2 = make_piece(wave + 24);
+    const Piece q0 = make_piece(wave), q1 = make_piece(has_q1 ? wave + 12 : wave), q2 = make_piece(wave + 24);
     auto issue = [&](const Piece& q, int y) {
-      const int row = y + q.isg;
+      const int row = y + q.adv;
       const bool ok = (unsigned)row < (unsigned)H && q.colok;
       const char* src = ok ? q.src + (size_t)row * q.rb : reinterpret_cast<const char*>(p.zero16);
-      const unsigned dst = q.dst + (q.isg ? gslot(row) : aslot(row)) * q.rowb;
+      const unsigned dst = q.dst + (q.adv ? gslot(row) : aslot(row)) * q.rowb;
       cw_dma_1k(src, (unsigned)sfl((int)dst));
     };
-    auto dma = [&](int y) { issue(q0, y); issue(q1, y); issue(q2, y); };
+    auto dma = [&](int y) { issue(q0, y); if (has_q1) issue(q1, y); issue(q2, y); };
     auto dma_first = [&](int y) {
 #pragma unroll
       for (int e = 0; e < 3; ++e) {
         const int c = wave + 12 * e;
-        if (c < 32) {
+        if (c < 32 && ((c >> 2) & 3) != 3) {
           const int tensor = (c >> 2) & 3, chunk = c & 3, row = y - 1 + (c >> 4);
           const int piece = chunk * 64 + lane, px = (piece * 171) >> 9, part = piece - px * 3;
           const int gx = xs - 1 + px;
@@ -566,10 +610,35 @@
     dma_first(yb0);
     dma(yb0);
     dma(yb0 + 1);
+    if (wave == 2) {
+      const T* z6g = reinterpret_cast<const T*>(p.dz6);
+#pragma unroll
+      for (int e = 0; e < 3; ++e) {
+        const int row = yb0 - 1 + e;
+        const bool rowok = (unsigned)row < (unsigned)H;
+#pragma unroll
+        for (int part = 0; part < 2; ++part) {
+          const int pos = part * 64 + lane, gx = xs - 1 + pos;
+          const bool exists = rowok && (unsigned)gx < (unsigned)W;
+          if (part == 0 || lane < 2) put_dA(gslot(row), pos, exists ? Elem<T>::to_f32(z6g[(size_t)(b * H + row) * W + gx]) : 0.f, exists);
+        }
+      }
+    }
     for (int y = yb0; y < yb1; ++y) {
-      cw_wait_vm<3>();
+      if (has_q1) cw_wait_vm<3>(); else cw_wait_vm<2>();
       __syncthreads();
       dma(y + 2);
+      if (wave == 2) {
+        const int row = y + 2;
+        const bool rowok = (unsigned)row < (unsigned)H;
+        const T* zr = reinterpret_cast<const T*>(smem + CW_Z6H_OFF + gslot(row) * 1024);
+#pragma unroll
+        for (int part = 0; part < 2; ++part) {
+          const int pos = part * 64 + lane;
+          const bool exists = rowok && (unsigned)(xs - 1 + pos) < (unsigned)W;
+          if (part == 0 || lane < 2) put_dA(gslot(row), pos, Elem<T>::to_f32(zr[pos == 0 ? 71 : pos == 65 ? 72 : pos - 1]), exists);
+        }
+      }
       const int grow = y - (dyi - 1);
       const unsigned abase = lds0 + CW_A_OFF + (layer * 3 + aslot(y)) * WG_AROW + tr_lane + kh * 8 * PIXB;
       const unsigned gbase = lds0 + CW_G_OFF + (layer * 5 + gslot(grow)) * WG_GROW + tr_lane + kh * 8 * PIXB;
@@ -670,7 +739,8 @@
   CwP p;
   for (int i = 0; i < 5; ++i) p.act[i] = a->act[i];
   const long npix = (long)a->N * a->H * a->W;
-  for (int i = 0; i < 5; ++i) p.g[i] = reinterpret_cast<char*>(scratch) + (size_t)i * npix * 48;
+  for (int i = 0; i < 4; ++i) p.g[i] = reinterpret_cast<char*>(scratch) + (size_t)i * npix * 48;
+  p.w_out = a->w_out;
   p.x0 = reinterpret_cast<char*>(scratch) + (size_t)5 * npix * 48;
   p.dz6 = reinterpret_cast<char*>(scratch) + (size_t)npix * (5 * 48 + 16);
   void* zp = nullptr;
diff --git a/deepdenoiser_amd/program.py b/deepdenoiser_amd/program.py
--- a/deepdenoiser_amd/program.py
+++ b/deepdenoiser_amd/program.py
@@ -88,6 +88,7 @@
         self.post_hidden = []
         self._invert_records = {}
         self._compose_scratch = []
+        self._compose_masks = []
         self._atable_ring = []
         S = arch.number_of_scales()
         if H % (1 << (len(arch.filters) - 1)) or W % (1 << (len(arch.filters) - 1)):
@@ -711,6 +712,10 @@
             del g.fwd_ops[n_fwd0:]
             ps, save = g.params, self.training
             fused_bwd = self.training and os.environ.get("DD_FUSE_COMPOSE_BWD", "1") != "0"
+            masks = None
+            if (fused_bwd and os.environ.get("DD_COMPOSE_STREAM_BWD", "1") != "0" and os.environ.get("DD_COMPOSE_MASKS", "1") != "0"):
+                masks = torch.empty(int(lib.dd_compose_mask_bytes(N, h, w)), dtype=torch.uint8, device=self.arch.device)
+                self._compose_masks.append(masks)
 
             def make_fused():
                 ca = L.ComposeArgs()
@@ -725,6 +730,8 @@
                     for i, t in enumerate(acts):
                         ca.save_act[i], ca.ld_act[i] = t.ptr, t.ld
                     ca.save_wl, ca.ld_wl = wl.ptr, wl.ld
+                    if masks is not None:
+                        ca.save_mask = masks.data_ptr()
                 ca.N, ca.H, ca.W, ca.dtype = N, h, w, g.code
 
                 def fused(stream, ca=ca):
@@ -755,6 +762,8 @@
                         if not pool or pool[-1].numel() < need:
                             pool.append(torch.empty(need, dtype=torch.uint8, device=self.arch.device))
                         cb.scratch, cb.scratch_bytes = pool[-1].data_ptr(), pool[-1].numel()
+                        if masks is not None:
+                            cb.mask = masks.data_ptr()
 
                     def make_fused_bwd():
                         cb.w_in, cb.w_out = ps.value_ptr(lay_in.kernel), ps.value_ptr(lay_out.kernel)
diff --git a/include/dd_hip.h b/include/dd_hip.h
--- a/include/dd_hip.h
+++ b/include/dd_hip.h
@@ -169,8 +169,10 @@
   void* save_act[5]; int ld_act[5];
   void* save_wl; int ld_wl;
   int N, H, W, dtype;
+  void* save_mask;
 } dd_compose_args;
 int dd_compose_net_fwd(const dd_compose_args* a, dd_stream stream);
+long dd_compose_mask_bytes(int N, int H, int W);
 int dd_compose_stream_plan(int N, int H, int W, int cus, int* out8);
 
 typedef struct {
@@ -185,6 +187,7 @@
   float* dw_in; float* db_in; float* dw_res[4]; float* db_res[4]; float* dw_out; float* db_out;
   int N, H, W, dtype;
   void* scratch; long scratch_bytes;
+  const void* mask;
 } dd_compose_bwd_args;
 int dd_compose_net_bwd(const dd_compose_bwd_args* a, dd_stream stream);
 long dd_compose_bwd_scratch_bytes(int N, int H, int W);
```

Result: no change. 15980 tiles/s (-0.2%).
